# mravanelli/pytorch-kaldi

Hardware: AMD Instinct MI355X
Metric: train_frames_per_sec (higher is better)
Workload: dtype bf16

## Files before the change

include/pk_amd.h:

```cpp
#ifndef PK_AMD_H
#define PK_AMD_H

#include <stdint.h>

#ifdef __cplusplus
extern "C" {
#endif

#define PK_PREC_F32 0
#define PK_PREC_BF16 1

#define PK_ACT_LINEAR 0
#define PK_ACT_RELU 1
#define PK_ACT_TANH 2
#define PK_ACT_SIGMOID 3
#define PK_ACT_LEAKY_RELU 4
#define PK_ACT_ELU 5

#define PK_CELL_LIGRU 0
#define PK_CELL_RNN 1
#define PK_CELL_LSTM 2
#define PK_CELL_GRU 3
#define PK_CELL_MINGRU 4

#define PK_REC_STEPWISE 0
#define PK_REC_PERSISTENT 1

int pk_version(void);
const char* pk_last_error(void);
int pk_num_cu(void);

int pk_gemm(void* stream, int prec, int M, int N, int K, float alpha, const float* A, int64_t a_rs,
            int64_t a_cs, const float* B, int64_t b_rs, int64_t b_cs, float beta, float* C, int64_t ldc,
            const float* bias, int splitk, float* workspace);
void pk_gemm_f32_set_form(int form);

int pk_gemm_bf16_tile_m(int M);
int pk_gemm_bf16_auto_splitk(int M, int N, int K);
int pk_gemm_bf16_auto_splitk_cus(int M, int N, int K, int cus);
void pk_gemm_bf16_set_tile(int tile);
int pk_gemm_bf16(void* stream, int M, int N, int K, float alpha, const uint16_t* A, int64_t lda, int a_kc,
                 const uint16_t* B, int64_t ldb, int b_kc, float beta, float* C, int64_t ldc, const float* bias,
                 int splitk, float* workspace);
int64_t pk_gemm_bf16_stats_floats(int M, int N);
int pk_gemm_bf16_stats(void* stream, int M, int N, int K, float alpha, const uint16_t* A, int64_t lda, int a_kc,
                       const uint16_t* B, int64_t ldb, int b_kc, float* C, int64_t ldc, const float* bias, float* stats,
                       int* row_blocks);
int pk_cvt_bf16(void* stream, const float* src, int64_t ld_src, int64_t rows, int nseg, int seglen, int segpad,
                uint16_t* dst, int64_t ld_dst);

int64_t pk_bn_partial_floats(int64_t M, int64_t N);
int pk_bn_stats(void* stream, const float* x, int64_t ldx, int64_t M, int64_t N, float* partial, float* mean,
                float* var);
int pk_bn_stats_merge(void* stream, const float* partial, int rb, int64_t N, float* mean, float* var);
int pk_bn_finalize(void* stream, int64_t N, const float* mean, const float* var, const float* gamma,
                   const float* beta, float eps, float* scale, float* shift, float* running_mean,
                   float* running_var, float momentum, double count);
int pk_bn_finalize_gates(void* stream, int G, int H, const float* mean, const float* var, const float* gamma,
                         const float* beta, float eps, float* scale, float* shift, float* const* running_mean,
                         float* const* running_var, int64_t* const* num_batches, float momentum, double count);
int pk_bn_stats_merge_finalize_gates(void* stream, const float* partial, int rb, int G, int H, float* mean, float* var,
                                     const float* gamma, const float* beta, float eps, float* scale, float* shift,
                                     float* const* running_mean, float* const* running_var, int64_t* const* num_batches,
                                     float momentum, double count);
int pk_affine_act_fwd(void* stream, const float* x, int64_t ldx, int64_t M, int64_t N, const float* scale,
                      const float* shift, int act, const float* mask, float* y, int64_t ldy);
int pk_act_bwd(void* stream, const float* dy, const float* a, const float* mask, int act, int64_t n, float* g);
int pk_bn_bwd_reduce(void* stream, const float* g, const float* g2, int64_t ldg, const float* x, int64_t ldx,
                     int64_t M, int64_t N, const float* mean, const float* var, float eps, float* partial,
                     float* sum_g, float* sum_gx);
int pk_bn_bwd_apply(void* stream, const float* g, const float* g2, int64_t ldg, const float* x, int64_t ldx,
                    int64_t M, int64_t N, const float* mean, const float* var, float eps, const float* gamma,
                    const float* sum_g, const float* sum_gx, double count, float* dx, int64_t lddx);
int pk_bn_bwd_bf16(void* stream, const uint16_t* g0, const uint16_t* g1, int64_t g_pitch, int G, int H, const float* x,
                   int64_t ldx, int64_t M, const float* mean, const float* var, float eps, const float* gamma,
                   double count, float* partial, float* sum_g, float* sum_gx, uint16_t* out, int64_t out_pitch,
                   float* acc_beta, float* acc_gamma);
int pk_bn_act_bwd_small_covers(int64_t M, int64_t N);
int pk_bn_act_bwd_small(void* stream, const float* dy, const float* a, const float* mask, int act, const float* z,
                        const float* mean, const float* var, float eps, const float* gamma, int64_t M, int64_t N,
                        uint16_t* dzb, int64_t ldb, float* dz, float* sum_g, float* sum_gx, float* acc_beta,
                        float* acc_gamma, float* db, float* acc_bias);
int pk_colsum(void* stream, const float* g, const float* g2, int64_t ldg, int64_t M, int64_t N, float* partial,
              float* out);
int pk_add(void* stream, const float* a, const float* b, int64_t n, float* out);

int pk_mt19937_bernoulli(void* stream, uint32_t* state, int64_t n, float keep, float* out);

int pk_sinc_bank_fwd(void* stream, const float* low_hz, const float* band_hz, const float* n_, const float* window, int N, int K,
                     float sample_rate, float min_low, float min_band, float* filt, float* mx, int32_t* kstar);
int pk_sinc_bank_bwd(void* stream, const float* g, const float* low_hz, const float* band_hz, const float* n_, const float* window,
                     const float* mx, const int32_t* kstar, int N, int K, float sample_rate, float min_low, float min_band,
                     float* dlow, float* dband);

int pk_ln_last_act_drop_fwd(void* stream, const float* z, int64_t B, int C, int L, const float* gamma, const float* beta,
                            float eps, int act, const float* mask, float* a, float* y, float* mean, float* rinv);
int pk_ln_last_act_drop_bwd(void* stream, const float* dy, const float* z, const float* a, const float* mask, int64_t B, int C,
                            int L, const float* gamma, const float* mean, const float* rinv, float eps, int act, float* dz,
                            float* pg);

int pk_layernorm_fwd(void* stream, const float* x, int64_t rows, int64_t F, const float* gamma, const float* beta,
                     float eps, float* y, float* mean, float* rinv);
int pk_layernorm_bwd(void* stream, const float* dy, const float* x, int64_t rows, int64_t F, const float* gamma,
                     const float* mean, const float* rinv, float eps, float* dx, float* dgx);

int pk_logsoftmax_fwd(void* stream, const float* x, int64_t rows, int64_t N, float* y);
int pk_logsoftmax_bwd(void* stream, const float* dy, const float* y, int64_t rows, int64_t N, float* dx);
int pk_logsoftmax_bwd_ld(void* stream, const float* dy, const float* y, int64_t rows, int64_t N, float* dx, int64_t lddx);
int pk_logsoftmax_fwd_ld(void* stream, const float* x, int64_t ldx, int64_t rows, int64_t N, float* y);
int64_t pk_logsoftmax_bwd_bf16_partial_floats(int64_t rows, int64_t N);
int pk_logsoftmax_bwd_bf16(void* stream, const float* dy, const float* y, int64_t rows, int64_t N, uint16_t* dxb,
                           int64_t ldb, float* partial, float* colsum);
int64_t pk_nll_err_partial_floats(int64_t rows);
int pk_nll_err_fwd(void* stream, const float* y, const int64_t* lab, int64_t ignore_index, int64_t rows, int64_t N,
                   float* partial, float* out4, float* loss_out, float* bad_acc);
int pk_logsoftmax_fwd_ld_argmax(void* stream, const float* x, int64_t ldx, int64_t rows, int64_t N, float* y, int32_t* amax);
int pk_nll_err_fwd_argmax(void* stream, const float* y, const int64_t* lab, const int32_t* amax, int64_t ignore_index,
                          int64_t rows, int64_t N, float* partial, float* out4, float* loss_out, float* bad_acc);
int pk_nll_logsoftmax_bwd_bf16(void* stream, const float* y, const int64_t* lab, const float* dloss, const float* count,
                               int64_t ignore_index, int64_t rows, int64_t N, uint16_t* dxb, int64_t ldb, float* partial,
                               float* colsum);
int pk_logsoftmax_bwd_bf16_p(void* stream, const float* dy, const float* y, int64_t rows, int64_t N, uint16_t* dxb,
                             int64_t ldb, int64_t pitch, float* partial, float* colsum);
int pk_nll_logsoftmax_bwd_bf16_p(void* stream, const float* y, const int64_t* lab, const float* dloss, const float* count,
                                 int64_t ignore_index, int64_t rows, int64_t N, uint16_t* dxb, int64_t ldb, int64_t pitch,
                                 float* partial, float* colsum);

int pk_rec_num_saved(int cell);
int pk_rec_num_gates(int cell);
int64_t pk_rec_work_floats(int cell, int T, int B, int bidir, int H);
int64_t pk_rec_ln_saved_floats(int T, int B, int bidir, int H);
int64_t pk_rec_ln_work_floats(int T, int B, int bidir, int H);
int pk_rec_fwd(void* stream, int algo, int prec, int cell, int act, int T, int B, int bidir, int H,
               const float* P, const float* pscale, const float* pshift, const float* U, const float* mask,
               float mask_scalar, const float* ln_gamma, const float* ln_beta, float* Y, float* S, float* LNS,
               float* work);
int pk_rec_bwd(void* stream, int algo, int prec, int cell, int act, int T, int B, int bidir, int H,
               const float* U, const float* mask, float mask_scalar, const float* ln_gamma, const float* Y,
               const float* S, const float* LNS, const float* dY, float* dP2, float* dU, float* dln_gamma,
               float* dln_beta, float* work);

int pk_rec_plan_cus(int R, int H);
int pk_rec_self_fill(int cell);
int pk_rec_fwd_bf16(void* stream, int cell, int act, int T, int B, int bidir, int H, const float* P,
                    const float* pscale, const float* pshift, const float* U, const float* mask, float mask_scalar,
                    float* Y, float* S, uint16_t* Yb, int64_t y_pitch, int prefilled);
int pk_rec_bwd_bf16(void* stream, int cell, int act, int T, int B, int bidir, int H, const float* U, const float* mask,
                    float mask_scalar, const float* Y, const float* S, const float* dY, float* dP2, uint16_t* dGb,
                    int64_t g_pitch, int prefilled);
int pk_rec_fwd_bf16_ln(void* stream, int cell, int act, int T, int B, int bidir, int H, const float* P,
                       const float* pscale, const float* pshift, const float* U, const float* mask, float mask_scalar,
                       const float* ln_gamma, const float* ln_beta, float ln_eps, float* Y, float* S, float* LNS,
                       uint16_t* Yb, int64_t y_pitch, int prefilled, float* lnwork);
int pk_rec_bwd_bf16_ln(void* stream, int cell, int act, int T, int B, int bidir, int H, const float* U, const float* mask,
                       float mask_scalar, const float* ln_gamma, float ln_eps, const float* Y, const float* S,
                       const float* LNS, const float* dY, float* dP2, uint16_t* dGb, int64_t g_pitch, int prefilled,
                       float* lnwork, float* dln_gamma, float* dln_beta);
void pk_persist2_set_trace(void* dev_buf);
void pk_persist2_set_empty_step(int on);
void pk_persist2_set_mode(int force_safe);
void pk_persist2_set_poll_delay(int units);
void pk_persist2_set_lstm_waves(int waves);
int pk_persist2_get_lstm_waves(void);
void pk_rec_helper_set_mode(int mode);
int pk_rec_helper_get_mode(void);
int pk_rec2p_fwd_bf16(void* stream, int cell, int act, int T, int B, int bidir, int H, const float* P,
                      const float* pscale, const float* pshift, const float* U, const float* mask, float mask_scalar,
                      float* Y, float* S, uint16_t* Yb, uint16_t* Xb, int64_t y_pitch, int prefilled);
int pk_rec2p_bwd_bf16(void* stream, int cell, int act, int T, int B, int bidir, int H, const float* U, const float* mask,
                      float mask_scalar, const float* Y, const float* S, const float* dY, uint16_t* dGb, int64_t g_pitch,
                      int prefilled);
int pk_rec2p_fwd_bf16_ln(void* stream, int cell, int act, int T, int B, int bidir, int H, const float* P,
                         const float* pscale, const float* pshift, const float* U, const float* mask, float mask_scalar,
                         const float* ln_gamma, const float* ln_beta, float ln_eps, float* Y, float* S, float* LNS,
                         uint16_t* Yb, uint16_t* Xb, int64_t y_pitch, int prefilled, float* lnwork);
int pk_rec2p_bwd_bf16_ln(void* stream, int cell, int act, int T, int B, int bidir, int H, const float* U, const float* mask,
                         float mask_scalar, const float* ln_gamma, float ln_eps, const float* Y, const float* S,
                         const float* LNS, const float* dY, uint16_t* dGb, int64_t g_pitch, int prefilled, float* lnwork,
                         float* dln_gamma, float* dln_beta);
unsigned pk_persist2_error_count(void);
void pk_persist2_error_reset(void);

int pk_conv1d_pool_fwd(void* stream, const float* x, const float* w, const float* bias, int B, int Cin, int L,
                       int Cout, int K, int pool, float* y, int32_t* argmax, float* work);
int64_t pk_conv_fwd_work_floats(int Cin, int Cout, int K);
int64_t pk_conv_partial_floats(int B, int Cin, int L, int Cout, int K, int pool);
int pk_conv1d_pool_bwd(void* stream, const float* x, const float* w, const float* dy, const int32_t* argmax, int B,
                       int Cin, int L, int Cout, int K, int pool, float* dw, float* dbias, float* dx,
                       float* partial);

int pk_rmsprop_step(void* stream, float* p, const float* g, float* square_avg, int64_t n, float lr, float alpha,
                    float eps, float weight_decay);
int pk_sgd_step(void* stream, float* p, const float* g, float* momentum_buf, int64_t n, float lr, float momentum,
                float weight_decay, int first_step);
int pk_adam_step(void* stream, float* p, const float* g, float* exp_avg, float* exp_avg_sq, float* max_exp_avg_sq,
                 int64_t n, float lr, float beta1, float beta2, float eps, float weight_decay, int step);
int pk_fused_step(void* stream, int kind, float* p, float* g, float* s0, float* s1, float* s2, int64_t n, float lr, float h0,
                  float h1, float h2, float weight_decay, int step, int zero_grad, const int64_t* segs, int nseg,
                  uint16_t* shadow);

unsigned pk_persist_error_count(void);
void pk_persist_error_reset(void);

int pk_linear_bn_act_bf16_covers(int64_t M, int64_t N, int64_t K);
int pk_linear_bn_act_bf16(void* stream, int M, int N, int K, const uint16_t* xb, int64_t ldx, const uint16_t* wb, int64_t ldw,
                          const float* bias, const float* gamma, const float* beta, float eps, float momentum,
                          float* running_mean, float* running_var, int act, const float* mask, float* z, float* a,
                          float* y, uint16_t* yb, int64_t ldyb, float* mean, float* var);
int pk_gemm_bf16_small_splitk(int M, int N, int K);
int pk_linear_bn_act_bf16_sk(void* stream, int M, int N, int K, const uint16_t* xb, int64_t ldx, const uint16_t* wb,
                             int64_t ldw, const float* bias, const float* gamma, const float* beta, float eps,
                             float momentum, float* running_mean, float* running_var, int act, const float* mask,
                             float* z, float* a, float* y, uint16_t* yb, int64_t ldyb, float* mean, float* var,
                             int splitk, float* ws);
int pk_conv1d_pool_dgrad(void* stream, const float* w, const float* dy, const int32_t* argmax, int B, int Cin, int L, int Cout,
                         int K, int pool, float* dx, float* work);
int pk_conv_bf16_covers(int Cin, int Cout, int K, int pool);
int64_t pk_conv_bf16_work_floats(int B, int Cin, int L, int Cout, int K, int pool, int backward);
int pk_conv1d_pool_fwd_bf16(void* stream, const float* x, const float* w, const float* bias, int B, int Cin, int L, int Cout,
                            int K, int pool, float* y, int32_t* argmax, float* work);
int pk_conv1d_pool_bwd_bf16(void* stream, const float* x, const float* w, const float* dy, const int32_t* argmax, int B,
                            int Cin, int L, int Cout, int K, int pool, float* dw, float* dx, float* work);
int pk_selftest_mfma(void* stream, int* h_bad_count);
int pk_selftest_permlane(void* stream, int* h_bad_count);
int pk_selftest_dpp_row_sum(void* stream, int* h_bad_count);
int pk_selftest_cu_hog(void* stream, int blocks, int usec, float* buf);

typedef struct pk_ark pk_ark;
pk_ark* pk_ark_open(const char* path, int64_t offset);
void pk_ark_close(pk_ark* a);
int pk_ark_next(pk_ark* a, int key_expected, char* key, int keycap, int64_t* rows, int64_t* cols);
int pk_ark_read(pk_ark* a, float* dst);
int pk_ark_skip(pk_ark* a);
int pk_ivec_next(pk_ark* a, char* key, int keycap, int64_t* n);
int pk_ivec_read(pk_ark* a, int32_t* dst);
int pk_context_window(const float* x, int64_t rows, int64_t cols, int left, int right, float* out);
int pk_mean_var_norm(float* x, int64_t rows, int64_t cols);

#ifdef __cplusplus
}
#endif
#endif
```

pytorch-kaldi_amd/_lib.py:

```python
import ctypes
import os
import re
import threading

HERE = os.path.dirname(os.path.abspath(__file__))
LIB_PATH = os.path.join(HERE, "lib", "libpk_amd.so")
HEADER = os.path.join(HERE, "..", "include", "pk_amd.h")

_lock = threading.Lock()
_lib = None

c_void_p, c_int, c_float, c_double, c_int64 = ctypes.c_void_p, ctypes.c_int, ctypes.c_float, ctypes.c_double, ctypes.c_int64
P = c_void_p

SIGNATURES = {
    "pk_version": (c_int, []),
    "pk_last_error": (ctypes.c_char_p, []),
    "pk_num_cu": (c_int, []),
    "pk_gemm": (c_int, [P, c_int, c_int, c_int, c_int, c_float, P, c_int64, c_int64, P, c_int64, c_int64, c_float, P,
                        c_int64, P, c_int, P]),
    "pk_gemm_f32_set_form": (None, [c_int]),
    "pk_gemm_bf16_tile_m": (c_int, [c_int]),
    "pk_gemm_bf16_auto_splitk": (c_int, [c_int, c_int, c_int]),
    "pk_gemm_bf16_set_tile": (None, [c_int]),
    "pk_gemm_bf16": (c_int, [P, c_int, c_int, c_int, c_float, P, c_int64, c_int, P, c_int64, c_int, c_float, P, c_int64, P,
                             c_int, P]),
    "pk_gemm_bf16_stats_floats": (c_int64, [c_int, c_int]),
    "pk_gemm_bf16_stats": (c_int, [P, c_int, c_int, c_int, c_float, P, c_int64, c_int, P, c_int64, c_int, P, c_int64, P, P, P]),
    "pk_bn_stats_merge": (c_int, [P, P, c_int, c_int64, P, P]),
    "pk_cvt_bf16": (c_int, [P, P, c_int64, c_int64, c_int, c_int, c_int, P, c_int64]),
    "pk_bn_partial_floats": (c_int64, [c_int64, c_int64]),
    "pk_bn_stats": (c_int, [P, P, c_int64, c_int64, c_int64, P, P, P]),
    "pk_bn_finalize": (c_int, [P, c_int64, P, P, P, P, c_float, P, P, P, P, c_float, c_double]),
    "pk_bn_finalize_gates": (c_int, [P, c_int, c_int, P, P, P, P, c_float, P, P, P, P, P, c_float, c_double]),
    "pk_bn_stats_merge_finalize_gates": (c_int, [P, P, c_int, c_int, c_int, P, P, P, P, c_float, P, P, P, P, P, c_float,
                                                 c_double]),
    "pk_affine_act_fwd": (c_int, [P, P, c_int64, c_int64, c_int64, P, P, c_int, P, P, c_int64]),
    "pk_act_bwd": (c_int, [P, P, P, P, c_int, c_int64, P]),
    "pk_bn_bwd_reduce": (c_int, [P, P, P, c_int64, P, c_int64, c_int64, c_int64, P, P, c_float, P, P, P]),
    "pk_bn_bwd_apply": (c_int, [P, P, P, c_int64, P, c_int64, c_int64, c_int64, P, P, c_float, P, P, P, c_double, P,
                                c_int64]),
    "pk_bn_bwd_bf16": (c_int, [P, P, P, c_int64, c_int, c_int, P, c_int64, c_int64, P, P, c_float, P, c_double, P, P, P, P,
                               c_int64, P, P]),
    "pk_colsum": (c_int, [P, P, P, c_int64, c_int64, c_int64, P, P]),
    "pk_add": (c_int, [P, P, P, c_int64, P]),
    "pk_mt19937_bernoulli": (c_int, [P, P, c_int64, c_float, P]),
    "pk_sinc_bank_fwd": (c_int, [P, P, P, P, P, c_int, c_int, c_float, c_float, c_float, P, P, P]),
    "pk_sinc_bank_bwd": (c_int, [P, P, P, P, P, P, P, P, c_int, c_int, c_float, c_float, c_float, P, P]),
    "pk_ln_last_act_drop_fwd": (c_int, [P, P, c_int64, c_int, c_int, P, P, c_float, c_int, P, P, P, P, P]),
    "pk_ln_last_act_drop_bwd": (c_int, [P, P, P, P, P, c_int64, c_int, c_int, P, P, P, c_float, c_int, P, P]),
    "pk_layernorm_fwd": (c_int, [P, P, c_int64, c_int64, P, P, c_float, P, P, P]),
    "pk_layernorm_bwd": (c_int, [P, P, P, c_int64, c_int64, P, P, P, c_float, P, P]),
    "pk_logsoftmax_fwd": (c_int, [P, P, c_int64, c_int64, P]),
    "pk_logsoftmax_bwd": (c_int, [P, P, P, c_int64, c_int64, P]),
    "pk_logsoftmax_bwd_ld": (c_int, [P, P, P, c_int64, c_int64, P, c_int64]),
    "pk_logsoftmax_fwd_ld": (c_int, [P, P, c_int64, c_int64, c_int64, P]),
    "pk_logsoftmax_fwd_ld_argmax": (c_int, [P, P, c_int64, c_int64, c_int64, P, P]),
    "pk_logsoftmax_bwd_bf16_partial_floats": (c_int64, [c_int64, c_int64]),
    "pk_logsoftmax_bwd_bf16": (c_int, [P, P, P, c_int64, c_int64, P, c_int64, P, P]),
    "pk_nll_err_partial_floats": (c_int64, [c_int64]),
    "pk_nll_err_fwd": (c_int, [P, P, P, c_int64, c_int64, c_int64, P, P, P, P]),
    "pk_nll_err_fwd_argmax": (c_int, [P, P, P, P, c_int64, c_int64, c_int64, P, P, P, P]),
    "pk_nll_logsoftmax_bwd_bf16": (c_int, [P, P, P, P, P, c_int64, c_int64, c_int64, P, c_int64, P, P]),
    "pk_logsoftmax_bwd_bf16_p": (c_int, [P, P, P, c_int64, c_int64, P, c_int64, c_int64, P, P]),
    "pk_nll_logsoftmax_bwd_bf16_p": (c_int, [P, P, P, P, P, c_int64, c_int64, c_int64, P, c_int64, c_int64, P, P]),
    "pk_rec_num_saved": (c_int, [c_int]),
    "pk_rec_num_gates": (c_int, [c_int]),
    "pk_conv1d_pool_dgrad": (c_int, [P, P, P, P, c_int, c_int, c_int, c_int, c_int, c_int, P, P]),
    "pk_conv_bf16_covers": (c_int, [c_int, c_int, c_int, c_int]),
    "pk_conv_bf16_work_floats": (c_int64, [c_int, c_int, c_int, c_int, c_int, c_int, c_int]),
    "pk_conv1d_pool_fwd_bf16": (c_int, [P, P, P, P, c_int, c_int, c_int, c_int, c_int, c_int, P, P, P]),
    "pk_conv1d_pool_bwd_bf16": (c_int, [P, P, P, P, P, c_int, c_int, c_int, c_int, c_int, c_int, P, P, P]),
    "pk_bn_act_bwd_small_covers": (c_int, [c_int64, c_int64]),
    "pk_bn_act_bwd_small": (c_int, [P, P, P, P, c_int, P, P, P, c_float, P, c_int64, c_int64, P, c_int64, P, P, P, P, P, P, P]),
    "pk_rec_work_floats": (c_int64, [c_int, c_int, c_int, c_int, c_int]),
    "pk_rec_ln_saved_floats": (c_int64, [c_int, c_int, c_int, c_int]),
    "pk_rec_ln_work_floats": (c_int64, [c_int, c_int, c_int, c_int]),
    "pk_rec_fwd": (c_int, [P, c_int, c_int, c_int, c_int, c_int, c_int, c_int, c_int, P, P, P, P, P, c_float, P, P, P,
                           P, P, P]),
    "pk_rec_bwd": (c_int, [P, c_int, c_int, c_int, c_int, c_int, c_int, c_int, c_int, P, P, c_float, P, P, P, P, P, P,
                           P, P, P, P]),
    "pk_rec_self_fill": (c_int, [c_int]),
    "pk_rec_plan_cus": (c_int, [c_int, c_int]),
    "pk_gemm_bf16_auto_splitk_cus": (c_int, [c_int, c_int, c_int, c_int]),
    "pk_rec_fwd_bf16": (c_int, [P, c_int, c_int, c_int, c_int, c_int, c_int, P, P, P, P, P, c_float, P, P, P, c_int64, c_int]),
    "pk_rec_bwd_bf16": (c_int, [P, c_int, c_int, c_int, c_int, c_int, c_int, P, P, c_float, P, P, P, P, P, c_int64, c_int]),
    "pk_rec2p_fwd_bf16_ln": (c_int, [P, c_int, c_int, c_int, c_int, c_int, c_int, P, P, P, P, P, c_float, P, P, c_float, P, P, P,
                                     P, P, c_int64, c_int, P]),
    "pk_rec2p_bwd_bf16_ln": (c_int, [P, c_int, c_int, c_int, c_int, c_int, c_int, P, P, c_float, P, c_float, P, P, P, P, P,
                                     c_int64, c_int, P, P, P]),
    "pk_rec_fwd_bf16_ln": (c_int, [P, c_int, c_int, c_int, c_int, c_int, c_int, P, P, P, P, P, c_float, P, P, c_float, P, P, P,
                                   P, c_int64, c_int, P]),
    "pk_rec_bwd_bf16_ln": (c_int, [P, c_int, c_int, c_int, c_int, c_int, c_int, P, P, c_float, P, c_float, P, P, P, P, P, P,
                                   c_int64, c_int, P, P, P]),
    "pk_rec2p_fwd_bf16": (c_int, [P, c_int, c_int, c_int, c_int, c_int, c_int, P, P, P, P, P, c_float, P, P, P, P, c_int64, c_int]),
    "pk_rec2p_bwd_bf16": (c_int, [P, c_int, c_int, c_int, c_int, c_int, c_int, P, P, c_float, P, P, P, P, c_int64, c_int]),
    "pk_persist2_set_trace": (None, [P]),
    "pk_persist2_set_empty_step": (None, [c_int]),
    "pk_persist2_set_mode": (None, [c_int]),
    "pk_persist2_set_poll_delay": (None, [c_int]),
    "pk_persist2_set_lstm_waves": (None, [c_int]),
    "pk_rec_helper_set_mode": (None, [c_int]),
    "pk_rec_helper_get_mode": (c_int, []),
    "pk_persist2_get_lstm_waves": (c_int, []),
    "pk_persist2_error_count": (ctypes.c_uint, []),
    "pk_persist2_error_reset": (None, []),
    "pk_conv1d_pool_fwd": (c_int, [P, P, P, P, c_int, c_int, c_int, c_int, c_int, c_int, P, P, P]),
    "pk_conv_fwd_work_floats": (c_int64, [c_int, c_int, c_int]),
    "pk_conv_partial_floats": (c_int64, [c_int, c_int, c_int, c_int, c_int, c_int]),
    "pk_conv1d_pool_bwd": (c_int, [P, P, P, P, P, c_int, c_int, c_int, c_int, c_int, c_int, P, P, P, P]),
    "pk_ark_open": (P, [ctypes.c_char_p, c_int64]),
    "pk_ark_close": (None, [P]),
    "pk_ark_next": (c_int, [P, c_int, ctypes.c_char_p, c_int, ctypes.POINTER(c_int64), ctypes.POINTER(c_int64)]),
    "pk_ark_read": (c_int, [P, P]),
    "pk_ark_skip": (c_int, [P]),
    "pk_ivec_next": (c_int, [P, ctypes.c_char_p, c_int, ctypes.POINTER(c_int64)]),
    "pk_ivec_read": (c_int, [P, P]),
    "pk_context_window": (c_int, [P, c_int64, c_int64, c_int, c_int, P]),
    "pk_mean_var_norm": (c_int, [P, c_int64, c_int64]),
    "pk_rmsprop_step": (c_int, [P, P, P, P, c_int64, c_float, c_float, c_float, c_float]),
    "pk_sgd_step": (c_int, [P, P, P, P, c_int64, c_float, c_float, c_float, c_int]),
    "pk_adam_step": (c_int, [P, P, P, P, P, P, c_int64, c_float, c_float, c_float, c_float, c_float, c_int]),
    "pk_fused_step": (c_int, [P, c_int, P, P, P, P, P, c_int64, c_float, c_float, c_float, c_float, c_float, c_int, c_int, P, c_int, P]),
    "pk_persist_error_count": (ctypes.c_uint, []),
    "pk_persist_error_reset": (None, []),
    "pk_linear_bn_act_bf16_covers": (c_int, [c_int64, c_int64, c_int64]),
    "pk_linear_bn_act_bf16": (c_int, [P, c_int, c_int, c_int, P, c_int64, P, c_int64, P, P, P, c_float, c_float, P, P, c_int, P,
                                      P, P, P, P, c_int64, P, P]),
    "pk_gemm_bf16_small_splitk": (c_int, [c_int, c_int, c_int]),
    "pk_linear_bn_act_bf16_sk": (c_int, [P, c_int, c_int, c_int, P, c_int64, P, c_int64, P, P, P, c_float, c_float, P, P, c_int, P,
                                         P, P, P, P, c_int64, P, P, c_int, P]),
    "pk_selftest_mfma": (c_int, [P, ctypes.POINTER(c_int)]),
    "pk_selftest_permlane": (c_int, [P, ctypes.POINTER(c_int)]),
    "pk_selftest_dpp_row_sum": (c_int, [P, ctypes.POINTER(c_int)]),
    "pk_selftest_cu_hog": (c_int, [P, c_int, c_int, P]),
}


def declared_symbols():
    with open(HEADER) as f:
        text = re.sub(r"/\*.*?\*/", "", f.read(), flags=re.S)
    return sorted(set(re.findall(r"\b(pk_[a-z0-9_]+)\s*\(", text)))


class PkError(RuntimeError):
    pass


def _map_torch_hip_runtime():
    import torch

    hip = os.path.join(os.path.dirname(torch.__file__), "lib", "libamdhip64.so")
    if os.path.exists(hip):
        ctypes.CDLL(hip, mode=ctypes.RTLD_GLOBAL)
    return hip


def hip_runtimes_mapped():
    try:
        with open("/proc/self/maps") as f:
            return {line.split()[-1] for line in f if "libamdhip64" in line}
    except OSError:
        return set()


def load():
    global _lib
    if _lib is not None:
        return _lib
    with _lock:
        if _lib is not None:
            return _lib
        if not os.path.exists(LIB_PATH):
            raise PkError(
                "libpk_amd.so is not built (%s). Run `python -c 'import __graft_entry__ as g; g.build()'`; "
                "this engine has no CPU fallback." % LIB_PATH)
        warn_unknown_switches()
        _map_torch_hip_runtime()
        lib = ctypes.CDLL(LIB_PATH)
        runtimes = hip_runtimes_mapped()
        if len(runtimes) > 1:
            raise PkError("two HIP runtimes in one process (%s): libpk_amd.so must share the one torch uses - streams and "
                          "device pointers of one runtime mean nothing to the other" % ", ".join(sorted(runtimes)))
        for name, (res, args) in SIGNATURES.items():
            fn = getattr(lib, name)
            fn.restype = res
            fn.argtypes = args
        _lib = lib
    return _lib


def check(rc, what):
    if rc != 0:
        msg = load().pk_last_error()
        raise PkError("%s failed (rc=%d): %s" % (what, rc, msg.decode() if msg else "?"))


def raise_if_persist_failed():
    lib = load()
    n = lib.pk_persist_error_count() + lib.pk_persist2_error_count()
    if n:
        lib.pk_persist_error_reset()
        lib.pk_persist2_error_reset()
        raise PkError("persistent recurrent kernel: %d wave(s) timed out waiting for a peer workgroup "
                      "(results of that launch are invalid)" % n)


_profiler = None
_raw_load = load


class _TimedLib:

    def __init__(self, lib, prof):
        self._lib, self._prof = lib, prof

    def __getattr__(self, name):
        fn = getattr(self._lib, name)
        sig = SIGNATURES.get(name)
        if sig is None or not sig[1] or sig[1][0] is not P or name.startswith("pk_selftest_"):
            return fn
        prof = self._prof

        def timed(*a):
            import torch

            e0 = torch.cuda.Event(enable_timing=True)
            e1 = torch.cuda.Event(enable_timing=True)
            e0.record()
            rc = fn(*a)
            e1.record()
            prof.events.append((name, e0, e1))
            return rc

        return timed


_EXP_CACHE = (None, {})
# ... 107 lines not shown
```

pytorch-kaldi_amd/csrc/pk_gemm_bf16.hip:

```cpp
#include <stdlib.h>

#include "pk_common.h"

namespace {

constexpr int TM = 128, TN = 128, TK = 64;
typedef short s4v __attribute__((ext_vector_type(4)));

struct BArgs {
    int M, N, K;
    float alpha, beta;
    const unsigned short* A;
    long lda;
    const unsigned short* B;
    long ldb;
    float* C;
    long ldc;
    const float* bias;
    float* ws;
    int k_per_split;
    int tiles_m, tiles_n;
    int items, per_xcd;
    const unsigned short* zeros;
    float* stats;
// ... 993 lines not shown
                for (int ah = 0; ah < 2; ++ah)
#pragma unroll
                    for (int i = 0; i < 4; ++i) {
                        const int row = m0 + ah * 128 + wm * 64 + i * 16 + (lane & 15);
                        const f32x4 v = acc[ah][bh][i][j];
                        f32x4 o;
#pragma unroll
                        for (int r = 0; r < 4; ++r) o[r] = alpha * v[r] + bv[r];
                        *reinterpret_cast<f32x4*>(base + (long)row * ld + col) = o;
                    }
            }
        return;
    }
#pragma unroll
    for (int ah = 0; ah < 2; ++ah)
#pragma unroll
        for (int bh = 0; bh < 2; ++bh)
#pragma unroll
            for (int i = 0; i < 4; ++i)
#pragma unroll
                for (int j = 0; j < 2; ++j)
                    store_frag(p, acc[ah][bh][i][j], m0 + ah * 128 + wm * 64 + i * 16 + (lane & 15),
                               n0 + bh * 128 + wn * 32 + j * 16 + (lane >> 4) * 4, split, vec_ok);
}

__global__ void splitk_reduce_bf_kernel(const float* __restrict__ ws, int splitk, int M, int N, float alpha, float beta,
                                        const float* __restrict__ bias, float* __restrict__ C, long ldc) {
    const long total = (long)M * N;
    if ((N & 3) == 0 && (ldc & 3) == 0 && (((uintptr_t)C | (uintptr_t)ws) & 15) == 0) {
        const long quads = total >> 2;
        for (long qd = blockIdx.x * (long)blockDim.x + threadIdx.x; qd < quads; qd += (long)gridDim.x * blockDim.x) {
            const long i = qd << 2;
            const int row = (int)(i / N), col = (int)(i - (long)row * N);
            f32x4 s = f32x4{0.f, 0.f, 0.f, 0.f};
            for (int k0 = 0; k0 < splitk; k0 += 8) {
                f32x4 t[8];
#pragma unroll
                for (int j = 0; j < 8; ++j) t[j] = *reinterpret_cast<const f32x4*>(ws + (long)(k0 + j < splitk ? k0 + j : splitk - 1) * total + i);
#pragma unroll
                for (int j = 0; j < 8; ++j)
#pragma unroll
                    for (int e = 0; e < 4; ++e) s[e] += (k0 + j < splitk) ? t[j][e] : 0.f;
            }
            float* c = C + (long)row * ldc + col;
            f32x4 o;
#pragma unroll
            for (int e = 0; e < 4; ++e) o[e] = alpha * s[e] + (bias ? bias[col + e] : 0.f);
            if (beta != 0.f) {
                const f32x4 cv = *reinterpret_cast<const f32x4*>(c);
#pragma unroll
                for (int e = 0; e < 4; ++e) o[e] += beta * cv[e];
            }
            *reinterpret_cast<f32x4*>(c) = o;
        }
        return;
    }
    for (long i = blockIdx.x * (long)blockDim.x + threadIdx.x; i < total; i += (long)gridDim.x * blockDim.x) {
        const int row = (int)(i / N), col = (int)(i % N);
        float s = 0.f;
        for (int k = 0; k < splitk; ++k) s += ws[(long)k * total + i];
        float o = alpha * s + (bias ? bias[col] : 0.f);
        float* c = C + (long)row * ldc + col;
        if (beta != 0.f) o += beta * (*c);
        *c = o;
    }
}

__global__ void cvt_bf16_kernel(const float* __restrict__ src, long lds, long rows, int nseg, int seglen, int segpad,
                                unsigned short* __restrict__ dst, long ldd) {
    const long chunks_per_row = ldd >> 3;
    const long total = rows * chunks_per_row;
    for (long i = blockIdx.x * (long)blockDim.x + threadIdx.x; i < total; i += (long)gridDim.x * blockDim.x) {
        const long r = i / chunks_per_row;
        const int c0 = (int)(i - r * chunks_per_row) * 8;
        const float* s = src + r * lds;
        unsigned pk[4];
#pragma unroll
        for (int e = 0; e < 4; ++e) {
            float v[2];
#pragma unroll
            for (int h = 0; h < 2; ++h) {
                const int c = c0 + 2 * e + h;
                const int sg = c / segpad, off = c - sg * segpad;
                v[h] = (sg < nseg && off < seglen) ? s[sg * seglen + off] : 0.f;
            }
            pk[e] = pk_pack_bf2(v[0], v[1]);
        }
        *reinterpret_cast<uint4*>(dst + r * ldd + c0) = make_uint4(pk[0], pk[1], pk[2], pk[3]);
    }
}

}

extern "C" int pk_cvt_bf16(void* stream, const float* src, int64_t ld_src, int64_t rows, int nseg, int seglen, int segpad,
                           uint16_t* dst, int64_t ld_dst) {
    if (rows <= 0) return 0;
    PK_REQUIRE(nseg >= 1 && seglen >= 1 && segpad >= seglen, "pk_cvt_bf16: bad segments");
    PK_REQUIRE((ld_dst % 8) == 0 && ld_dst >= (int64_t)nseg * segpad - (segpad - seglen) && ((uintptr_t)dst & 15) == 0,
               "pk_cvt_bf16: destination pitch must be a multiple of 8 elements and hold every segment");
    const long total = rows * (ld_dst >> 3);
    long blocks = (total + 255) / 256;
    if (blocks > 8192) blocks = 8192;
    hipLaunchKernelGGL(cvt_bf16_kernel, dim3((unsigned)blocks), dim3(256), 0, pk_stream(stream), src, (long)ld_src,
                       (long)rows, nseg, seglen, segpad, (unsigned short*)dst, (long)ld_dst);
    PK_LAUNCH_CHECK();
    return 0;
}

static int g_gemm_tile_forced = -1;
extern "C" void pk_gemm_bf16_set_tile(int tile) { g_gemm_tile_forced = (tile == 128 || tile == 256) ? tile : 0; }
static int gemm_tile_for(int M, int N, int a_kc, int b_kc, int K = 1 << 30) {
    int& forced = g_gemm_tile_forced;
    if (forced < 0) {
        const char* e = pk_experiment("gemm_tile");
        forced = (e && atoi(e) == 128) ? 128 : (e && atoi(e) == 256) ? 256 : 0;
    }
    if (forced) return forced;
    static int rows256 = -1;
    if (rows256 < 0) {
        const char* e = pk_experiment("gemm_tile_rows");
        rows256 = (e && atoi(e) == 0) ? 0 : 1;
    }
    if (rows256 && a_kc && M >= 16384 && N >= 1024) return 256;
    if (!a_kc && !b_kc && M >= 1024 && N >= 1024) {
        const long tiles256 = (long)((M + 255) / 256) * ((N + 255) / 256);
        if (K < 2048 && tiles256 < 64) return 128;
        return 256;
    }
    return 128;
}

extern "C" int pk_gemm_bf16_tile_m(int M) {
    (void)M;
    return TM;
}

extern "C" int pk_gemm_bf16_auto_splitk_cus(int M, int N, int K, int cus) {
    if (K < 2048 || M <= 0 || N <= 0) return 1;
    const int t = gemm_tile_for(M, N, 0, 0);
    const long tiles = (long)((M + t - 1) / t) * ((N + t - 1) / t);
    long ncu = pk_num_cu();
    if (cus > 0 && cus < ncu) ncu = cus;
    long s = (t == 256 ? ncu : 2 * ncu) / (tiles > 0 ? tiles : 1);
    if (s < 1) s = 1;
    if (s > 32) s = 32;
    const long kmax = K / 512 > 0 ? K / 512 : 1;
    if (s > kmax) s = kmax;
    return (int)s;
}
extern "C" int pk_gemm_bf16_auto_splitk(int M, int N, int K) { return pk_gemm_bf16_auto_splitk_cus(M, N, K, 0); }

static int gemm_bf16_impl(void* stream, int M, int N, int K, float alpha, const uint16_t* A, int64_t lda, int a_kc,
                          const uint16_t* B, int64_t ldb, int b_kc, float beta, float* C, int64_t ldc, const float* bias,
                          int splitk, float* workspace, float* stats) {
    if (M <= 0 || N <= 0) return 0;
    PK_REQUIRE(K >= 0, "pk_gemm_bf16: negative K");
    PK_REQUIRE((lda % 8) == 0 && (ldb % 8) == 0 && ((uintptr_t)A & 15) == 0 && ((uintptr_t)B & 15) == 0,
               "pk_gemm_bf16: operands need 16-byte aligned bases and pitches that are multiples of 8 elements");
    PK_REQUIRE(!a_kc || (K % 8) == 0 || lda >= ((K + 7) & ~7), "pk_gemm_bf16: A pitch shorter than K rounded up to 8");
    PK_REQUIRE(!b_kc || (K % 8) == 0 || ldb >= ((K + 7) & ~7), "pk_gemm_bf16: B pitch shorter than K rounded up to 8");
    PK_REQUIRE(a_kc || lda >= ((M + 7) & ~7), "pk_gemm_bf16: k-major A needs a pitch of at least M rounded up to 8");
    PK_REQUIRE(b_kc || ldb >= ((N + 7) & ~7), "pk_gemm_bf16: k-major B needs a pitch of at least N rounded up to 8");
    hipStream_t st = pk_stream(stream);
    BArgs p;
    p.M = M; p.N = N; p.K = K;
    p.alpha = alpha; p.beta = beta;
    p.A = A; p.lda = lda; p.B = B; p.ldb = ldb;
    p.C = C; p.ldc = ldc; p.bias = bias;
    p.stats = stats;
    const int tile = gemm_tile_for(M, N, a_kc, b_kc, K);
    PK_REQUIRE(stats == nullptr || (tile == 256 && a_kc && b_kc && splitk <= 1 && beta == 0.f), "pk_gemm_bf16_stats: internal: shape not covered");
    p.tiles_m = (M + tile - 1) / tile;
    p.tiles_n = (N + tile - 1) / tile;
    static void* zp = nullptr;
    if (zp == nullptr) PK_CHECK_HIP(hipGetSymbolAddress(&zp, HIP_SYMBOL(g_zero_page)));
    p.zeros = (const unsigned short*)zp;
    if (splitk < 1) splitk = 1;
    if (splitk > 1) {
        PK_REQUIRE(workspace != nullptr, "pk_gemm_bf16: split-K needs a workspace");
        int kps = (K + splitk - 1) / splitk;
        kps = ((kps + TK - 1) / TK) * TK;
        splitk = kps > 0 ? (K + kps - 1) / kps : 1;
        p.k_per_split = kps;
    }
    if (splitk <= 1) {
        splitk = 1;
        p.k_per_split = ((K + TK - 1) / TK) * TK;
        if (p.k_per_split == 0) p.k_per_split = TK;
    }
    p.ws = splitk > 1 ? workspace : nullptr;
    p.items = splitk * p.tiles_m * p.tiles_n;
    p.per_xcd = (p.items + 7) / 8;
    {
        static int skinny_on = -1;
        if (skinny_on < 0) {
            const char* e = pk_experiment("gemm_skinny");
            skinny_on = (e && e[0] == '0') ? 0 : 1;
        }
        if (skinny_on && !g_gemm_tile_forced && a_kc && M <= TM && splitk > 1 && p.k_per_split <= SK_TILES * TK && stats == nullptr) {
            static bool attr_done = false;
            if (!attr_done) {
                PK_CHECK_HIP(hipFuncSetAttribute((const void*)gemm_bf16sk_kernel<true>, hipFuncAttributeMaxDynamicSharedMemorySize, SK_TILES * SSTAGE));
                PK_CHECK_HIP(hipFuncSetAttribute((const void*)gemm_bf16sk_kernel<false>, hipFuncAttributeMaxDynamicSharedMemorySize, SK_TILES * SSTAGE));
                attr_done = true;
            }
            const dim3 sgrid((unsigned)((N + SN - 1) / SN), (unsigned)splitk);
            if (b_kc) hipLaunchKernelGGL((gemm_bf16sk_kernel<true>), sgrid, dim3(256), SK_TILES * SSTAGE, st, p);
            else hipLaunchKernelGGL((gemm_bf16sk_kernel<false>), sgrid, dim3(256), SK_TILES * SSTAGE, st, p);
            PK_LAUNCH_CHECK();
            const long total = (long)M * N;
            int blocks = (int)((total + 255) / 256);
            if (blocks > 2048) blocks = 2048;
            hipLaunchKernelGGL(splitk_reduce_bf_kernel, dim3(blocks), dim3(256), 0, st, workspace, splitk, M, N, alpha, beta,
                               bias, C, (long)ldc);
            PK_LAUNCH_CHECK();
            return 0;
        }
        if (skinny_on && !g_gemm_tile_forced && !a_kc && !b_kc && splitk == 1 && K <= 512 && stats == nullptr &&
            (long)((M + TM - 1) / TM) * ((N + TN - 1) / TN) <= 192 && M >= 64 && N >= 64) {
            const dim3 tgrid((unsigned)((N + 63) / 64), (unsigned)((M + 63) / 64));
            hipLaunchKernelGGL(gemm_bf16_t64_kernel, tgrid, dim3(256), T64_TILES * T64_STAGE, st, p);
            PK_LAUNCH_CHECK();
            return 0;
        }
        if (skinny_on && !g_gemm_tile_forced && a_kc && M <= TM && N >= 4 * SN && splitk == 1 && stats == nullptr) {
            BnActArgs q = {};
            const dim3 sgrid((unsigned)((N + SN - 1) / SN));
            if (b_kc) hipLaunchKernelGGL((gemm_bf16s_kernel<false, true>), sgrid, dim3(256), 2 * SSTAGE, st, p, q);
            else hipLaunchKernelGGL((gemm_bf16s_kernel<false, false>), sgrid, dim3(256), 2 * SSTAGE, st, p, q);
            PK_LAUNCH_CHECK();
            return 0;
        }
    }
    if (tile == 256) {
        static bool attr_done = false;
        if (!attr_done) {
            PK_CHECK_HIP(hipFuncSetAttribute((const void*)gemm_bf16_256_kernel<true, true>, hipFuncAttributeMaxDynamicSharedMemorySize, 8 * PIECE));
            PK_CHECK_HIP(hipFuncSetAttribute((const void*)gemm_bf16_256_kernel<true, false>, hipFuncAttributeMaxDynamicSharedMemorySize, 8 * PIECE));
            PK_CHECK_HIP(hipFuncSetAttribute((const void*)gemm_bf16_256_kernel<false, true>, hipFuncAttributeMaxDynamicSharedMemorySize, 8 * PIECE));
            PK_CHECK_HIP(hipFuncSetAttribute((const void*)gemm_bf16_256_kernel<false, false>, hipFuncAttributeMaxDynamicSharedMemorySize, 8 * PIECE));
            attr_done = true;
        }
        dim3 grid256((unsigned)(p.per_xcd * 8)), block512(512);
        const size_t lds256 = 8 * PIECE;
        if (a_kc && b_kc) hipLaunchKernelGGL((gemm_bf16_256_kernel<true, true>), grid256, block512, lds256, st, p);
        else if (a_kc && !b_kc) hipLaunchKernelGGL((gemm_bf16_256_kernel<true, false>), grid256, block512, lds256, st, p);
        else if (!a_kc && b_kc) hipLaunchKernelGGL((gemm_bf16_256_kernel<false, true>), grid256, block512, lds256, st, p);
        else hipLaunchKernelGGL((gemm_bf16_256_kernel<false, false>), grid256, block512, lds256, st, p);
        PK_LAUNCH_CHECK();
        if (splitk > 1) {
            const long total = (long)M * N;
            int blocks = (int)((total + 255) / 256);
            if (blocks > 2048) blocks = 2048;
            hipLaunchKernelGGL(splitk_reduce_bf_kernel, dim3(blocks), dim3(256), 0, st, workspace, splitk, M, N, alpha, beta,
                               bias, C, (long)ldc);
            PK_LAUNCH_CHECK();
        }
        return 0;
    }
    dim3 grid((unsigned)(p.per_xcd * 8)), block(256);
    static int forced = -1;
    if (forced < 0) {
        const char* e = pk_experiment("gemm_stages");
        forced = (e && e[0] == '1') ? 1 : (e && e[0] == '2') ? 2 : 0;
        PK_CHECK_HIP(hipFuncSetAttribute((const void*)gemm_bf16x_kernel<true, true, 2>, hipFuncAttributeMaxDynamicSharedMemorySize, 65536));
        PK_CHECK_HIP(hipFuncSetAttribute((const void*)gemm_bf16x_kernel<true, false, 2>, hipFuncAttributeMaxDynamicSharedMemorySize, 65536));
        PK_CHECK_HIP(hipFuncSetAttribute((const void*)gemm_bf16x_kernel<false, true, 2>, hipFuncAttributeMaxDynamicSharedMemorySize, 65536));
        PK_CHECK_HIP(hipFuncSetAttribute((const void*)gemm_bf16x_kernel<false, false, 2>, hipFuncAttributeMaxDynamicSharedMemorySize, 65536));
    }
    const int stages = forced ? forced : (a_kc ? 1 : 2);
    const size_t lds = stages == 2 ? 65536 : 32768;
#define PK_LAUNCH_BF(ST)                                                                                     \
    do {                                                                                                     \
        if (a_kc && b_kc) hipLaunchKernelGGL((gemm_bf16x_kernel<true, true, ST>), grid, block, lds, st, p);    \
        else if (a_kc && !b_kc) hipLaunchKernelGGL((gemm_bf16x_kernel<true, false, ST>), grid, block, lds, st, p); \
        else if (!a_kc && b_kc) hipLaunchKernelGGL((gemm_bf16x_kernel<false, true, ST>), grid, block, lds, st, p); \
        else hipLaunchKernelGGL((gemm_bf16x_kernel<false, false, ST>), grid, block, lds, st, p);              \
    } while (0)
    if (stages == 2) PK_LAUNCH_BF(2);
    else PK_LAUNCH_BF(1);
#undef PK_LAUNCH_BF
    PK_LAUNCH_CHECK();
    if (splitk > 1) {
        const long total = (long)M * N;
        int blocks = (int)((total + 255) / 256);
        if (blocks > 2048) blocks = 2048;
        hipLaunchKernelGGL(splitk_reduce_bf_kernel, dim3(blocks), dim3(256), 0, st, workspace, splitk, M, N, alpha, beta,
                           bias, C, (long)ldc);
        PK_LAUNCH_CHECK();
    }
    return 0;
}

extern "C" int pk_gemm_bf16(void* stream, int M, int N, int K, float alpha, const uint16_t* A, int64_t lda, int a_kc,
                            const uint16_t* B, int64_t ldb, int b_kc, float beta, float* C, int64_t ldc,
                            const float* bias, int splitk, float* workspace) {
    return gemm_bf16_impl(stream, M, N, K, alpha, A, lda, a_kc, B, ldb, b_kc, beta, C, ldc, bias, splitk, workspace, nullptr);
}

extern "C" int64_t pk_gemm_bf16_stats_floats(int M, int N) { return (int64_t)((M + 255) / 256) * N * 3; }

extern "C" int pk_gemm_bf16_stats(void* stream, int M, int N, int K, float alpha, const uint16_t* A, int64_t lda, int a_kc,
                                  const uint16_t* B, int64_t ldb, int b_kc, float* C, int64_t ldc, const float* bias,
                                  float* stats, int* row_blocks) {
    PK_REQUIRE(row_blocks != nullptr, "pk_gemm_bf16_stats: null row_blocks");
    const bool fused = stats != nullptr && M > 0 && N > 0 && K > 0 && a_kc && b_kc && gemm_tile_for(M, N, a_kc, b_kc) == 256;
    *row_blocks = fused ? (M + 255) / 256 : 0;
    return gemm_bf16_impl(stream, M, N, K, alpha, A, lda, a_kc, B, ldb, b_kc, 0.f, C, ldc, bias, 1, nullptr,
                          fused ? stats : nullptr);
}

extern "C" int pk_gemm_bf16_small_splitk(int M, int N, int K) {
    if (M < 1 || M > TM || N < 1 || K < 2 * TK) return 1;
    const int col_tiles = (N + SN - 1) / SN;
    int s = 256 / col_tiles;
    const int need = (K + SK_TILES * TK - 1) / (SK_TILES * TK);
    if (s < need) s = need;
    if (s > 16) s = 16;
    const int tiles = (K + TK - 1) / TK;
    if (s > tiles) s = tiles;
    if (s < 2) return 1;
    int kps = ((K + s - 1) / s + TK - 1) / TK * TK;
    if (kps > SK_TILES * TK) return 1;
    return (K + kps - 1) / kps;
}

extern "C" int pk_linear_bn_act_bf16_sk(void* stream, int M, int N, int K, const uint16_t* xb, int64_t ldx, const uint16_t* wb,
                                        int64_t ldw, const float* bias, const float* gamma, const float* beta, float eps,
                                        float momentum, float* running_mean, float* running_var, int act, const float* mask,
                                        float* z, float* a, float* y, uint16_t* yb, int64_t ldyb, float* mean, float* var,
                                        int splitk, float* ws) {
    PK_REQUIRE(pk_linear_bn_act_bf16_covers(M, N, K), "pk_linear_bn_act_bf16_sk: needs 2 <= M <= 128 rows and N a multiple of 8 (got %d x %d)", M, N);
    PK_REQUIRE((ldx % 8) == 0 && (ldw % 8) == 0 && ((uintptr_t)xb & 15) == 0 && ((uintptr_t)wb & 15) == 0 && ldx >= ((K + 7) & ~7) &&
                   ldw >= ((K + 7) & ~7),
               "pk_linear_bn_act_bf16_sk: operands need 16-byte aligned bases and pitches that are multiples of 8 elements");
    PK_REQUIRE(z && a && yb && mean && var && (mask == nullptr || y != nullptr) && ldyb >= N && (ldyb % 4) == 0,
               "pk_linear_bn_act_bf16_sk: null output or bad pitch");
    PK_REQUIRE((((uintptr_t)z | (uintptr_t)a | (uintptr_t)y | (uintptr_t)mask | (uintptr_t)ws | (uintptr_t)bias) & 15) == 0 && ((uintptr_t)yb & 7) == 0,
               "pk_linear_bn_act_bf16_sk: fp32 matrices need 16-byte aligned bases");
    PK_REQUIRE(splitk >= 2 && ws != nullptr, "pk_linear_bn_act_bf16_sk: needs splitk >= 2 and a workspace of splitk x M x N floats");
    int kps = ((K + splitk - 1) / splitk + TK - 1) / TK * TK;
    PK_REQUIRE(kps <= SK_TILES * TK, "pk_linear_bn_act_bf16_sk: %d splits of K = %d exceed %d k-tiles per workgroup", splitk, K, SK_TILES);
    splitk = (K + kps - 1) / kps;
    hipStream_t st = pk_stream(stream);
    BArgs p;
    p.M = M; p.N = N; p.K = K;
    p.alpha = 1.f; p.beta = 0.f;
    p.A = xb; p.lda = ldx; p.B = wb; p.ldb = ldw;
    p.C = z; p.ldc = N; p.bias = nullptr;
    p.stats = nullptr; p.ws = ws;
    p.tiles_m = 1; p.tiles_n = (N + TN - 1) / TN;
    p.k_per_split = kps;
    p.items = p.tiles_n; p.per_xcd = (p.items + 7) / 8;
    static void* zp = nullptr;
    if (zp == nullptr) PK_CHECK_HIP(hipGetSymbolAddress(&zp, HIP_SYMBOL(g_zero_page)));
    p.zeros = (const unsigned short*)zp;
    static bool attr_done = false;
    if (!attr_done) {
        PK_CHECK_HIP(hipFuncSetAttribute((const void*)gemm_bf16sk_kernel<true>, hipFuncAttributeMaxDynamicSharedMemorySize, SK_TILES * SSTAGE));
        attr_done = true;
    }
    hipLaunchKernelGGL((gemm_bf16sk_kernel<true>), dim3((unsigned)((N + SN - 1) / SN), (unsigned)splitk), dim3(256), SK_TILES * SSTAGE, st, p);
    PK_LAUNCH_CHECK();
    BnActArgs q;
    q.gamma = gamma; q.beta = beta; q.mask = mask;
    q.eps = eps; q.momentum = momentum; q.unbias = M > 1 ? (float)M / (float)(M - 1) : 1.f;
    q.rmean = running_mean; q.rvar = running_var; q.mean = mean; q.var = var;
    q.zout = z; q.aout = a; q.yout = y; q.yb = (unsigned short*)yb; q.ldyb = ldyb; q.act = act;
    hipLaunchKernelGGL(linear_bn_act_epi_kernel, dim3((unsigned)((N + EP_COLS - 1) / EP_COLS)), dim3(256), 0, st, ws, splitk, M, N, bias, q);
    PK_LAUNCH_CHECK();
    return 0;
}

extern "C" int pk_linear_bn_act_bf16_covers(int64_t M, int64_t N, int64_t K) {
    return M >= 2 && M <= TM && N >= 8 && (N % 8) == 0 && K >= 1;
}
extern "C" int pk_linear_bn_act_bf16(void* stream, int M, int N, int K, const uint16_t* xb, int64_t ldx, const uint16_t* wb,
                                     int64_t ldw, const float* bias, const float* gamma, const float* beta, float eps,
                                     float momentum, float* running_mean, float* running_var, int act, const float* mask,
                                     float* z, float* a, float* y, uint16_t* yb, int64_t ldyb, float* mean, float* var) {
    PK_REQUIRE(pk_linear_bn_act_bf16_covers(M, N, K), "pk_linear_bn_act_bf16: needs 2 <= M <= 128 rows and N a multiple of 8 (got %d x %d)", M, N);
    PK_REQUIRE((ldx % 8) == 0 && (ldw % 8) == 0 && ((uintptr_t)xb & 15) == 0 && ((uintptr_t)wb & 15) == 0 && ldx >= ((K + 7) & ~7) &&
                   ldw >= ((K + 7) & ~7),
               "pk_linear_bn_act_bf16: operands need 16-byte aligned bases and pitches that are multiples of 8 elements");
    PK_REQUIRE(z && a && yb && mean && var && (mask == nullptr || y != nullptr) && ldyb >= N && (ldyb % 4) == 0,
               "pk_linear_bn_act_bf16: null output or bad pitch");
    PK_REQUIRE((((uintptr_t)z | (uintptr_t)a | (uintptr_t)y | (uintptr_t)mask) & 15) == 0 && ((uintptr_t)yb & 7) == 0,
               "pk_linear_bn_act_bf16: fp32 matrices need 16-byte aligned bases");
    hipStream_t st = pk_stream(stream);
    BArgs p;
    p.M = M; p.N = N; p.K = K;
    p.alpha = 1.f; p.beta = 0.f;
    p.A = xb; p.lda = ldx; p.B = wb; p.ldb = ldw;
    p.C = z; p.ldc = N; p.bias = bias;
    p.stats = nullptr; p.ws = nullptr;
    p.tiles_m = 1; p.tiles_n = (N + TN - 1) / TN;
    p.k_per_split = ((K + TK - 1) / TK) * TK;
    p.items = p.tiles_n; p.per_xcd = (p.items + 7) / 8;
    static void* zp = nullptr;
    if (zp == nullptr) PK_CHECK_HIP(hipGetSymbolAddress(&zp, HIP_SYMBOL(g_zero_page)));
    p.zeros = (const unsigned short*)zp;
    BnActArgs q;
    q.gamma = gamma; q.beta = beta; q.mask = mask;
    q.eps = eps; q.momentum = momentum; q.unbias = M > 1 ? (float)M / (float)(M - 1) : 1.f;
    q.rmean = running_mean; q.rvar = running_var; q.mean = mean; q.var = var;
    q.zout = z; q.aout = a; q.yout = y; q.yb = (unsigned short*)yb; q.ldyb = ldyb; q.act = act;
    hipLaunchKernelGGL((gemm_bf16s_kernel<true>), dim3((unsigned)((N + SN - 1) / SN)), dim3(256), 2 * SSTAGE, st, p, q);
    PK_LAUNCH_CHECK();
    return 0;
}
```

pytorch-kaldi_amd/csrc/pk_rec2_common.h:

```cpp
#pragma once
#ifndef PK_REC2_PRECISE
#define PK_CELL_FAST_MATH 1
#endif
#include "pk_cell.h"

#define PK_R2_FILL_AHEAD 4
struct R2Args {
    int T, B, R, H, Hp, YH, act;
    int C, Pn, rpc, row0;
    const float *P, *pscale, *pshift, *U, *mask;
    float mask_scalar;
    float* Y;
    float* S;
    unsigned short* Yb;
    unsigned short* Xb;
    int Ypitch;
    const float* dY;
    float* dP2;
    unsigned short* dGb;
    int Gpitch;
    float* Yx;
    float* dGx;
    float* Xx;
    unsigned* err;
    int spin_limit;
    float* trash;
    int poll_delay;
    int force_safe;
    unsigned* xcd_tab;
    unsigned hs_gen;
    unsigned long long* trace;
    int helper_delay;
    int self_fill;
    int flush_late;
    int empty_step;
    const float *ln_gamma, *ln_beta;
    float ln_eps;
    float* lnh;
    float* lnstat;
    float* lnx;
    float* lnpart;
    int ln_cg0;
    int ln_ncg;
};

struct Plan2 {
    int Pn, C, rpc, launches;
};

namespace {

typedef unsigned int u32x4 __attribute__((ext_vector_type(4)));

constexpr int KPAD = 576;
constexpr int KSTEPS = 18;
constexpr int RMAX = 16;

__host__ __device__ constexpr int pk_r2_lda_bf16(int k_elems) { return k_elems + 8 * ((((2 - k_elems / 8) % 16) + 16) % 16); }
__host__ __device__ constexpr int pk_r2_lda_f32(int k_elems) { return k_elems + 4 * ((((2 - k_elems / 4) % 16) + 16) % 16); }


#define PK_TRACE(slot)                                                                      \
    do {                                                                                    \
        if (TR && a.trace != nullptr && blockIdx.x == 0 && tid == 0) a.trace[(long)step_idx * 8 + (slot)] = __builtin_amdgcn_s_memtime(); \
    } while (0)

__device__ __forceinline__ bool has_sent16(const u32x4 v) {
    const unsigned m01 = v[0] > v[1] ? v[0] : v[1], m23 = v[2] > v[3] ? v[2] : v[3];
    return (m01 > m23 ? m01 : m23) == 0xFFFFFFFFu;
}
__device__ __forceinline__ unsigned short to_bf_pub(float f) {
    const unsigned short u = __builtin_bit_cast(unsigned short, (__bf16)f);
    return u == (unsigned short)0xFFFF ? (unsigned short)0x7FC0 : u;
}
__device__ __forceinline__ bool spin_check2(int& spins, int spin_limit, unsigned* err, int lane) {
    if (++spins > spin_limit) {
        if (lane == 0) atomicAdd_system(err, 1u);
        return true;
    }
    if ((spins & 63) == 0 && __hip_atomic_load(err, __ATOMIC_RELAXED, __HIP_MEMORY_SCOPE_SYSTEM) != 0u) return true;
    __builtin_amdgcn_s_sleep(1);
    return false;
}
__device__ __forceinline__ __amdgpu_buffer_rsrc_t make_rsrc(const void* p, unsigned bytes) {
    return __builtin_amdgcn_make_buffer_rsrc(const_cast<void*>(p), 0, (int)bytes, 0x00020000);
}

template <bool FAST>
__device__ __forceinline__ u32x4 poll_load(__amdgpu_buffer_rsrc_t rs, unsigned off) {
    return FAST ? __builtin_amdgcn_raw_buffer_load_b128(rs, off, 0, 2) : __builtin_amdgcn_raw_buffer_load_b128(rs, off, 0, 16);
}
template <bool FAST>
__device__ __forceinline__ void pub_store(__amdgpu_buffer_rsrc_t rs, unsigned off, u32x4 v) {
    if (FAST) __builtin_amdgcn_raw_buffer_store_b128(v, rs, off, 0, 0);
    else __builtin_amdgcn_raw_buffer_store_b128(v, rs, off, 0, 16);
}

template <int NCH, bool FAST>
__device__ __forceinline__ bool poll_to_lds(__amdgpu_buffer_rsrc_t rs, const unsigned (&goff)[NCH], const int (&loff)[NCH],
                                            unsigned char* tile, unsigned* err, int spin_limit, int lane, bool dead,
                                            int& retries) {
    u32x4 v[NCH];
#pragma unroll
    for (int i = 0; i < NCH; ++i) v[i] = poll_load<FAST>(rs, goff[i]);
    bool bad = false;
#pragma unroll
    for (int i = 0; i < NCH; ++i) bad = bad | has_sent16(v[i]);
    if (__any(bad) && !dead) {
        int spins = 0;
        while (true) {
#pragma unroll
            for (int i = 0; i < NCH; ++i)
                if (has_sent16(v[i])) v[i] = poll_load<FAST>(rs, goff[i]);
            bad = false;
#pragma unroll
            for (int i = 0; i < NCH; ++i) bad = bad | has_sent16(v[i]);
            ++retries;
            if (!__any(bad)) break;
            if (spin_check2(spins, spin_limit, err, lane)) {
                dead = true;
                break;
            }
        }
    }
#pragma unroll
    for (int i = 0; i < NCH; ++i) *reinterpret_cast<u32x4*>(tile + loff[i]) = v[i];
    return dead;
}

__device__ __forceinline__ float dpp_row_sum(float v) {
    v += __int_as_float(__builtin_amdgcn_update_dpp(0, __float_as_int(v), 0xB1, 0xF, 0xF, true));
    v += __int_as_float(__builtin_amdgcn_update_dpp(0, __float_as_int(v), 0x4E, 0xF, 0xF, true));
    v += __int_as_float(__builtin_amdgcn_update_dpp(0, __float_as_int(v), 0x141, 0xF, 0xF, true));
    v += __int_as_float(__builtin_amdgcn_update_dpp(0, __float_as_int(v), 0x140, 0xF, 0xF, true));
    return v;
}
__device__ __forceinline__ unsigned ln_bits(float f) {
    const unsigned u = __float_as_uint(f);
    return u == 0xFFFFFFFFu ? 0x7FC00000u : u;
}
template <bool FAST, int NP = 3>
__device__ __forceinline__ bool ln_row_allreduce(__amdgpu_buffer_rsrc_t rsx, unsigned pub_off, const unsigned (&poll_off)[NP],
                                                 float (&a)[4], float (&b)[4], unsigned* err, int spin_limit, int lane, bool dead) {
#pragma unroll
    for (int r = 0; r < 4; ++r) {
        a[r] = dpp_row_sum(a[r]);
        b[r] = dpp_row_sum(b[r]);
    }
    pub_store<FAST>(rsx, pub_off, u32x4{ln_bits(a[0]), ln_bits(b[0]), ln_bits(a[1]), ln_bits(b[1])});
    pub_store<FAST>(rsx, pub_off + 16u, u32x4{ln_bits(a[2]), ln_bits(b[2]), ln_bits(a[3]), ln_bits(b[3])});
    u32x4 v[2 * NP];
#pragma unroll
    for (int i = 0; i < 2 * NP; ++i) v[i] = poll_load<FAST>(rsx, poll_off[i >> 1] + (unsigned)(i & 1) * 16u);
    bool bad = false;
#pragma unroll
    for (int i = 0; i < 2 * NP; ++i) bad = bad | has_sent16(v[i]);
    if (__any(bad) && !dead) {
        int spins = 0;
        while (true) {
#pragma unroll
            for (int i = 0; i < 2 * NP; ++i)
                if (has_sent16(v[i])) v[i] = poll_load<FAST>(rsx, poll_off[i >> 1] + (unsigned)(i & 1) * 16u);
            bad = false;
#pragma unroll
            for (int i = 0; i < 2 * NP; ++i) bad = bad | has_sent16(v[i]);
            if (!__any(bad)) break;
            if (spin_check2(spins, spin_limit, err, lane)) {
                dead = true;
                break;
            }
        }
    }
#pragma unroll
    for (int r = 0; r < 4; ++r) {
        const int ch = r >> 1, e = (r & 1) * 2;
        float sa = __uint_as_float(v[ch][e]), sb = __uint_as_float(v[ch][e + 1]);
#pragma unroll
        for (int g = 1; g < NP; ++g) {
            sa += __uint_as_float(v[2 * g + ch][e]);
            sb += __uint_as_float(v[2 * g + ch][e + 1]);
        }
        a[r] = dpp_row_sum(sa);
        b[r] = dpp_row_sum(sb);
    }
    return dead;
}
template <int NP>
struct LnSlotsN {
    unsigned pub, poll[NP], slab, size;
    bool pub_ok, poll_ok[NP];
    __device__ __forceinline__ unsigned pub_at(int step) const { return pub_ok ? pub + (unsigned)step * slab : size; }
    __device__ __forceinline__ void poll_at(int step, unsigned (&o)[NP]) const {
#pragma unroll
        for (int i = 0; i < NP; ++i) o[i] = poll_ok[i] ? poll[i] + (unsigned)step * slab : size;
    }
};
// ... 187 lines not shown
```

pytorch-kaldi_amd/csrc/pk_rec_persist2.hip:

```cpp
#include <atomic>
#include <stdlib.h>

#include "pk_rec2_common.h"

namespace {

template <int CELL, int ACT, bool TR, bool LN = false, bool NOSAVE = false>
__global__ __launch_bounds__(256, 1) void rec2_fwd_kernel(R2Args a) {
    const int act = ACT >= 0 ? ACT : a.act;
    constexpr int G = pk_cell_gates(CELL), NS = pk_cell_saved(CELL);
    constexpr int LDA = pk_r2_lda_bf16(KPAD);
    constexpr int ATILE = RMAX * LDA * 2;
    constexpr int NCH = (RMAX * (KPAD / 8) + 255) / 256;
    constexpr int NF = G + 1 + NS + (LN ? 1 : 0);
    constexpr int WAVE_LDS = NF * 1024 + 512;
    constexpr int LDS_TRASH = 2 * ATILE + 4 * WAVE_LDS;
    extern __shared__ __attribute__((aligned(16))) unsigned char smem[];

    const int tid = threadIdx.x, lane = tid & 63, wave = tid >> 6;
    const int c = blockIdx.x % a.C, p = blockIdx.x / a.C;
    const int H = a.H, Hp = a.Hp, B = a.B, T = a.T, GH = G * H;
    const int n_base = a.row0 + c * a.rpc;
    int nrows = a.R - n_base;
    nrows = nrows < a.rpc ? nrows : a.rpc;
    if (nrows <= 0) return;
    const int ubase = p * 64 + wave * 16;
    const int unit = ubase + (lane & 15);
    const bool unit_ok = unit < H;
    const int kq = lane >> 4;

    bf16x8 Bf[G][KSTEPS];
    {
        const unsigned szU = (unsigned)((size_t)G * H * H * 4);
        const __amdgpu_buffer_rsrc_t rsU = make_rsrc(a.U, szU);
#pragma unroll
        for (int g = 0; g < G; ++g) {
            u32x4 raw[KSTEPS][2];
#pragma unroll
            for (int kk = 0; kk < KSTEPS; ++kk) {
                const int k0 = kk * 32 + kq * 8;
                const unsigned off = (unsigned)(((g * H + unit) * H + k0) * 4);
                raw[kk][0] = __builtin_amdgcn_raw_buffer_load_b128(rsU, (unit_ok && k0 < H) ? off : szU, 0, 0);
                raw[kk][1] = __builtin_amdgcn_raw_buffer_load_b128(rsU, (unit_ok && k0 + 4 < H) ? off + 16 : szU, 0, 0);
            }
#pragma unroll
            for (int kk = 0; kk < KSTEPS; ++kk) {
                bf16x8 f;
#pragma unroll
                for (int e = 0; e < 8; ++e) {
                    const int k = kk * 32 + kq * 8 + e;
                    const float w = (k < H) ? __uint_as_float(raw[kk][e >> 2][e & 3]) : 0.f;
                    f[e] = (short)pk_f2bf(w);
                }
                Bf[g][kk] = f;
            }
        }
    }
    float psc[G], psh[G];
#pragma unroll
    for (int g = 0; g < G; ++g) {
        psc[g] = unit_ok ? a.pscale[g * H + unit] : 0.f;
        psh[g] = unit_ok ? a.pshift[g * H + unit] : 0.f;
    }
    for (int i = tid; i < (LDS_TRASH + 16) / 4; i += 256) reinterpret_cast<unsigned*>(smem)[i] = 0u;

    const int CPR = Hp >> 3;
    const unsigned TS = (unsigned)B * a.Ypitch * 2u;
    const unsigned szYb = (unsigned)T * TS;
    unsigned cbase[NCH], cstep[NCH];
    int clds[NCH];
#pragma unroll
    for (int i = 0; i < NCH; ++i) {
        const int ci = tid + 256 * i;
        const bool ok = ci < nrows * CPR;
        const int row = ok ? ci / CPR : 0, col = ok ? ci - row * CPR : 0;
        const int n = n_base + row;
        const int dir = n >= B ? 1 : 0, b = n - dir * B;
        cbase[i] = ok ? ((unsigned)b * a.Ypitch + dir * Hp + col * 8) * 2u + (unsigned)(dir ? (T - 1) : 0) * TS : szYb;
        cstep[i] = ok ? (dir ? 0u - TS : TS) : 0u;
        clds[i] = ok ? row * (LDA * 2) + col * 16 : LDS_TRASH;
    }
    float rvf[4], msk[4], hprev[4], cprev[4];
#pragma unroll
    for (int r = 0; r < 4; ++r) {
        const int row = kq * 4 + r, n = n_base + row;
        const bool ok = row < nrows && unit_ok;
        rvf[r] = ok ? 1.f : 0.f;
        msk[r] = (a.mask != nullptr && ok) ? a.mask[(long)n * H + unit] : a.mask_scalar;
        hprev[r] = 0.f;
        cprev[r] = 0.f;
    }
    const int vrow = lane >> 2, vu0 = ubase + (lane & 3) * 4;
    const int vn = n_base + (vrow < nrows ? vrow : 0);
    const int vdir = vn >= B ? 1 : 0, vb = vn - vdir * B;
    int vnv = H - vu0;
    vnv = vnv > 4 ? 4 : (vnv < 0 ? 0 : vnv);
    const int edge = __any(vnv > 0 && vnv < 4) != 0 ? ((H & 1) ? 2 : 1) : 0;
    vnv = vrow < nrows ? vnv : 0;
    const unsigned vP0 = ((unsigned)vb * GH + vu0), vPs = (unsigned)B * GH;
    const unsigned vY0 = ((unsigned)vb * a.YH + vdir * H + vu0), vYs = (unsigned)B * a.YH;
    const unsigned vS0 = (((unsigned)vdir * T * B + vb) * (NS * H) + vu0), vSs = (unsigned)B * NS * H;
    const int prow = lane >> 1, phalf = lane & 1;
    const int pu0 = ubase + phalf * 8;
    const bool pk_ok = lane < 32 && prow < nrows && pu0 < Hp;
    const int pn = n_base + (prow < nrows ? prow : 0);
    const int pdir = pn >= B ? 1 : 0, pb = pn - pdir * B;
    const unsigned pbase = pk_ok ? ((unsigned)pb * a.Ypitch + pdir * Hp + pu0) * 2u : szYb;

    unsigned char* wl = smem + 2 * ATILE + wave * WAVE_LDS;
    float* patchP = reinterpret_cast<float*>(wl);
    float* patchY = reinterpret_cast<float*>(wl + G * 1024);
    float* patchS = reinterpret_cast<float*>(wl + (G + 1) * 1024);
    float* patchL = reinterpret_cast<float*>(wl + (G + 1 + NS) * 1024);
    unsigned short* patchB = reinterpret_cast<unsigned short*>(wl + NF * 1024);
    const __amdgpu_buffer_rsrc_t rs = make_rsrc(a.Yb, szYb);
    float* trash = a.trash + (tid & 63) * 4;
    const LnSlots ls = LN ? ln_slots(a, c, p, wave, lane, T) : LnSlots();
    const __amdgpu_buffer_rsrc_t rsx = make_rsrc(LN ? (const void*)a.lnx : (const void*)a.Yb, LN ? ls.size : 0u);
    const float gam = (LN && unit_ok) ? a.ln_gamma[unit] : 0.f, bet = (LN && unit_ok) ? a.ln_beta[unit] : 0.f;
    const float invH = 1.0f / (float)H, inv_nm1 = 1.0f / (float)(H - 1);
    float piv[4] = {0.f, 0.f, 0.f, 0.f};
    pk_f32x2 st_val = {0.f, 0.f};
    const int st_row = kq * 4 + (lane & 3);
    const bool st_ok = LN && p == 0 && wave == 0 && (lane & 15) < 4 && st_row < nrows;
    float* const st_base = st_ok ? a.lnstat + (long)(n_base + st_row) * 2 : trash;
    const long st_step = st_ok ? (long)a.R * 2 : 0;

    f32x4 pv[G];
    auto load_proj = [&](int tt, auto E) {
        const unsigned ts = (unsigned)(vdir ? (T - 1 - tt) : tt);
#pragma unroll
        for (int g = 0; g < G; ++g) pv[g] = ld4<decltype(E)::value>(a.P, vP0 + ts * vPs + g * H, vnv);
    };
    const bool want_y = a.Y != nullptr;
    auto flush_outputs = [&](int tt, auto E) {
        constexpr int EE = decltype(E)::value;
        const unsigned ts = (unsigned)(vdir ? (T - 1 - tt) : tt);
        if (!NOSAVE || want_y) st4<EE>(a.Y, vY0 + ts * vYs, vnv, trash, patch_get_vec(patchY, lane));
        if constexpr (!NOSAVE) {
#pragma unroll
            for (int k = 0; k < NS; ++k) st4<EE>(a.S, vS0 + ts * vSs + k * H, vnv, trash, patch_get_vec(patchS + k * 256, lane));
        }
        if (LN) {
            st4<EE>(a.lnh, vY0 + ts * vYs, vnv, trash, patch_get_vec(patchL, lane));
            *reinterpret_cast<pk_f32x2*>(st_base + (long)tt * st_step) = st_val;
        }
    };
#define PK_LP0(E) load_proj(0, E)
    PK_EDGE_DISPATCH(PK_LP0);
    const u32x4 sentinel = u32x4{0xFFFFFFFFu, 0xFFFFFFFFu, 0xFFFFFFFFu, 0xFFFFFFFFu};
    if (a.self_fill) {
        for (int tt = 0; tt < PK_R2_FILL_AHEAD && tt < T; ++tt)
            pub_store<false>(rs, pbase + (pk_ok ? (unsigned)(pdir ? (T - 1 - tt) : tt) * TS : 0u), sentinel);
        asm volatile("s_waitcnt vmcnt(0)" ::: "memory");
    }
    __syncthreads();

    bool dead = false;
    const bool fast_rt = __builtin_amdgcn_readfirstlane((int)(cluster_on_one_xcd(a, c, p, tid, dead) && a.force_safe == 0)) != 0;
    auto run = [&](auto FASTC, auto SEC) {
    const bool fast = decltype(FASTC)::value < 0 ? fast_rt : decltype(FASTC)::value != 0;
    constexpr int SE = decltype(SEC)::value;
    for (int t = 0; t < T; ++t) {
        const int step_idx = t;
        PK_TRACE(0);
        f32x4 acc[G];
#pragma unroll
        for (int g = 0; g < G; ++g) acc[g] = f32x4{0.f, 0.f, 0.f, 0.f};
        unsigned char* At = smem + (t & 1) * ATILE;
        if (t > 0) {
            unsigned goff[NCH];
#pragma unroll
            for (int i = 0; i < NCH; ++i) goff[i] = cbase[i] + (unsigned)(t - 1) * cstep[i];
            for (int d = 0; d < a.poll_delay; ++d) __builtin_amdgcn_s_sleep(1);
            int retries = 0;
            dead = fast ? poll_to_lds<NCH, true>(rs, goff, clds, At, a.err, a.spin_limit, lane, dead, retries)
                        : poll_to_lds<NCH, false>(rs, goff, clds, At, a.err, a.spin_limit, lane, dead, retries);
            if (a.trace != nullptr && blockIdx.x == 0 && tid == 0) a.trace[(long)step_idx * 8 + 6] = (unsigned long long)retries;
        }
        PK_TRACE(1);
#pragma unroll
        for (int g = 0; g < G; ++g) patch_put_vec(patchP + g * 256, lane, pv[g]);
        if (t > 0) PK_BARRIER_LDS();
        else PK_LDS_ORDER();
        PK_TRACE(2);
        if (t > 0) {
#define PK_FO(E) flush_outputs(t - 1, E)
            PK_EDGE_DISPATCH_S(PK_FO);
        }
        if (t + 1 < T) {
#define PK_LP1(E) load_proj(t + 1, E)
            PK_EDGE_DISPATCH_S(PK_LP1);
        }
        if (a.self_fill && t + PK_R2_FILL_AHEAD < T) {
            const unsigned off = pbase + (pk_ok ? (unsigned)(pdir ? (T - 1 - (t + PK_R2_FILL_AHEAD)) : (t + PK_R2_FILL_AHEAD)) * TS : 0u);
            if (fast) pub_store<true>(rs, off, sentinel);
            else pub_store<false>(rs, off, sentinel);
        }
        const bool empty = TR && a.empty_step != 0;
        if (t > 0 && !empty) {
            const unsigned char* Ar = At + (lane & 15) * (LDA * 2) + kq * 16;
#pragma unroll
            for (int kk = 0; kk < KSTEPS; ++kk) {
                const bf16x8 af = *reinterpret_cast<const bf16x8*>(Ar + kk * 64);
#pragma unroll
                for (int g = 0; g < G; ++g) acc[g] = __builtin_amdgcn_mfma_f32_16x16x32_bf16(af, Bf[g][kk], acc[g], 0, 0, 0);
            }
        }
        PK_TRACE(3);
        float pre[G][4];
#pragma unroll
        for (int g = 0; g < G; ++g) patch_get_cd(patchP + g * 256, kq, lane, pre[g]);
        float hv[4], sv[NS][4];
#pragma unroll
        for (int r = 0; r < 4; ++r) {
            float pr[G];
#pragma unroll
            for (int g = 0; g < G; ++g) pr[g] = pre[g][r] * psc[g] + psh[g] + acc[g][r];
            float h, cc, s[NS];
            if (empty) {
                h = 0.25f;
                cc = 0.f;
#pragma unroll
                for (int k = 0; k < NS; ++k) s[k] = pr[0];
            } else {
                pk_cell_fwd<CELL>(act, pr, hprev[r], cprev[r], msk[r], h, cc, s);
            }
            h = rvf[r] != 0.f ? h : 0.f;
            cc = rvf[r] != 0.f ? cc : 0.f;
            hprev[r] = h;
            cprev[r] = cc;
            hv[r] = h;
#pragma unroll
            for (int k = 0; k < NS; ++k) sv[k][r] = s[k];
            if (!LN) patchB[(kq * 4 + r) * 16 + (lane & 15)] = to_bf_pub(h);
        }
        if (LN) {
            if (t == 0) {
                float ma[4], mb[4];
#pragma unroll
                for (int r = 0; r < 4; ++r) {
                    ma[r] = rvf[r] != 0.f ? hv[r] : 0.f;
                    mb[r] = 0.f;
                }
                unsigned po0[3];
                ls.poll_at(T, po0);
                dead = fast ? ln_row_allreduce<true>(rsx, ls.pub_at(T), po0, ma, mb, a.err, a.spin_limit, lane, dead)
                            : ln_row_allreduce<false>(rsx, ls.pub_at(T), po0, ma, mb, a.err, a.spin_limit, lane, dead);
#pragma unroll
                for (int r = 0; r < 4; ++r) piv[r] = ma[r] * invH;
            }
            float la[4], lb[4];
#pragma unroll
            for (int r = 0; r < 4; ++r) {
                const float d = hv[r] - piv[r];
                la[r] = rvf[r] != 0.f ? d : 0.f;
                lb[r] = rvf[r] != 0.f ? d * d : 0.f;
            }
            unsigned po[3];
            ls.poll_at(t, po);
            dead = fast ? ln_row_allreduce<true>(rsx, ls.pub_at(t), po, la, lb, a.err, a.spin_limit, lane, dead)
                        : ln_row_allreduce<false>(rsx, ls.pub_at(t), po, la, lb, a.err, a.spin_limit, lane, dead);
            patch_put_cd(patchL, kq, lane, hv);
            float mu4[4], ri4[4];
#pragma unroll
            for (int r = 0; r < 4; ++r) {
                const float md = la[r] * invH;
                const float mu = piv[r] + md;
                const float var = fmaxf((lb[r] - la[r] * md) * inv_nm1, 0.f);
                const float ri = 1.0f / (sqrtf(var) + a.ln_eps);
                const float hn = rvf[r] != 0.f ? gam * ((hv[r] - mu) * ri) + bet : 0.f;
                hv[r] = hn;
                hprev[r] = hn;
                piv[r] = mu;
                mu4[r] = mu;
                ri4[r] = ri;
                patchB[(kq * 4 + r) * 16 + (lane & 15)] = to_bf_pub(hn);
            }
            const int u3 = lane & 3;
            st_val[0] = u3 == 0 ? mu4[0] : u3 == 1 ? mu4[1] : u3 == 2 ? mu4[2] : mu4[3];
            st_val[1] = u3 == 0 ? ri4[0] : u3 == 1 ? ri4[1] : u3 == 2 ? ri4[2] : ri4[3];
        }
        PK_TRACE(4);
        PK_LDS_ORDER();
        {
            const u32x4 o = *reinterpret_cast<const u32x4*>(reinterpret_cast<const unsigned char*>(patchB) + (prow & 15) * 32 + phalf * 16);
            const unsigned off = pbase + (pk_ok ? (unsigned)(pdir ? (T - 1 - t) : t) * TS : 0u);
            if (fast) pub_store<true>(rs, off, o);
            else pub_store<false>(rs, off, o);
        }
        if (!NOSAVE || want_y) patch_put_cd(patchY, kq, lane, hv);
        if constexpr (!NOSAVE) {
#pragma unroll
            for (int k = 0; k < NS; ++k) patch_put_cd(patchS + k * 256, kq, lane, sv[k]);
        }
        PK_LDS_ORDER();
        PK_TRACE(5);
    }
    };
    if constexpr (LN) {
        run(BoolC<-1>(), BoolC<-1>());
    } else {
        PK_RUN_SPECIALISED(run, fast_rt);
    }
#define PK_FOL(E) flush_outputs(T - 1, E)
    PK_EDGE_DISPATCH(PK_FOL);
}

template <int CELL, int ACT, bool TR, bool LN = false>
__global__ __launch_bounds__(256, 1) void rec2_bwd_kernel(R2Args a) {
    const int act = ACT >= 0 ? ACT : a.act;
    constexpr int G = pk_cell_gates(CELL), NS = pk_cell_saved(CELL);
    constexpr bool LSTM = (CELL == PK_CELL_LSTM);
    constexpr int LDA = pk_r2_lda_bf16(G * KPAD);
    constexpr int ATILE = RMAX * LDA * 2;
    constexpr int NBUF = (2 * ATILE > 96 * 1024) ? 1 : 2;
    constexpr int NCH = (RMAX * G * (KPAD / 8) + 255) / 256;
    constexpr int NIN = NS + 2 + (LSTM ? 1 : 0) + (LN ? 1 : 0);
    constexpr int ILN = NS + 2 + (LSTM ? 1 : 0);
    constexpr int WAVE_LDS = (NIN + G) * 1024 + G * 512;
    constexpr int LDS_TRASH = NBUF * ATILE + 4 * WAVE_LDS;
    extern __shared__ __attribute__((aligned(16))) unsigned char smem[];

    const int tid = threadIdx.x, lane = tid & 63, wave = tid >> 6;
    const int c = blockIdx.x % a.C, p = blockIdx.x / a.C;
    const int H = a.H, Hp = a.Hp, B = a.B, T = a.T, GH = G * H;
    const unsigned TB = (unsigned)T * B;
    const int n_base = a.row0 + c * a.rpc;
    int nrows = a.R - n_base;
    nrows = nrows < a.rpc ? nrows : a.rpc;
    if (nrows <= 0) return;
    const int ubase = p * 64 + wave * 16;
    const int unit = ubase + (lane & 15);
    const bool unit_ok = unit < H;
    const int kq = lane >> 4;

    bf16x8 Bf[G][KSTEPS];
    {
        const unsigned szU = (unsigned)((size_t)G * H * H * 4);
        const __amdgpu_buffer_rsrc_t rsU = make_rsrc(a.U, szU);
#pragma unroll
        for (int g = 0; g < G; ++g)
#pragma unroll
            for (int kk = 0; kk < KSTEPS; ++kk) {
                unsigned raw[8];
#pragma unroll
                for (int e = 0; e < 8; ++e) {
                    const int j = kk * 32 + kq * 8 + e;
                    raw[e] = __builtin_amdgcn_raw_buffer_load_b32(rsU, (unit_ok && j < H) ? (unsigned)(((g * H + j) * H + unit) * 4) : szU, 0, 0);
                }
                bf16x8 f;
#pragma unroll
                for (int e = 0; e < 8; ++e) f[e] = (short)pk_f2bf(__uint_as_float(raw[e]));
                Bf[g][kk] = f;
            }
    }
    for (int i = tid; i < (LDS_TRASH + 16) / 4; i += 256) reinterpret_cast<unsigned*>(smem)[i] = 0u;

    const int CPR = Hp >> 3;
    const unsigned TS = (unsigned)B * a.Gpitch * 2u;
    const unsigned ndir = (unsigned)(a.R / B);
    const unsigned szGb = ndir * (unsigned)T * TS;
    unsigned cbase[NCH], cstep[NCH];
    int clds[NCH];
#pragma unroll
    for (int i = 0; i < NCH; ++i) {
        const int ci = tid + 256 * i;
        const bool ok = ci < nrows * G * CPR;
        const int row = ok ? ci / (G * CPR) : 0;
        const int rem = ok ? ci - row * (G * CPR) : 0;
        const int g = rem / CPR, col = rem - g * CPR;
        const int n = n_base + row;
        const int dir = n >= B ? 1 : 0, b = n - dir * B;
        cbase[i] = ok ? (unsigned)dir * (unsigned)T * TS + ((unsigned)b * a.Gpitch + g * Hp + col * 8) * 2u +
                            (unsigned)(dir ? 0 : (T - 1)) * TS
                      : szGb;
        cstep[i] = ok ? (dir ? TS : 0u - TS) : 0u;
        clds[i] = ok ? row * (LDA * 2) + (g * KPAD + col * 8) * 2 : LDS_TRASH;
    }
    float rvf[4], msk[4], dh_dir[4], dc_car[4];
#pragma unroll
    for (int r = 0; r < 4; ++r) {
        const int row = kq * 4 + r, n = n_base + row;
        const bool ok = row < nrows && unit_ok;
        rvf[r] = ok ? 1.f : 0.f;
        msk[r] = (a.mask != nullptr && ok) ? a.mask[(long)n * H + unit] : a.mask_scalar;
        dh_dir[r] = 0.f;
        dc_car[r] = 0.f;
    }
    const int vrow = lane >> 2, vu0 = ubase + (lane & 3) * 4;
    const int vn = n_base + (vrow < nrows ? vrow : 0);
    const int vdir = vn >= B ? 1 : 0, vb = vn - vdir * B;
    int vnv = H - vu0;
    vnv = vnv > 4 ? 4 : (vnv < 0 ? 0 : vnv);
    const int edge = __any(vnv > 0 && vnv < 4) != 0 ? ((H & 1) ? 2 : 1) : 0;
    vnv = vrow < nrows ? vnv : 0;
    const unsigned vY0 = ((unsigned)vb * a.YH + vdir * H + vu0), vYs = (unsigned)B * a.YH;
    const unsigned vS0 = (((unsigned)vdir * TB + vb) * (NS * H) + vu0), vSs = (unsigned)B * NS * H;
    const unsigned vG0 = (((unsigned)vdir * TB + vb) * GH + vu0), vGs = (unsigned)B * GH;
    const int prow = lane >> 1, phalf = lane & 1;
    const int pu0 = ubase + phalf * 8;
    const bool pk_ok = lane < 32 && prow < nrows && pu0 < Hp;
    const int pn = n_base + (prow < nrows ? prow : 0);
    const int pdir = pn >= B ? 1 : 0, pb = pn - pdir * B;
    const unsigned pbase = pk_ok ? (unsigned)pdir * (unsigned)T * TS + ((unsigned)pb * a.Gpitch + pu0) * 2u : szGb;

    unsigned char* wl = smem + NBUF * ATILE + wave * WAVE_LDS;
    float* patchI = reinterpret_cast<float*>(wl);
    float* patchG = reinterpret_cast<float*>(wl + NIN * 1024);
    unsigned short* patchB = reinterpret_cast<unsigned short*>(wl + (NIN + G) * 1024);
    const __amdgpu_buffer_rsrc_t rs = make_rsrc(a.dGb, szGb);
    float* trash = a.trash + (tid & 63) * 4;
    const __amdgpu_buffer_rsrc_t rsx = make_rsrc(LN ? (const void*)a.lnx : (const void*)a.dGb,
                                                 LN ? (unsigned)T * ((unsigned)a.ln_ncg * 4u * 4u * (unsigned)a.Pn * 32u) : 0u);

    f32x4 iv[NIN];
    auto load_step_e = [&](int t, auto E) {
        constexpr int EE = decltype(E)::value;
        const unsigned ts = (unsigned)(vdir ? (T - 1 - t) : t);
        const unsigned tp = t > 0 ? (vdir ? ts + 1 : ts - 1) : ts;
        const int nvp = t > 0 ? vnv : 0;
#pragma unroll
        for (int k = 0; k < NS; ++k) iv[k] = ld4<EE>(a.S, vS0 + ts * vSs + k * H, vnv);
        iv[NS] = ld4<EE>(a.Y, vY0 + tp * vYs, nvp);
        iv[NS + 1] = ld4<EE>(a.dY, vY0 + ts * vYs, vnv);
        if (LSTM) iv[NS + 2] = ld4<EE>(a.S, vS0 + tp * vSs + 4 * H, nvp);
        if (LN) iv[ILN] = ld4<EE>(a.lnh, vY0 + ts * vYs, vnv);
        if (t == 0) {
            iv[NS] = f32x4{0.f, 0.f, 0.f, 0.f};
            if (LSTM) iv[NS + 2] = f32x4{0.f, 0.f, 0.f, 0.f};
        }
    };
    const LnSlots ls = LN ? ln_slots(a, c, p, wave, lane, T) : LnSlots();
    const float gam = (LN && unit_ok) ? a.ln_gamma[unit] : 0.f;
    const float invH = 1.0f / (float)H, inv_nm1 = 1.0f / (float)(H - 1);
    float accg = 0.f, accb = 0.f;
    pk_f32x2 stn[4];
    long st_off[4];
#pragma unroll
    for (int r = 0; r < 4; ++r) {
        const int row = kq * 4 + r;
        st_off[r] = (LN && row < nrows) ? (long)(n_base + row) * 2 : 0;
        stn[r] = pk_f32x2{0.f, 1.f};
    }
    auto load_stats = [&](int t) {
#pragma unroll
        for (int r = 0; r < 4; ++r) stn[r] = *reinterpret_cast<const pk_f32x2*>(a.lnstat + (long)t * a.R * 2 + st_off[r]);
    };
    if (LN) load_stats(T - 1);
    auto load_step = [&](int t, auto SEC) {
        constexpr int SE = decltype(SEC)::value;
#define PK_LS(E) load_step_e(t, E)
        PK_EDGE_DISPATCH_S(PK_LS);
    };
    auto flush_outputs_e = [&](int tt, auto E) {
        const unsigned ts = (unsigned)(vdir ? (T - 1 - tt) : tt);
#pragma unroll
        for (int g = 0; g < G; ++g)
// ... 194 lines not shown
    if (C >= 8) C -= C % 8;
    {
        static int cap = -1;
        if (cap < 0) {
            const char* e = pk_experiment("rec_clusters");
            cap = e ? atoi(e) : 0;
        }
        const int full = (((R + RMAX - 1) / RMAX) + 7) & ~7;
        const int want = cap > 0 ? cap : full;
        if (want < C) C = want;
    }
    int rpc = (R + C - 1) / C;
    if (rpc > RMAX) rpc = RMAX;
    if (rpc < 1) rpc = 1;
    int need = (R + rpc - 1) / rpc;
    pl.launches = (need + C - 1) / C;
    if (pl.launches == 1) C = need;
    pl.C = C;
    pl.rpc = rpc;
    return 0;
}

static inline int64_t ln_stat_offset(int64_t T, int64_t R, int64_t H) { return (T * R * H + 3) / 4 * 4; }
extern "C" int64_t pk_rec_ln_saved_floats(int T, int B, int bidir, int H) {
    const int64_t R = (int64_t)B * (1 + bidir);
    const int64_t pers = ln_stat_offset(T, R, H) + (int64_t)T * R * 2 + 64;
    const int64_t step = (int64_t)T * R * (H + 2);
    return pers > step ? pers : step;
}
static int64_t ln_exchange_floats(int T, const Plan2& pl) { return (int64_t)(T + 1) * pl.launches * pl.C * 4 * (4 * pl.Pn) * 8; }
int64_t pk_rec4f_ln_work_floats(int T, int B, int bidir, int H);
extern "C" int64_t pk_rec_ln_work_floats(int T, int B, int bidir, int H) {
    Plan2 pl;
    if (T <= 0 || B <= 0 || H <= 0 || H > KPAD || pk_rec2_make_plan(B * (1 + bidir), H, pl) != 0) return 0;
    const int64_t ncg = (int64_t)pl.launches * pl.C;
    const int64_t gen2 = ln_exchange_floats(T, pl) + 2 * ncg * KPAD + pk_bn_partial_floats(ncg, KPAD) + 256;
    const int64_t gen4 = pk_rec4f_ln_work_floats(T, B, bidir, H);
    return gen2 > gen4 ? gen2 : gen4;
}
int pk_rec2_ln_setup(hipStream_t st, R2Args& a, const Plan2& pl, const PkLnHost* ln, bool backward) {
    a.ln_gamma = a.ln_beta = nullptr;
    a.lnh = a.lnstat = a.lnx = a.lnpart = nullptr;
    a.ln_eps = 0.f; a.ln_cg0 = 0; a.ln_ncg = 0;
    if (ln == nullptr) return 0;
    PK_REQUIRE(ln->gamma && ln->LNS && ln->lnwork && (backward ? (ln->dgamma && ln->dbeta) : ln->beta != nullptr),
               "persistent recurrence with per-step LayerNorm: gamma / beta / LNS / scratch pointers missing");
    PK_REQUIRE(a.H > 1, "per-step LayerNorm needs H > 1");
    const int64_t xf = ln_exchange_floats(a.T, pl);
    PK_REQUIRE((double)xf * 4.0 < 4.0e9, "per-step LayerNorm: the row-statistics exchange exceeds the 4 GB buffer-descriptor range");
    PK_REQUIRE((((uintptr_t)ln->LNS | (uintptr_t)ln->lnwork) & 15) == 0, "per-step LayerNorm: LNS / scratch must be 16-byte aligned");
    a.ln_gamma = ln->gamma; a.ln_beta = ln->beta; a.ln_eps = ln->eps;
    a.lnh = ln->LNS;
    a.lnstat = ln->LNS + ln_stat_offset(a.T, a.R, a.H);
    a.lnx = ln->lnwork;
    a.lnpart = ln->lnwork + xf;
    a.ln_ncg = pl.launches * pl.C;
    PK_CHECK_HIP(hipMemsetAsync(a.lnx, 0xFF, (size_t)xf * 4, st));
    if (backward) PK_CHECK_HIP(hipMemsetAsync(a.lnpart, 0, (size_t)2 * a.ln_ncg * KPAD * 4, st));
    return 0;
}
int pk_rec2_ln_finish(hipStream_t st, const R2Args& a, const PkLnHost* ln) {
    if (ln == nullptr) return 0;
    float* part = a.lnpart + (size_t)2 * a.ln_ncg * KPAD;
    int rc = pk_colsum((void*)st, a.lnpart, nullptr, KPAD, a.ln_ncg, a.H, part, ln->dgamma);
    if (rc) return rc;
    return pk_colsum((void*)st, a.lnpart + (size_t)a.ln_ncg * KPAD, nullptr, KPAD, a.ln_ncg, a.H, part, ln->dbeta);
}

int pk_rec2_check(const char* who, int cell_ok, int cell, int T, int B, int bidir, int H) {
    PK_REQUIRE(cell_ok, "%s: cell %d is not covered by this entry point", who, cell);
    PK_REQUIRE(T > 0 && B > 0 && H > 0 && H <= KPAD && (bidir == 0 || bidir == 1), "%s: bad geometry T=%d B=%d H=%d (H <= %d)",
               who, T, B, H, KPAD);
    return 0;
}

static int default_poll_delay(bool backward, int cell) {
    static int env[2] = {-2, -2};
    int& e = env[backward ? 1 : 0];
    if (e == -2) {
        const char* v = pk_experiment(backward ? "poll_delay_bwd" : "poll_delay_fwd");
        e = v ? atoi(v) : -1;
    }
    if (e >= 0) return e;
    if (backward && cell == PK_CELL_LSTM) return 0;
    return 2;
}

int pk_rec2_host_setup(R2Args& a, bool backward, int cell) {
    int rc = ensure_err2();
    if (rc) return rc;
    a.err = g2_err_dev; a.spin_limit = 400000; a.trace = g2_trace; a.xcd_tab = g2_xcd_tab; a.force_safe = g2_force_safe;
    a.trash = g2_trash; a.poll_delay = g2_poll_delay >= 0 ? g2_poll_delay : default_poll_delay(backward, cell);
    a.helper_delay = 0;
    a.empty_step = g2_empty_step;
    a.self_fill = 0;
    {
        static int fl = -1;
        if (fl < 0) {
            const char* e = pk_experiment("rec_flush_late");
            fl = e ? atoi(e) : 0;
        }
        a.flush_late = fl;
    }
    return 0;
}
int pk_rec2_check_residency(const void* kernel, int threads, size_t lds, int grid, const char* who) {
    struct Entry { const void* k; size_t lds; int threads; int cap; };
    static Entry cache[64];
    static int n_cache = 0;
    int cap = -1;
    for (int i = 0; i < n_cache; ++i)
        if (cache[i].k == kernel && cache[i].lds == lds && cache[i].threads == threads) cap = cache[i].cap;
    if (cap < 0) {
        int per_cu = 0;
        PK_CHECK_HIP(hipOccupancyMaxActiveBlocksPerMultiprocessor(&per_cu, kernel, threads, lds));
        cap = per_cu * pk_num_cu();
        if (n_cache < 64) cache[n_cache++] = Entry{kernel, lds, threads, cap};
    }
    PK_REQUIRE(grid <= cap, "%s: a grid of %d workgroups cannot be co-resident on this device (%d fit): the persistent "
               "recurrence would dead-lock into spin time-outs", who, grid, cap);
    return 0;
}

int pk_rec2_reset_handshake(hipStream_t st, R2Args& a) {
    static std::atomic<unsigned> gen{0};
    hipStreamCaptureStatus cs = hipStreamCaptureStatusNone;
    if (hipStreamIsCapturing(st, &cs) != hipSuccess) cs = hipStreamCaptureStatusNone;
    unsigned g = gen.fetch_add(1u) + 1u;
    if (g >= 0x0FFFFFEFu) {
        PK_REQUIRE(cs == hipStreamCaptureStatusNone, "persistent recurrence: the handshake generation wrapped inside a stream "
                   "capture (2^28 launches): end the capture, launch once eagerly, capture again");
        PK_CHECK_HIP(hipDeviceSynchronize());
        PK_CHECK_HIP(hipMemset(g2_xcd_tab, 0xFF, XCD_TAB_BYTES));
        PK_CHECK_HIP(hipDeviceSynchronize());
        gen.store(1u);
        g = 1u;
    }
    if (cs != hipStreamCaptureStatusNone) PK_CHECK_HIP(hipMemsetAsync(g2_xcd_tab, 0xFF, XCD_TAB_BYTES, st));
    a.hs_gen = g;
    return 0;
}

extern "C" int pk_rec_self_fill(int cell) {
    (void)cell;
    return 1;
}

extern "C" int pk_rec_plan_cus(int R, int H) {
    Plan2 pl;
    if (R <= 0 || H <= 0 || H > KPAD || pk_rec2_make_plan(R, H, pl) != 0) return 0;
    return pl.C * pl.Pn;
}

extern "C" void pk_persist2_set_mode(int force_safe) { g2_force_safe = force_safe ? 1 : 0; }
extern "C" void pk_persist2_set_poll_delay(int units) { g2_poll_delay = units; }
extern "C" void pk_persist2_set_trace(void* dev_buf) { g2_trace = (unsigned long long*)dev_buf; }
extern "C" void pk_persist2_set_empty_step(int on) { g2_empty_step = on; }
extern "C" unsigned pk_persist2_error_count(void) { return g2_err_host ? *g2_err_host : 0u; }
extern "C" void pk_persist2_error_reset(void) {
    if (g2_err_host) *g2_err_host = 0u;
}

typedef void (*Rec2Kernel)(R2Args);
inline int act_slot(int act) { return act == PK_ACT_RELU ? 0 : act == PK_ACT_TANH ? 1 : 2; }
template <int CELL>
Rec2Kernel pick_fwd(int act) {
    return act == PK_ACT_RELU ? rec2_fwd_kernel<CELL, PK_ACT_RELU, false>
         : act == PK_ACT_TANH ? rec2_fwd_kernel<CELL, PK_ACT_TANH, false> : rec2_fwd_kernel<CELL, -1, false>;
}
template <int CELL>
Rec2Kernel pick_fwd_nosave(int act) {
    return act == PK_ACT_RELU ? rec2_fwd_kernel<CELL, PK_ACT_RELU, false, false, true>
         : act == PK_ACT_TANH ? rec2_fwd_kernel<CELL, PK_ACT_TANH, false, false, true> : rec2_fwd_kernel<CELL, -1, false, false, true>;
}
template <int CELL>
Rec2Kernel pick_bwd(int act) {
    return act == PK_ACT_RELU ? rec2_bwd_kernel<CELL, PK_ACT_RELU, false>
         : act == PK_ACT_TANH ? rec2_bwd_kernel<CELL, PK_ACT_TANH, false> : rec2_bwd_kernel<CELL, -1, false>;
}
inline bool traced(int cell, int act) { return g2_trace != nullptr && cell == PK_CELL_LIGRU && act == PK_ACT_RELU; }
inline Rec2Kernel pick_fwd_ln(int cell) {
    return cell == PK_CELL_LIGRU ? rec2_fwd_kernel<PK_CELL_LIGRU, -1, false, true>
         : cell == PK_CELL_RNN ? rec2_fwd_kernel<PK_CELL_RNN, -1, false, true> : rec2_fwd_kernel<PK_CELL_LSTM, -1, false, true>;
}
inline Rec2Kernel pick_bwd_ln(int cell) {
    return cell == PK_CELL_LIGRU ? rec2_bwd_kernel<PK_CELL_LIGRU, -1, false, true>
         : cell == PK_CELL_RNN ? rec2_bwd_kernel<PK_CELL_RNN, -1, false, true> : rec2_bwd_kernel<PK_CELL_LSTM, -1, false, true>;
}
inline Rec2Kernel pick_fwd(int cell, int act) {
    if (traced(cell, act)) return rec2_fwd_kernel<PK_CELL_LIGRU, PK_ACT_RELU, true>;
    return cell == PK_CELL_LIGRU ? pick_fwd<PK_CELL_LIGRU>(act) : cell == PK_CELL_RNN ? pick_fwd<PK_CELL_RNN>(act) : pick_fwd<PK_CELL_LSTM>(act);
}
inline Rec2Kernel pick_bwd(int cell, int act) {
    if (traced(cell, act)) return rec2_bwd_kernel<PK_CELL_LIGRU, PK_ACT_RELU, true>;
    return cell == PK_CELL_LIGRU ? pick_bwd<PK_CELL_LIGRU>(act) : cell == PK_CELL_RNN ? pick_bwd<PK_CELL_RNN>(act) : pick_bwd<PK_CELL_LSTM>(act);
}

static int rec_fwd_bf16_impl(void* stream, int cell, int act, int T, int B, int bidir, int H, const float* P,
                             const float* pscale, const float* pshift, const float* U, const float* mask,
                             float mask_scalar, float* Y, float* S, uint16_t* Yb, int64_t y_pitch, int prefilled,
                             const PkLnHost* ln) {
    int rc = pk_rec2_check("pk_rec_fwd_bf16", 1, cell, T, B, bidir, H);
    if (rc) return rc;
    PK_REQUIRE(S != nullptr || (ln == nullptr && !traced(cell, act)), "pk_rec_fwd_bf16: S may be null only without per-step LayerNorm");
    PK_REQUIRE(Y != nullptr || S == nullptr, "pk_rec_fwd_bf16: Y may be null only together with S");
    hipStream_t st = pk_stream(stream);
    const int ndir = 1 + bidir, R = B * ndir, Hp = (H + 7) & ~7;
    PK_REQUIRE(y_pitch >= (int64_t)ndir * Hp && (y_pitch % 8) == 0 && ((uintptr_t)Yb & 15) == 0,
               "pk_rec_fwd_bf16: Yb pitch must be a multiple of 8 and hold %d x %d elements", ndir, Hp);
    PK_REQUIRE((double)T * B * y_pitch * 2.0 < 4.0e9, "pk_rec_fwd_bf16: exchange buffer exceeds the 4 GB buffer-descriptor range");
    Plan2 pl;
    rc = pk_rec2_make_plan(R, H, pl);
    if (rc) return rc;
    R2Args a;
    a.T = T; a.B = B; a.R = R; a.H = H; a.Hp = Hp; a.YH = ndir * H; a.act = act;
    a.C = pl.C; a.Pn = pl.Pn; a.rpc = pl.rpc; a.row0 = 0;
    a.P = P; a.pscale = pscale; a.pshift = pshift; a.U = U; a.mask = mask; a.mask_scalar = mask_scalar;
    a.Y = Y; a.S = S; a.Yb = (unsigned short*)Yb; a.Xb = nullptr; a.Ypitch = (int)y_pitch;
    a.dY = nullptr; a.dP2 = nullptr; a.dGb = nullptr; a.Gpitch = 0;
    rc = pk_rec2_host_setup(a, false, cell);
    if (rc) return rc;
    const bool lstm8 = cell == PK_CELL_LSTM && pk_rec2l_enabled();
    a.self_fill = prefilled == 2 ? 1 : 0;
    if (prefilled != 1 && !a.self_fill) PK_CHECK_HIP(hipMemsetAsync(Yb, 0xFF, (size_t)T * B * y_pitch * 2, st));
    rc = pk_rec2_ln_setup(st, a, pl, ln, false);
    if (rc) return rc;
    if (lstm8 && !ln) return pk_rec2l_launch(st, a, pl, act, false);
    if (!ln && pk_rec3_covers(cell, 0)) return pk_rec3_launch(st, a, pl, cell, act, false, traced(cell, act));
    const int G = pk_cell_gates(cell);
    const size_t lds = 2 * (size_t)RMAX * pk_r2_lda_bf16(KPAD) * 2 + 4 * ((size_t)(G + 1 + pk_cell_saved(cell) + (ln ? 1 : 0)) * 1024 + 512) + 16;
    const bool nosave = S == nullptr;
    const Rec2Kernel k = ln ? pick_fwd_ln(cell)
                       : nosave ? (cell == PK_CELL_LIGRU ? pick_fwd_nosave<PK_CELL_LIGRU>(act) : cell == PK_CELL_RNN ? pick_fwd_nosave<PK_CELL_RNN>(act)
                                                                                                                      : pick_fwd_nosave<PK_CELL_LSTM>(act))
                                : pick_fwd(cell, act);
    {
        static size_t granted[3][8] = {{0}, {0}, {0}};
        const int slot = cell == PK_CELL_LIGRU ? 0 : cell == PK_CELL_RNN ? 1 : 2;
        const int as = ln ? 4 : nosave ? 5 + act_slot(act) : traced(cell, act) ? 3 : act_slot(act);
        if (granted[slot][as] < lds) {
            PK_CHECK_HIP(hipFuncSetAttribute((const void*)k, hipFuncAttributeMaxDynamicSharedMemorySize, (int)lds));
            granted[slot][as] = lds;
        }
    }
    for (int l = 0; l < pl.launches; ++l) {
        a.row0 = l * pl.C * pl.rpc;
        a.ln_cg0 = l * pl.C;
        rc = pk_rec2_reset_handshake(st, a);
        if (rc) return rc;
        dim3 grid(pl.C * pl.Pn), block(256);
        rc = pk_rec2_check_residency((const void*)k, 256, lds, pl.C * pl.Pn, "pk_rec_fwd_bf16");
        if (rc) return rc;
        const int help = ln ? 0 : pk_rec_helper_wanted(false, pl.launches, cell);
        if (help && (rc = pk_rec_helper_fork(st)) != 0) return rc;
        hipLaunchKernelGGL(k, grid, block, lds, st, a);
        PK_LAUNCH_CHECK();
        if (help && (rc = pk_rec_helper_launch(st, a, pl, G, pk_cell_saved(cell), false, true, help)) != 0) return rc;
    }
    return 0;
}
extern "C" int pk_rec_fwd_bf16(void* stream, int cell, int act, int T, int B, int bidir, int H, const float* P,
                               const float* pscale, const float* pshift, const float* U, const float* mask,
                               float mask_scalar, float* Y, float* S, uint16_t* Yb, int64_t y_pitch, int prefilled) {
    return rec_fwd_bf16_impl(stream, cell, act, T, B, bidir, H, P, pscale, pshift, U, mask, mask_scalar, Y, S, Yb, y_pitch,
                             prefilled, nullptr);
}
extern "C" int pk_rec_fwd_bf16_ln(void* stream, int cell, int act, int T, int B, int bidir, int H, const float* P,
                                  const float* pscale, const float* pshift, const float* U, const float* mask,
                                  float mask_scalar, const float* ln_gamma, const float* ln_beta, float ln_eps, float* Y,
                                  float* S, float* LNS, uint16_t* Yb, int64_t y_pitch, int prefilled, float* lnwork) {
    PK_REQUIRE(ln_gamma && ln_beta && LNS && lnwork, "pk_rec_fwd_bf16_ln: null LayerNorm argument");
    const PkLnHost ln = {ln_gamma, ln_beta, ln_eps, LNS, lnwork, nullptr, nullptr};
    return rec_fwd_bf16_impl(stream, cell, act, T, B, bidir, H, P, pscale, pshift, U, mask, mask_scalar, Y, S, Yb, y_pitch,
                             prefilled, &ln);
}

static int rec_bwd_bf16_impl(void* stream, int cell, int act, int T, int B, int bidir, int H, const float* U,
                             const float* mask, float mask_scalar, const float* Y, const float* S, const float* dY,
                             float* dP2, uint16_t* dGb, int64_t g_pitch, int prefilled, const PkLnHost* ln) {
    int rc = pk_rec2_check("pk_rec_bwd_bf16", 1, cell, T, B, bidir, H);
    if (rc) return rc;
    hipStream_t st = pk_stream(stream);
    const int ndir = 1 + bidir, R = B * ndir, Hp = (H + 7) & ~7, G = pk_cell_gates(cell);
    PK_REQUIRE(g_pitch >= (int64_t)G * Hp && (g_pitch % 8) == 0 && ((uintptr_t)dGb & 15) == 0,
               "pk_rec_bwd_bf16: dGb pitch must be a multiple of 8 and hold %d x %d elements", G, Hp);
    PK_REQUIRE((double)ndir * T * B * g_pitch * 2.0 < 4.0e9, "pk_rec_bwd_bf16: exchange buffer exceeds the 4 GB buffer-descriptor range");
    Plan2 pl;
    rc = pk_rec2_make_plan(R, H, pl);
    if (rc) return rc;
    R2Args a;
    a.T = T; a.B = B; a.R = R; a.H = H; a.Hp = Hp; a.YH = ndir * H; a.act = act;
    a.C = pl.C; a.Pn = pl.Pn; a.rpc = pl.rpc; a.row0 = 0;
    a.P = nullptr; a.pscale = nullptr; a.pshift = nullptr; a.U = U; a.mask = mask; a.mask_scalar = mask_scalar;
    a.Y = const_cast<float*>(Y); a.S = const_cast<float*>(S); a.Yb = nullptr; a.Xb = nullptr; a.Ypitch = 0;
    a.dY = dY; a.dP2 = dP2; a.dGb = (unsigned short*)dGb; a.Gpitch = (int)g_pitch;
    rc = pk_rec2_host_setup(a, true, cell);
    if (rc) return rc;
    const bool lstm8 = cell == PK_CELL_LSTM && pk_rec2l_enabled();
    a.self_fill = prefilled == 2 ? 1 : 0;
    if (prefilled != 1 && !a.self_fill) PK_CHECK_HIP(hipMemsetAsync(dGb, 0xFF, (size_t)ndir * T * B * g_pitch * 2, st));
    rc = pk_rec2_ln_setup(st, a, pl, ln, true);
    if (rc) return rc;
    if (lstm8 && !ln) return pk_rec2l_launch(st, a, pl, act, true);
    if (!ln && pk_rec3_covers(cell, 1)) return pk_rec3_launch(st, a, pl, cell, act, true, traced(cell, act));
    const size_t atile = (size_t)RMAX * pk_r2_lda_bf16(G * KPAD) * 2;
    const int nin = pk_cell_saved(cell) + 2 + (cell == PK_CELL_LSTM ? 1 : 0) + (ln ? 1 : 0);
    const size_t lds = (2 * atile > 96 * 1024 ? 1 : 2) * atile + 4 * ((size_t)(nin + G) * 1024 + (size_t)G * 512) + 16;
    const Rec2Kernel k = ln ? pick_bwd_ln(cell) : pick_bwd(cell, act);
    {
        static size_t granted[3][5] = {{0, 0, 0, 0, 0}, {0, 0, 0, 0, 0}, {0, 0, 0, 0, 0}};
        const int slot = cell == PK_CELL_LIGRU ? 0 : cell == PK_CELL_RNN ? 1 : 2;
        const int as = ln ? 4 : traced(cell, act) ? 3 : act_slot(act);
        if (granted[slot][as] < lds) {
            PK_CHECK_HIP(hipFuncSetAttribute((const void*)k, hipFuncAttributeMaxDynamicSharedMemorySize, (int)lds));
            granted[slot][as] = lds;
        }
    }
    for (int l = 0; l < pl.launches; ++l) {
        a.row0 = l * pl.C * pl.rpc;
        a.ln_cg0 = l * pl.C;
        rc = pk_rec2_reset_handshake(st, a);
        if (rc) return rc;
        dim3 grid(pl.C * pl.Pn), block(256);
        rc = pk_rec2_check_residency((const void*)k, 256, lds, pl.C * pl.Pn, "pk_rec_bwd_bf16");
        if (rc) return rc;
        const int help = ln ? 0 : pk_rec_helper_wanted(true, pl.launches, cell);
        if (help && (rc = pk_rec_helper_fork(st)) != 0) return rc;
        hipLaunchKernelGGL(k, grid, block, lds, st, a);
        PK_LAUNCH_CHECK();
        if (help && (rc = pk_rec_helper_launch(st, a, pl, G, pk_cell_saved(cell), true, true, help)) != 0) return rc;
    }
    return pk_rec2_ln_finish(st, a, ln);
}
extern "C" int pk_rec_bwd_bf16(void* stream, int cell, int act, int T, int B, int bidir, int H, const float* U,
                               const float* mask, float mask_scalar, const float* Y, const float* S, const float* dY,
                               float* dP2, uint16_t* dGb, int64_t g_pitch, int prefilled) {
    return rec_bwd_bf16_impl(stream, cell, act, T, B, bidir, H, U, mask, mask_scalar, Y, S, dY, dP2, dGb, g_pitch, prefilled,
                             nullptr);
}
extern "C" int pk_rec_bwd_bf16_ln(void* stream, int cell, int act, int T, int B, int bidir, int H, const float* U,
                                  const float* mask, float mask_scalar, const float* ln_gamma, float ln_eps, const float* Y,
                                  const float* S, const float* LNS, const float* dY, float* dP2, uint16_t* dGb,
                                  int64_t g_pitch, int prefilled, float* lnwork, float* dln_gamma, float* dln_beta) {
    PK_REQUIRE(ln_gamma && LNS && lnwork && dln_gamma && dln_beta, "pk_rec_bwd_bf16_ln: null LayerNorm argument");
    const PkLnHost ln = {ln_gamma, nullptr, ln_eps, const_cast<float*>(LNS), lnwork, dln_gamma, dln_beta};
    return rec_bwd_bf16_impl(stream, cell, act, T, B, bidir, H, U, mask, mask_scalar, Y, S, dY, dP2, dGb, g_pitch, prefilled,
                             &ln);
}
```

pytorch-kaldi_amd/functional.py:

```python
import ctypes
import os
import weakref

import torch

from . import _lib

PREC = {"fp32": 0, "bf16": 1}
ACT = {"linear": 0, "relu": 1, "tanh": 2, "sigmoid": 3, "leaky_relu": 4, "elu": 5}
CELL = {"liGRU": 0, "RNN": 1, "LSTM": 2, "GRU": 3, "minimalGRU": 4}
REC_STEPWISE, REC_PERSISTENT = 0, 1


class _Settings:

    def __init__(self):
        self.precision = os.environ.get("PK_PRECISION", "fp32")
        self.rec_algo = os.environ.get("PK_REC_ALGO", "auto")
        self.mask_rng = os.environ.get("PK_MASK_RNG", "device")
        assert self.mask_rng in ("reference", "reference_host", "device"), self.mask_rng
        self.wgrad_side = _lib.experiment("wgrad_side", "1") != "0"
        self.self_fill = _lib.experiment("rec_self_fill", "1") != "0"
        self.side_late = _lib.experiment("side_late", "1") != "0"
        self.side_cus = _lib.experiment("side_cus", "0") != "0"
# ... 208 lines not shown
            raise _lib.PkError("forced dropout mask %s for a %s tensor" % (tuple(m.shape), tuple(like.shape)))
        return m.to(device=like.device, dtype=torch.float32) / (1.0 - p)
    if _Ahead.queue:
        shape, q, m = _Ahead.queue.pop(0)
        if shape == tuple(like.shape) and q == p and m.device == like.device:
            return m
        _Ahead.queue = []
    return torch.empty_like(like).bernoulli_(1.0 - p).div_(1.0 - p)


def _p(t):
    return None if t is None else ctypes.c_void_p(t.data_ptr())


def _stream():
    return ctypes.c_void_p(torch.cuda.current_stream().cuda_stream)


def _need_gpu(*ts):
    for t in ts:
        if t is not None and not t.is_cuda:
            raise _lib.PkError("pytorch-kaldi_amd runs on the GPU only (got a %s tensor); there is no CPU fallback. "
                               "Set use_cuda=True in the cfg." % t.device)
        if t is not None and t.dtype != torch.float32:
            raise _lib.PkError("pytorch-kaldi_amd kernels take fp32 tensors (got %s)" % t.dtype)


def _rows2d(x):
    if x.dim() != 2:
        x = x.reshape(-1, x.shape[-1])
    if x.stride(1) != 1 or (x.shape[0] > 1 and x.stride(0) < x.shape[1]):
        x = x.contiguous()
    return x


def _new(*shape, like):
    return torch.empty(*shape, device=like.device, dtype=torch.float32)


def _splitk(out_tiles, K):
    if K < 4096:
        return 1
    slots = int(_lib.experiment("f32_splitk_slots", "1024"))
    s = max(1, slots // max(1, out_tiles))
    return int(min(16, s, max(1, K // 1024)))


def _small_m_splitk(M, N, K):
    if M > 256 or K < 512 or _lib.experiment("f32_small_splitk", "1") == "0":
        return 1
    return int(max(1, min(16, 512 // max(1, _tiles(M, N)), K // 64)))


def gemm(M, N, K, A, a_rs, a_cs, B, b_rs, b_cs, C, ldc, alpha=1.0, beta=0.0, bias=None, splitk=1, prec=None):
    lib = _lib.load()
    ws = None
    if splitk == 1 and a_cs == 1 and (prec or settings.precision) == "fp32":
        splitk = _small_m_splitk(M, N, K)
    if splitk > 1:
        ws = torch.empty(splitk * M * N, device=C.device, dtype=torch.float32)
    rc = lib.pk_gemm(_stream(), PREC[prec or settings.precision], M, N, K, alpha, _p(A), a_rs, a_cs, _p(B), b_rs, b_cs,
                     beta, _p(C), ldc, _p(bias), splitk, _p(ws))
    _lib.check(rc, "pk_gemm")
    return C


def _tiles(M, N):
    return ((M + 127) // 128) * ((N + 127) // 128)


def _tiles_bf(M, N):
    return (M, N)


def _up(n, m):
    return (n + m - 1) // m * m


def weight_bf16(w):
    sh = getattr(w, "_pk_shadow", None)
    if sh is not None:
        view, version, alive, flat_version = sh
        if alive() is not None:
            owner = getattr(w, "_pk_owner", None)
            owner = owner() if owner is not None else None
            fv = owner.flat._version if owner is not None else flat_version
            if w._version == version and fv == flat_version:
                return view
            cvt_bf16(w.detach(), out=view)
            w._pk_shadow = (view, w._version, alive, fv)
            return view
    owner = getattr(w, "_pk_owner", None)
    owner = owner() if owner is not None else None
    if owner is not None and w.is_contiguous():
        owner.want_shadow(w)
    return cvt_bf16(w.contiguous())


def cvt_bf16(x2, nseg=1, seglen=None, segpad=None, out=None):
    lib = _lib.load()
    rows, cols = x2.shape
    if seglen is None:
        nseg, seglen = 1, cols
    if segpad is None:
        segpad = _up(seglen, 8)
    assert nseg * seglen == cols and x2.stride(1) == 1
    pitch = _up(nseg * segpad, 64)
    if out is None:
        out = torch.empty(rows, pitch, device=x2.device, dtype=torch.bfloat16)
    assert tuple(out.shape) == (rows, pitch) and out.dtype == torch.bfloat16 and out.is_contiguous()
    _lib.check(lib.pk_cvt_bf16(_stream(), _p(x2), x2.stride(0), rows, nseg, seglen, segpad, _p(out), pitch),
               "pk_cvt_bf16")
    return out


_SMALL_SPLITK = _lib.experiment("small_splitk", "1") != "0"


def gemm_bf16(M, N, K, A, lda, a_kc, B, ldb, b_kc, C, ldc, alpha=1.0, beta=0.0, bias=None, splitk=1):
    lib = _lib.load()
    ws = None
    if splitk == 1 and a_kc and M <= 128 and _SMALL_SPLITK:
        splitk = int(lib.pk_gemm_bf16_small_splitk(M, N, K))
    if splitk > 1:
        ws = torch.empty(splitk * M * N, device=C.device, dtype=torch.float32)

    def ptr(t):
        if isinstance(t, tuple):
            return ctypes.c_void_p(t[0].data_ptr() + 2 * t[1])
        return ctypes.c_void_p(t.data_ptr())

    rc = lib.pk_gemm_bf16(_stream(), M, N, K, alpha, ptr(A), lda, int(a_kc), ptr(B), ldb, int(b_kc), beta, _p(C), ldc,
                          _p(bias), splitk, _p(ws))
    _lib.check(rc, "pk_gemm_bf16")
    return C


def gemm_bf16_bn_stats(M, N, K, A, lda, a_kc, B, ldb, b_kc, C, ldc, bias=None, gates=None):
    lib = _lib.load()

    def done(mean, var):
        return (mean, var) if gates is None else (mean, var) + tuple(bn_finalize_gates(mean, var, *gates))

    if _lib.experiment("gemm_stats", "1") == "0":
        gemm_bf16(M, N, K, A, lda, a_kc, B, ldb, b_kc, C, ldc, bias=bias)
        return done(*bn_stats(C if ldc == N else C.as_strided((M, N), (ldc, 1))))
    stats = torch.empty(int(lib.pk_gemm_bf16_stats_floats(M, N)), device=C.device, dtype=torch.float32)
    rb = ctypes.c_int(0)
    rc = lib.pk_gemm_bf16_stats(_stream(), M, N, K, 1.0, _p(A), lda, int(a_kc), _p(B), ldb, int(b_kc), _p(C), ldc, _p(bias),
                                _p(stats), ctypes.byref(rb))
    _lib.check(rc, "pk_gemm_bf16_stats")
    if rb.value == 0:
        return done(*bn_stats(C if ldc == N else C.as_strided((M, N), (ldc, 1))))
    mean, var = torch.empty(N, device=C.device), torch.empty(N, device=C.device)
    if gates is not None:
        gamma, beta, eps, H, rms, rvs, nbs, momentum, count = gates
        G = len(rms)
        scale, shift = torch.empty_like(mean), torch.empty_like(mean)
        arr = lambda ts: (ctypes.c_void_p * G)(*[t.data_ptr() for t in ts])
        _lib.check(lib.pk_bn_stats_merge_finalize_gates(_stream(), _p(stats), rb.value, G, H, _p(mean), _p(var), _p(gamma),
                                                        _p(beta), eps, _p(scale), _p(shift), arr(rms), arr(rvs), arr(nbs),
                                                        momentum, float(count)), "pk_bn_stats_merge_finalize_gates")
        return mean, var, scale, shift
    _lib.check(lib.pk_bn_stats_merge(_stream(), _p(stats), rb.value, N, _p(mean), _p(var)), "pk_bn_stats_merge")
    return mean, var


def _splitk_bf(out_tiles, K):
    M, N = out_tiles
    return int(_lib.load().pk_gemm_bf16_auto_splitk_cus(int(M), int(N), int(K), int(_SideCus.cus)))


class _SideCus:
    cus = 0


def _sized_for(cus, fn):
    def run():
        old, _SideCus.cus = _SideCus.cus, cus
        try:
            fn()
        finally:
            _SideCus.cus = old
    return run


def bf16_mode():
    return settings.precision == "bf16"



class _Side:
    stream = None
    pending = False
    listener = None
    deferred = []


def set_side_listener(fn):
    _Side.listener = fn


def side_targets_ok(params):
    return bf16_mode() and side_targets_any_ok(params)


def side_targets_any_ok(params):
    if not bf16_mode() and _lib.experiment("f32_wgrad_side", "1") == "0":
        return False
    return (settings.wgrad_side and params is not None and len(params) > 0
            and all(getattr(q, "_pk_flat", False) and q.grad is not None and q.requires_grad for q in params))


class accumulating_backward:
    depth = 0

    def __enter__(self):
        accumulating_backward.depth += 1
        return self

    def __exit__(self, *exc):
        accumulating_backward.depth -= 1
        return False


def direct_grads_ok(params):
    return (accumulating_backward.depth > 0 and _Side.listener is None and _lib.experiment("direct_grads", "1") != "0"
            and torch.is_grad_enabled() is False and side_targets_ok(params))


def direct_affine_ok(params):
    return (accumulating_backward.depth > 0 and _Side.listener is None and _lib.experiment("direct_grads", "1") != "0"
            and torch.is_grad_enabled() and side_targets_ok(params))


_DEBUG_SKIP_SIDE = _lib.experiment("debug_skip_side", "0") == "1"


def _make_side_stream():
    return torch.cuda.Stream()


def side_launch(fn, keep, params=None, defer=False):
    if defer and settings.side_late and _lib.experiment("side_defer_heads", "1") != "0":
        _Side.deferred.append((fn, keep, params))
        _Side.pending = True
        return
    flush_deferred_side()
    main = torch.cuda.current_stream()
    if _Side.stream is None:
        _Side.stream = _make_side_stream()
    side = _Side.stream
    side.wait_stream(main)
    with torch.cuda.stream(side):
        if not _DEBUG_SKIP_SIDE:
            fn()
    for t in keep:
        if t is not None:
            t.record_stream(side)
    _Side.pending = True
    if _Side.listener is not None and params:
        _Side.listener(params)


def flush_deferred_side():
    if _Side.deferred:
        items, _Side.deferred = _Side.deferred, []
        for fn, keep, params in items:
            side_launch(fn, keep, params)


def join_side():
    flush_deferred_side()
    if _Side.pending:
        if _Side.stream is not None:
            torch.cuda.current_stream().wait_stream(_Side.stream)
        _Side.pending = False


def adjacent_view(ts):
    if not ts:
        return None
    base = ts[0]
    if len(ts) == 1:
        return base.detach() if base.is_contiguous() else None
    ptr, rows = base.data_ptr(), 0
    for t in ts:
        if (not t.is_contiguous() or t.dtype != base.dtype or t.shape[1:] != base.shape[1:] or t.data_ptr() != ptr
                or t.untyped_storage().data_ptr() != base.untyped_storage().data_ptr()):
            return None
        ptr += t.numel() * t.element_size()
        rows += t.shape[0]
    if base.data_ptr() % 16 != 0:
        return None
    return base.detach().as_strided((rows,) + tuple(base.shape[1:]), base.stride())


def _accumulate_rows(params, rows):
    with torch.no_grad():
        gview = adjacent_view([q.grad for q in params])
        whole = adjacent_view(list(rows)) if gview is not None else None
        if whole is not None and whole.shape == gview.shape:
            gview.add_(whole)
            return
        for q, r in zip(params, rows):
            q.grad.add_(r)

_XB_LAST = None


def _cvt_bf16_shared(x2):
    global _XB_LAST
    key = (x2.data_ptr(), tuple(x2.shape), tuple(x2.stride()), x2._version)
    if _XB_LAST is not None and _XB_LAST[1] == key and x2.numel() >= (1 << 20):
        return _XB_LAST[2]
    xb = cvt_bf16(x2)
    _XB_LAST = (x2, key, xb) if x2.numel() >= (1 << 20) else None
    return xb
# ... 976 lines not shown
            dlg, dlb = _new(H, like=dY), _new(H, like=dY)
        dGb = None
        if ctx.Yb is not None:
            Hp = _up(H, 8)
            dGb = torch.empty(ndir * TB, _up(G * Hp, 64), device=dY.device, dtype=torch.bfloat16)
            if ctx.Xb is not None:
                lnwork = _new(n_lnwork, like=dY)
                rc = lib.pk_rec2p_bwd_bf16_ln(_stream(), CELL[cell], ACT[act], T, B, int(bidir), H, _p(Ucat), _p(mask),
                                              float(mask_scalar), _p(ln_gamma), LN_EPS, _p(Y), _p(S), _p(LNS), _p(dY),
                                              _p(dGb), dGb.shape[1], 2 if settings.self_fill else 0, _p(lnwork),
                                              _p(dlg), _p(dlb))
                flat = dP2.view(ndir * TB, GH)
                for g_ in range(G):
                    flat[:, g_ * H:(g_ + 1) * H].copy_(dGb[:, g_ * Hp:g_ * Hp + H])
            elif ln_gamma is not None:
                lnwork = _new(n_lnwork, like=dY)
                rc = lib.pk_rec_bwd_bf16_ln(_stream(), CELL[cell], ACT[act], T, B, int(bidir), H, _p(Ucat), _p(mask),
                                            float(mask_scalar), _p(ln_gamma), LN_EPS, _p(Y), _p(S), _p(LNS), _p(dY),
                                            _p(dP2), _p(dGb), dGb.shape[1], 2 if settings.self_fill else 0, _p(lnwork),
                                            _p(dlg), _p(dlb))
            else:
                rc = lib.pk_rec_bwd_bf16(_stream(), CELL[cell], ACT[act], T, B, int(bidir), H, _p(Ucat), _p(mask),
                                         float(mask_scalar), _p(Y), _p(S), _p(dY), _p(dP2), _p(dGb), dGb.shape[1],
                                         2 if settings.self_fill else 0)
            _lib.check(rc, "pk_rec_bwd_bf16")
        else:
            side_u = (not bf) and ctx.side_u and side_targets_any_ok(ctx.uparams)
            flush_deferred_side()
            rc = lib.pk_rec_bwd(_stream(), ctx.algo, ctx.prec, CELL[cell], ACT[act], T, B, int(bidir), H, _p(Ucat),
                                _p(mask), float(mask_scalar), _p(ln_gamma), _p(Y), _p(S), _p(LNS), _p(dY), _p(dP2),
                                None if (bf or ctx.side_u) else _p(dU), _p(dlg), _p(dlb), _p(work))
            _lib.check(rc, "pk_rec_bwd")
            if ctx.side_u and not side_u:
                raise _lib.PkError("recurrent layer: the flat gradient buffer the weights' gradients were to be added to is gone "
                                   "between forward and backward (optim.FlatParams.zero_grad() re-aliases it)")
        NS_ = lib.pk_rec_num_saved(CELL[cell])

        def do_dU_f32():
            gview = adjacent_view([q.grad for q in ctx.uparams])
            if gview is not None:
                _deferred_dU_f32(cell, T, B, ndir, H, G, NS_, Y, S, dP2, gview, True)
            else:
                _deferred_dU_f32(cell, T, B, ndir, H, G, NS_, Y, S, dP2, dU, False)
                _accumulate_rows(ctx.uparams, [dU[g * H:(g + 1) * H] for g in range(G)])

        if bf:
            _deferred_dU_bf16(lib, cell, T, B, ndir, H, G, Y, S, dP2, dU, ctx.Yb, dGb, ctx.Xb)
            ctx.Yb = ctx.Xb = None
        g1 = dP2[0]
        g2 = dP2[1] if bidir else None
        dgamma = dbeta = dbias = None
        ldp = GH
        if use_bn and not bf and GH % 4 != 0:
            ldp = _up(GH, 4)
        dPraw = _new(TB, ldp, like=dY)
        if use_bn:
            part = _new(int(lib.pk_bn_partial_floats(TB, GH)), like=dY)
            sum_g, sum_gx = _new(GH, like=dY), _new(GH, like=dY)
            _lib.check(lib.pk_bn_bwd_reduce(_stream(), _p(g1), _p(g2), GH, _p(P), GH, TB, GH, _p(mean), _p(var), eps,
                                            _p(part), _p(sum_g), _p(sum_gx)), "pk_bn_bwd_reduce")
            dgamma, dbeta = sum_gx, sum_g
            if training:
                _lib.check(lib.pk_bn_bwd_apply(_stream(), _p(g1), _p(g2), GH, _p(P), GH, TB, GH, _p(mean), _p(var), eps,
                                               _p(gamma), _p(sum_g), _p(sum_gx), float(TB), _p(dPraw), ldp),
                           "pk_bn_bwd_apply")
            else:
                gs = g1
                if g2 is not None:
                    gs = _new(TB, GH, like=dY)
                    _lib.check(lib.pk_add(_stream(), _p(g1), _p(g2), TB * GH, _p(gs)), "pk_add")
                zero = torch.zeros_like(pscale)
                _lib.check(lib.pk_affine_act_fwd(_stream(), _p(gs), GH, TB, GH, _p(pscale), _p(zero), 0, None,
                                                 _p(dPraw), ldp), "pk_affine_act_fwd")
        else:
            if g2 is not None:
                _lib.check(lib.pk_add(_stream(), _p(g1), _p(g2), TB * GH, _p(dPraw)), "pk_add")
            else:
                dPraw = g1
            if ctx.has_bias:
                dbias = colsum(dPraw)
        dx = dW = None
        dW = _new(GH, D, like=dY)
        if bf:
            xb, Wb = x2, Wcat
            dPb = cvt_bf16(dPraw)
            if ctx.needs_input_grad[0]:
                dx = _new(TB, D, like=dY)
                gemm_bf16(TB, D, GH, dPb, dPb.shape[1], 1, Wb, Wb.shape[1], 0, dx, D)
                dx = dx.view(T, B, D)
            gemm_bf16(GH, D, TB, dPb, dPb.shape[1], 0, xb, xb.shape[1], 0, dW, D, splitk=_splitk_bf(_tiles_bf(GH, D), TB))
            return dx, dW, dbias, dU, dgamma, dbeta, None, None, None, dlg, dlb, None
        if ctx.needs_input_grad[0]:
            dx = _new(TB, D, like=dY)
            gemm(TB, D, GH, dPraw, ldp, 1, Wcat, D, 1, dx, D)
            dx = dx.view(T, B, D)
        side_w = ctx.side_w and side_targets_any_ok(ctx.wparams)
        if ctx.side_w and not side_w:
            raise _lib.PkError("recurrent layer: the flat gradient buffer of the input weights is gone between forward and backward")
        if ctx.side_u:
            side_launch(do_dU_f32, (Y, S, dP2, dU), ctx.uparams)

        def do_dW_f32():
            gview = adjacent_view([q.grad for q in ctx.wparams])
            sk = _splitk(_tiles(GH, D), TB)
            if gview is not None:
                gemm(GH, D, TB, dPraw, 1, ldp, x2, x2.stride(0), 1, gview, D, beta=1.0, splitk=sk)
            else:
                gemm(GH, D, TB, dPraw, 1, ldp, x2, x2.stride(0), 1, dW, D, splitk=sk)
                _accumulate_rows(ctx.wparams, [dW[g * H:(g + 1) * H] for g in range(G)])

        if side_w:
            side_launch(do_dW_f32, (dPraw, x2, dW), ctx.wparams)
        else:
            gemm(GH, D, TB, dPraw, 1, ldp, x2, x2.stride(0), 1, dW, D, splitk=_splitk(_tiles(GH, D), TB))
        return (dx, None if side_w else dW, dbias, None if ctx.side_u else dU, dgamma, dbeta, None, None, None, dlg, dlb, None)


def perf_path_ok(cell, H, use_ln, use_bn, training):
    if not bf16_mode() or settings.rec_algo == "stepwise":
        return False
    if cell not in ("liGRU", "RNN", "LSTM", "GRU", "minimalGRU") or H > 576 or use_ln:
        return False
    return training or not use_bn or not torch.is_grad_enabled()


class _Prefill:
    stream = None

    def __init__(self):
        self.done = 0

    def start(self, *bufs):
        if not settings.wgrad_side:
            return
        main = torch.cuda.current_stream()
        if _Prefill.stream is None:
            _Prefill.stream = torch.cuda.Stream()
        st = _Prefill.stream
        st.wait_stream(main)
        with torch.cuda.stream(st):
            for b in bufs:
                if b is not None:
                    b.view(torch.int16).fill_(-1)
        for b in bufs:
            if b is not None:
                b.record_stream(st)
        self.done = 1

    def wait(self):
        if self.done:
            torch.cuda.current_stream().wait_stream(_Prefill.stream)


class RecLayerPerfFn(torch.autograd.Function):

    @staticmethod
    def forward(ctx, x, xb_in, Wcat, bcat, Ucat, gamma, beta, running_mean, running_var, mask, cfg, edge=None):
        ctx.set_materialize_grads(False)
        _need_gpu(x, Wcat, bcat, Ucat, gamma, beta, mask)
        lib = _lib.load()
        cell, act, H, bidir, use_bn, training, eps, momentum, mask_scalar, xseg = cfg[:10]
        ctx.wparams, ctx.uparams = (cfg[10], cfg[11]) if len(cfg) > 10 else (None, None)
        ctx.side_w, ctx.side_u = (bool(cfg[12]), bool(cfg[13])) if len(cfg) > 13 else (False, False)
        ctx.affine = cfg[15] if len(cfg) > 15 else None
        T, B, D = x.shape
        G = lib.pk_rec_num_gates(CELL[cell])
        NS = lib.pk_rec_num_saved(CELL[cell])
        ndir = 2 if bidir else 1
        TB, GH = T * B, G * H
        Wcat = Wcat.contiguous()
        Ucat = Ucat.contiguous()
        if xb_in is None:
            xseg = None
            xb, Wb, K = cvt_bf16(_rows2d(x)), cvt_bf16(Wcat), D
        else:
            nseg, seglen, segpad = xseg
            assert nseg * seglen == D and xb_in.shape[0] == TB
            xb, Wb, K = xb_in, cvt_bf16(Wcat, nseg, seglen, segpad), nseg * segpad
            assert Wb.shape[1] == xb.shape[1]
        Hp = _up(H, 8)
        Yb = torch.empty(TB, _up(ndir * Hp, 64), device=x.device, dtype=torch.bfloat16)
        two_phase = cell in ("GRU", "minimalGRU")
        self_fill = settings.self_fill and lib.pk_rec_self_fill(CELL[cell]) == 1
        dGb = None
        if any(ctx.needs_input_grad) and not self_fill:
            dGb = torch.empty(ndir * TB, _up(G * Hp, 64), device=x.device, dtype=torch.bfloat16)
        Xb = torch.empty_like(Yb) if two_phase else None
        fill = _Prefill()
        if not self_fill:
            fill.start(Yb, Xb, dGb)
        P = _new(TB, GH, like=Wcat)
        mean = var = None
        bn_bufs = cfg[14] if len(cfg) > 14 else None
        pscale = pshift = None
        if use_bn and training and bn_bufs is not None:
            mean, var, pscale, pshift = gemm_bf16_bn_stats(TB, GH, K, xb, xb.shape[1], 1, Wb, Wb.shape[1], 1, P, GH, gates=(
                gamma, beta, eps, H, bn_bufs[0], bn_bufs[1], bn_bufs[2], momentum, ndir * TB))
        elif use_bn and training:
            mean, var = gemm_bf16_bn_stats(TB, GH, K, xb, xb.shape[1], 1, Wb, Wb.shape[1], 1, P, GH)
        else:
            gemm_bf16(TB, GH, K, xb, xb.shape[1], 1, Wb, Wb.shape[1], 1, P, GH)
        if use_bn:
            if pscale is not None:
                pass
            elif training:
                pscale, pshift = bn_finalize(mean, var, gamma, beta, eps, running_mean, running_var, momentum, ndir * TB)
            else:
                mean, var = running_mean, running_var
                pscale, pshift = bn_finalize(mean, var, gamma, beta, eps)
        else:
            pscale = torch.ones(GH, device=x.device)
            pshift = bcat.contiguous() if bcat is not None else torch.zeros(GH, device=x.device)
        infer = not any(ctx.needs_input_grad) and _Kinks.queue is None and _lib.experiment("fwd_nosave", "1") != "0"
        keep_y = bool(cfg[16]) if len(cfg) > 16 else True
        Y = _new(T, B, ndir * H, like=Wcat)
        S = None if infer else _new(ndir, TB, NS * H, like=Wcat)
        Yarg = Y if (keep_y or not infer) else None
        _lib.raise_if_persist_failed()
        fill.wait()
        if two_phase:
            rc = lib.pk_rec2p_fwd_bf16(_stream(), CELL[cell], ACT[act], T, B, int(bidir), H, _p(P), _p(pscale),
                                       _p(pshift), _p(Ucat), _p(mask), float(mask_scalar), _p(Yarg), _p(S), _p(Yb), _p(Xb),
                                       Yb.shape[1], 2 if self_fill else fill.done)
            _lib.check(rc, "pk_rec2p_fwd_bf16")
        else:
            rc = lib.pk_rec_fwd_bf16(_stream(), CELL[cell], ACT[act], T, B, int(bidir), H, _p(P), _p(pscale), _p(pshift),
                                     _p(Ucat), _p(mask), float(mask_scalar), _p(Yarg), _p(S), _p(Yb), Yb.shape[1],
                                     2 if self_fill else fill.done)
            _lib.check(rc, "pk_rec_fwd_bf16")
        if S is not None:
            _force_kinks(S, cell, T, B, ndir, H)
        ctx.self_fill = self_fill
        ctx.dGb = dGb if fill.done else None
        ctx.Xb = Xb
        ctx.save_for_backward(xb, Wb, Wcat, Ucat, P, mean, var, gamma, mask, Y, S, Yb)
        ctx.cfg = cfg[:9] + (xseg,)
        ctx.in_shape = x.shape
        ctx.has_bias = bcat is not None
        if use_bn and training:
            ctx.mark_non_differentiable(mean, var, Yb)
            return Y, mean, var, Yb
        ctx.mark_non_differentiable(Yb)
        return Y, None, None, Yb

    @staticmethod
    def backward(ctx, dY, _dm, _dv, _dyb):
        if dY is None:
            return (None,) * 12
        lib = _lib.load()
        xb, Wb, Wcat, Ucat, P, mean, var, gamma, mask, Y, S, Yb = ctx.saved_tensors
        cell, act, H, bidir, use_bn, training, eps, momentum, mask_scalar, xseg = ctx.cfg
        if use_bn and not training:
            raise _lib.PkError("perf-mode recurrent layer: backward through frozen BatchNorm statistics is not covered")
        T, B, D = ctx.in_shape
        G = lib.pk_rec_num_gates(CELL[cell])
        ndir = 2 if bidir else 1
        TB, GH = T * B, G * H
        Hp = _up(H, 8)
        dY = dY.contiguous()
        dGb, prefilled = ctx.dGb, 1
        ctx.dGb = None
        if dGb is None:
            dGb = torch.empty(ndir * TB, _up(G * Hp, 64), device=dY.device, dtype=torch.bfloat16)
            prefilled = 2 if ctx.self_fill else 0
        Gp = dGb.shape[1]
        flush_deferred_side()
        if ctx.Xb is not None:
            rc = lib.pk_rec2p_bwd_bf16(_stream(), CELL[cell], ACT[act], T, B, int(bidir), H, _p(Ucat), _p(mask),
                                       float(mask_scalar), _p(Y), _p(S), _p(dY), _p(dGb), Gp, prefilled)
            _lib.check(rc, "pk_rec2p_bwd_bf16")
        else:
            rc = lib.pk_rec_bwd_bf16(_stream(), CELL[cell], ACT[act], T, B, int(bidir), H, _p(Ucat), _p(mask),
                                     float(mask_scalar), _p(Y), _p(S), _p(dY), None, _p(dGb), Gp, prefilled)
            _lib.check(rc, "pk_rec_bwd_bf16")
        side_u, side_w = ctx.side_u, ctx.side_w
        Xb = ctx.Xb
        ctx.Xb = None
        dU = _new(GH, H, like=dY)

        def do_dU():
            _deferred_dU_bf16(lib, cell, T, B, ndir, H, G, Y, S, None, dU, Yb, dGb, Xb)
            if side_u:
                _accumulate_rows(ctx.uparams, [dU[g * H:(g + 1) * H] for g in range(G)])

        late = settings.side_late and bool(ctx.needs_input_grad[0])
        if side_u and not late:
            side_launch(do_dU, (Y, S, Yb, dGb, Xb, dU), ctx.uparams)
        elif not side_u:
            do_dU()
        dPb = torch.empty(TB, _up(GH, 64), device=dY.device, dtype=torch.bfloat16)
        part = _new(int(lib.pk_bn_partial_floats(TB, GH)), like=dY)
        sum_g = _new(GH, like=dY)
        sum_gx = _new(GH, like=dY) if use_bn else None
        g1 = ctypes.c_void_p(dGb.data_ptr() + 2 * TB * Gp) if bidir else None
        acc_g = acc_b = None
        if use_bn and ctx.affine is not None:
            acc_g = adjacent_view([q.grad for q in ctx.affine[0]])
            acc_b = adjacent_view([q.grad for q in ctx.affine[1]])
            if acc_g is None or acc_b is None:
                raise _lib.PkError("perf-mode recurrent layer: the BatchNorm gradients left the flat buffer between forward "
                                   "and backward (optim.FlatParams.zero_grad() re-aliases them)")
        rc = lib.pk_bn_bwd_bf16(_stream(), _p(dGb), g1, Gp, G, H, _p(P), GH, TB, _p(mean) if use_bn else None,
                                _p(var) if use_bn else None, eps, _p(gamma) if use_bn else None, float(TB), _p(part),
                                _p(sum_g), _p(sum_gx), _p(dPb), dPb.shape[1], _p(acc_b), _p(acc_g))
        _lib.check(rc, "pk_bn_bwd_bf16")
        dgamma = dbeta = dbias = None
        if use_bn and acc_g is None:
            dgamma, dbeta = sum_gx, sum_g
        elif not use_bn and ctx.has_bias:
            dbias = sum_g
        Kx = D if xseg is None else xseg[0] * xseg[2]
        dWp = _new(GH, Kx, like=dY)
        dW = None

        def do_dW():
            nonlocal dW
            gview = adjacent_view([q.grad for q in ctx.wparams]) if side_w else None
            sk = _splitk_bf(_tiles_bf(GH, Kx), TB)
            if gview is not None and xseg is None:
                gemm_bf16(GH, Kx, TB, dPb, dPb.shape[1], 0, xb, xb.shape[1], 0, gview, Kx, beta=1.0, splitk=sk)
                return
            gemm_bf16(GH, Kx, TB, dPb, dPb.shape[1], 0, xb, xb.shape[1], 0, dWp, Kx, splitk=sk)
            if gview is not None:
                nseg, seglen, segpad = xseg
                with torch.no_grad():
                    for s_ in range(nseg):
                        gview[:, s_ * seglen:(s_ + 1) * seglen].add_(dWp[:, s_ * segpad:s_ * segpad + seglen])
                return
            if xseg is None:
                dW = dWp
            else:
                nseg, seglen, segpad = xseg
                dW = torch.cat([dWp[:, s_ * segpad:s_ * segpad + seglen] for s_ in range(nseg)], 1)
            if side_w:
                _accumulate_rows(ctx.wparams, [dW[g * H:(g + 1) * H] for g in range(G)])

        if side_w and not late:
            side_launch(do_dW, (dPb, xb, dWp), ctx.wparams)
        dx = None
        if ctx.needs_input_grad[0]:
            Wb2 = Wb if xseg is None else cvt_bf16(Wcat)
            dx = _new(TB, D, like=dY)
            gemm_bf16(TB, D, GH, dPb, dPb.shape[1], 1, Wb2, Wb2.shape[1], 0, dx, D)
            dx = dx.view(T, B, D)
        if late:
            free = 0
            if settings.side_cus:
                held = int(lib.pk_rec_plan_cus(ndir * B, H))
                free = max(int(lib.pk_num_cu()) - held, 0) if held > 0 else 0
            if side_u:
                side_launch(_sized_for(free, do_dU), (Y, S, Yb, dGb, Xb, dU), ctx.uparams)
            if side_w:
                side_launch(_sized_for(free, do_dW), (dPb, xb, dWp), ctx.wparams)
        if not side_w:
            do_dW()
        return dx, None, (None if side_w else dW), dbias, (None if side_u else dU), dgamma, dbeta, None, None, None, None, None


CONV_BF16_DEFAULT = "1"


def conv_bf16_mode():
    return os.environ.get("PK_CONV_BF16", CONV_BF16_DEFAULT)


class ConvPoolFn(torch.autograd.Function):
    @staticmethod
    def forward(ctx, x, w, bias, pool):
        _need_gpu(x, w, bias)
        lib = _lib.load()
        x = x.contiguous()
        w = w.contiguous()
        B, Cin, L = x.shape
        Cout, _, K = w.shape
        Lp = (L - K + 1) // pool
        y = _new(B, Cout, Lp, like=x)
        arg = torch.empty(B, Cout, Lp, device=x.device, dtype=torch.int32)
        mode = conv_bf16_mode()
        ctx.conv_bf = (bf16_mode() and mode in ("1", "2") and (Cin >= 8 or mode == "2")
                       and lib.pk_conv_bf16_covers(Cin, Cout, K, pool) == 1)
        if ctx.conv_bf:
            work = _new(int(lib.pk_conv_bf16_work_floats(B, Cin, L, Cout, K, pool, 0)), like=x)
# ... 50 lines not shown
```

pytorch-kaldi_amd/nn.py:

```python
import math
import os
import weakref

import numpy as np
import torch
import torch.nn as nn

from . import functional as F_
from ._lib import PkError


def strtobool(s):
    s = str(s).strip().lower()
    if s in ("y", "yes", "t", "true", "on", "1"):
        return 1
    if s in ("n", "no", "f", "false", "off", "0"):
        return 0
    raise ValueError("invalid truth value %r" % (s,))


def _opt(options, key):
    try:
        return options[key]
    except KeyError:
# ... 250 lines not shown
            return rd["masks"][i]
        if rd is not None:
            self._rewind(rd["state0"], self._cur[:-1])
        m = self._draw(*want)
        if i == n_lay - 1 and self._done is None and self._ahead is None and self._alone(self):
            self._start(self._cur)
        return m

    def drain(self):
        self._join()
        if self._ahead is not None and torch.equal(torch.get_rng_state(), self._ahead["state1"]):
            torch.set_rng_state(self._ahead["state0"])
        self._ahead = self._ready = None


def drain_mask_prefetch():
    for pf in list(_MaskPrefetcher.live):
        pf.drain()
    _MaskPrefetcher.live = weakref.WeakSet()
    F_._RefRng.sync_back()


class _Recurrent(nn.Module):

    KIND = None

    def __init__(self, options, inp_dim):
        super().__init__()
        pre, gates, w_order, u_order, bn_order = _REC_SPEC[self.KIND]
        self._pre, self._gates = pre, gates
        self.input_dim = inp_dim
        lay = _ints(_opt(options, pre + "_lay"))
        setattr(self, pre + "_lay", lay)
        self._lay = lay
        self._drop = _floats(_opt(options, pre + "_drop"))
        self._use_bn = _bools(_opt(options, pre + "_use_batchnorm"))
        self._use_ln = _bools(_opt(options, pre + "_use_laynorm"))
        self._use_ln_inp = strtobool(_opt(options, pre + "_use_laynorm_inp"))
        self._use_bn_inp = strtobool(_opt(options, pre + "_use_batchnorm_inp"))
        self._orthinit = strtobool(_opt(options, pre + "_orthinit"))
        self._act = str(_opt(options, pre + "_act")).split(",")
        self.bidir = strtobool(_opt(options, pre + "_bidir"))
        self.use_cuda = strtobool(_opt(options, "use_cuda"))
        self.to_do = _opt(options, "to_do")
        self.test_flag = self.to_do != "train"
        for a in self._act:
            if a not in F_.ACT:
                raise PkError("%s: activation %r is not supported inside the recurrence" % (self.KIND, a))
        for name in [n for pair in zip(w_order, u_order) for n in pair] + ["ln"] + bn_order + ["act"]:
            setattr(self, name, nn.ModuleList([]))
        if self._use_ln_inp:
            self.ln0 = LayerNorm(self.input_dim)
        if self._use_bn_inp:
            self.bn0 = nn.BatchNorm1d(self.input_dim, momentum=0.05)
        self._n_lay = len(lay)
        cur = self.input_dim
        for i in range(self._n_lay):
            self.act.append(act_fun(self._act[i]))
            add_bias = not (self._use_ln[i] or self._use_bn[i])
            for name in w_order:
                getattr(self, name).append(nn.Linear(cur, lay[i], bias=add_bias))
            for name in u_order:
                getattr(self, name).append(nn.Linear(lay[i], lay[i], bias=False))
            if self._orthinit:
                for name in u_order:
                    nn.init.orthogonal_(getattr(self, name)[i].weight)
            for name in bn_order:
                getattr(self, name).append(nn.BatchNorm1d(lay[i], momentum=0.05))
            self.ln.append(LayerNorm(lay[i]))
            cur = 2 * lay[i] if self.bidir else lay[i]
        self.out_dim = lay[-1] + self.bidir * lay[-1]

    def pk_unused_parameters(self):
        out = []
        for i in range(self._n_lay):
            if not self._use_ln[i]:
                out += list(self.ln[i].parameters())
            if not self._use_bn[i]:
                for (_, _, b) in self._gates:
                    out += list(getattr(self, b)[i].parameters())
        return out

    def _drop_mask(self, i, batch, device):
        p = self._drop[i]
        if self.test_flag:
            return None, 1.0 - p
        rows = 2 * batch if self.bidir else batch
        if F_.settings.mask_rng == "device":
            H = self._lay[i]
            if (self._n_lay > 1 and len(set(self._lay)) == 1 and len(set(self._drop)) == 1 and (rows * H) % 4 == 0
                    and F_._lib.experiment("mask_one_draw", "1") != "0"):
                if i == 0:
                    self._mask_all = torch.empty(self._n_lay, rows, H, device=device).bernoulli_(1 - p)
                m_all = getattr(self, "_mask_all", None)
                if m_all is not None and m_all.shape[1] == rows and m_all.device == device:
                    if i == self._n_lay - 1:
                        self._mask_all = None
                    return m_all[i], 1.0
            return torch.empty(rows, H, device=device).bernoulli_(1 - p), 1.0
        if F_.settings.mask_rng == "reference":
            if i == 0:
                self._ref_masks = [(rows, device)] + F_._RefRng.masks(
                    [(rows, self._lay[j], self._drop[j]) for j in range(self._n_lay)], device)
            pend = getattr(self, "_ref_masks", None)
            if pend is None or pend[0] != (rows, device) or pend[1 + i] is None:
                return F_.ref_rng_mask(rows, self._lay[i], p, device), 1.0
            entry, pend[1 + i] = pend[1 + i], None
            if i == self._n_lay - 1:
                self._ref_masks = None
            return entry, 1.0
        if getattr(self, "_prefetch", None) is None or self._prefetch not in _MaskPrefetcher.live:
            self._prefetch = _MaskPrefetcher()
        m = self._prefetch.get(i, self._n_lay, rows, self._lay[i], p)
        return self._to_device_async(i, m, device), 1.0

    def _to_device_async(self, i, m, device):
        if device.type != "cuda":
            return m.to(device)
        if not hasattr(self, "_pin"):
            self._pin, self._pin_ev, self._pin_k = {}, {}, {}
        k = self._pin_k.get(i, 0)
        key = (i, k, tuple(m.shape))
        if key not in self._pin:
            self._pin[key] = torch.empty(m.shape, dtype=m.dtype).pin_memory()
            self._pin_ev[key] = None
        if self._pin_ev[key] is not None:
            self._pin_ev[key].synchronize()
        self._pin[key].copy_(m)
        d = self._pin[key].to(device, non_blocking=True)
        ev = torch.cuda.Event()
        ev.record()
        self._pin_ev[key] = ev
        self._pin_k[i] = 1 - k
        return d

    def pk_flat_groups(self):
        out = []
        if self._use_ln_inp:
            out.append(list(self.ln0.parameters()))
        if self._use_bn_inp:
            out.append(list(self.bn0.parameters()))
        for i in range(self._n_lay):
            Ws = [getattr(self, w)[i] for (w, _, _) in self._gates]
            Us = [getattr(self, u)[i] for (_, u, _) in self._gates]
            bns = [getattr(self, b)[i] for (_, _, b) in self._gates]
            out.append([m.weight for m in Ws])
            out.append([m.weight for m in Us])
            out.append([m.bias for m in Ws if m.bias is not None])
            out.append([b.weight for b in bns])
            out.append([b.bias for b in bns])
            out.append(list(self.ln[i].parameters()))
        return out

    def forward(self, x, drop_masks=None):
        if not x.is_cuda:
            raise PkError("pytorch-kaldi_amd.nn.%s runs on the GPU only: set use_cuda=True" % self.KIND)
        if self._use_ln_inp:
            x = self.ln0(x)
        if self._use_bn_inp:
            T, B, D = x.shape
            x = F_.norm_act_drop(x.reshape(T * B, D), self.bn0, True, self.training, "linear").view(T, B, D)
        masks = scalars = None
        if drop_masks is not None:
            masks = [m if m.numel() > 1 else None for m in drop_masks]
            scalars = [1.0 if m.numel() > 1 else float(m) for m in drop_masks]
            masks = [m.to(x.device).float().contiguous() if m is not None else None for m in masks]
        batch = x.shape[1]
        xb = xseg = None
        for i in range(self._n_lay):
            mask_i, scalar_i = (masks[i], scalars[i]) if masks is not None else self._drop_mask(i, batch, x.device)
            H = self._lay[i]
            Ws = [getattr(self, w)[i] for (w, _, _) in self._gates]
            Us = [getattr(self, u)[i] for (_, u, _) in self._gates]
            Wcat = Ucat = None
            bcat = None
            if Ws[0].bias is not None:
                bcat = torch.cat([m.bias for m in Ws], 0) if len(Ws) > 1 else Ws[0].bias
            gamma = beta = rmean = rvar = None
            use_bn = bool(self._use_bn[i])
            bns = [getattr(self, b)[i] for (_, _, b) in self._gates]
            affine = edge_t = None
            if use_bn:
                gps, bps = [b.weight for b in bns], [b.bias for b in bns]
                if (self.training and F_.direct_affine_ok(gps + bps)
                        and F_.perf_path_ok(self.KIND, H, bool(self._use_ln[i]), use_bn, self.training)):
                    gamma, beta = F_.adjacent_view([q.detach() for q in gps]), F_.adjacent_view([q.detach() for q in bps])
                    if (gamma is not None and beta is not None and F_.adjacent_view([q.grad for q in gps]) is not None
                            and F_.adjacent_view([q.grad for q in bps]) is not None):
                        affine, edge_t = (gps, bps), gps[0]
                if affine is None:
                    gamma = torch.cat(gps, 0)
                    beta = torch.cat(bps, 0)
                if not self.training:
                    rmean = torch.cat([b.running_mean for b in bns], 0)
                    rvar = torch.cat([b.running_var for b in bns], 0)
            if use_bn and self.training and x.shape[0] * x.shape[1] * (2 if self.bidir else 1) <= 1:
                raise ValueError("Expected more than 1 value per channel when training, got input size %s"
                                 % (tuple(x.shape),))
            cfg = (self.KIND, self._act[i], H, bool(self.bidir), use_bn, self.training, 1e-5, 0.05, scalar_i)
            if F_.perf_path_ok(self.KIND, H, bool(self._use_ln[i]), use_bn, self.training):
                wps, ups = [m.weight for m in Ws], [m.weight for m in Us]
                edge = torch.is_grad_enabled() and (use_bn or bcat is not None or x.requires_grad)
                side_w = edge and F_.side_targets_ok(wps)
                side_u = edge and F_.side_targets_ok(ups)
                if side_w or not torch.is_grad_enabled():
                    Wcat = F_.adjacent_view([w.detach() for w in wps])
                if side_u or not torch.is_grad_enabled():
                    Ucat = F_.adjacent_view([u.detach() for u in ups])
                if Wcat is None:
                    Wcat = torch.cat(wps, 0) if len(wps) > 1 else wps[0]
                if Ucat is None:
                    Ucat = torch.cat(ups, 0) if len(ups) > 1 else ups[0]
                keep_y = torch.is_grad_enabled() or i == self._n_lay - 1
                stats_in_kernel = use_bn and self.training
                bn_bufs = ([b.running_mean for b in bns], [b.running_var for b in bns],
                           [b.num_batches_tracked for b in bns]) if stats_in_kernel else None
                y, bmean, bvar, xb = F_.RecLayerPerfFn.apply(x, xb, Wcat.detach() if side_w else Wcat, bcat,
                                                           Ucat.detach() if side_u else Ucat, gamma, beta, rmean, rvar,
                                                           mask_i, cfg + (xseg, wps, ups, side_w, side_u, bn_bufs, affine,
                                                                          keep_y), edge_t)
                xseg = (2 if self.bidir else 1, H, (H + 7) // 8 * 8)
                if stats_in_kernel:
                    x = y
                    continue
            else:
                wps, ups = [m.weight for m in Ws], [m.weight for m in Us]
                edge = (not F_.bf16_mode()) and torch.is_grad_enabled() and (use_bn or bcat is not None or x.requires_grad)
                side_w = edge and F_.side_targets_any_ok(wps)
                side_u = edge and F_.side_targets_any_ok(ups)
                if side_w:
                    Wcat = F_.adjacent_view([w.detach() for w in wps])
                    if Wcat is None:
                        Wcat = torch.cat([w.detach() for w in wps], 0)
                else:
                    Wcat = torch.cat(wps, 0) if len(wps) > 1 else wps[0]
                if side_u:
                    Ucat = F_.adjacent_view([u.detach() for u in ups])
                    if Ucat is None:
                        Ucat = torch.cat([u.detach() for u in ups], 0)
                else:
                    Ucat = torch.cat(ups, 0) if len(ups) > 1 else ups[0]
                lng = self.ln[i].gamma if self._use_ln[i] else None
                lnb = self.ln[i].beta if self._use_ln[i] else None
                y, bmean, bvar = F_.RecLayerFn.apply(x, Wcat, bcat, Ucat, gamma, beta, rmean, rvar, mask_i, lng, lnb,
                                                     cfg + (wps, ups, side_w, side_u))
                xb = xseg = None
            if use_bn and self.training:
                n = x.shape[0] * x.shape[1] * (2 if self.bidir else 1)
                with torch.no_grad():
                    means, vars_ = [b.running_mean for b in bns], [b.running_var for b in bns]
                    torch._foreach_mul_(means + vars_, 0.95)
                    torch._foreach_add_(means, [bmean[k * H:(k + 1) * H] for k in range(len(bns))], alpha=0.05)
                    torch._foreach_add_(vars_, [bvar[k * H:(k + 1) * H] for k in range(len(bns))], alpha=0.05 * n / (n - 1))
                    torch._foreach_add_([b.num_batches_tracked for b in bns], 1)
            x = y
        if xb is not None:
            x._pk_twin = (xb, xseg, x._version)
        return x


class liGRU(_Recurrent):
    KIND = "liGRU"


class minimalGRU(_Recurrent):
    KIND = "minimalGRU"


class GRU(_Recurrent):
    KIND = "GRU"


class LSTM(_Recurrent):
    KIND = "LSTM"


class RNN(_Recurrent):
    KIND = "RNN"


class SincConv(nn.Module):

    @staticmethod
    def to_mel(hz):
        return 2595 * np.log10(1 + hz / 700)

    @staticmethod
    def to_hz(mel):
        return 700 * (10 ** (mel / 2595) - 1)

    def __init__(self, in_channels, out_channels, kernel_size, sample_rate=16000, min_low_hz=50, min_band_hz=50):
        super().__init__()
        if in_channels != 1:
            raise ValueError("SincConv only support one input channel (here, in_channels = {%i})" % (in_channels))
        self.out_channels = out_channels
        self.kernel_size = kernel_size + 1 if kernel_size % 2 == 0 else kernel_size
        self.sample_rate, self.min_low_hz, self.min_band_hz = sample_rate, min_low_hz, min_band_hz
        low_hz = 30
        high_hz = self.sample_rate / 2 - (self.min_low_hz + self.min_band_hz)
        mel = np.linspace(self.to_mel(low_hz), self.to_mel(high_hz), self.out_channels + 1)
        hz = self.to_hz(mel) / self.sample_rate
        self.low_hz_ = nn.Parameter(torch.Tensor(hz[:-1]).view(-1, 1))
        self.band_hz_ = nn.Parameter(torch.Tensor(np.diff(hz)).view(-1, 1))
        n_lin = torch.linspace(0, self.kernel_size, steps=self.kernel_size)
        self.window_ = 0.54 - 0.46 * torch.cos(2 * math.pi * n_lin / self.kernel_size)
        n = (self.kernel_size - 1) / 2
        self.n_ = torch.arange(-n, n + 1).view(1, -1) / self.sample_rate

    def _sinc(self, v):
        left = v[:, 0:int((v.shape[1] - 1) / 2)]
        yl = torch.sin(left) / left
        return torch.cat([yl, torch.ones([v.shape[0], 1], device=v.device), torch.flip(yl, dims=[1])], dim=1)

    def filters(self):
        dev = self.low_hz_.device
        self.n_ = self.n_.to(dev)
        self.window_ = self.window_.to(dev)
        if self.low_hz_.is_cuda:
            return F_.sinc_bank(self.low_hz_, self.band_hz_, self.n_, self.window_, self.sample_rate,
                                self.min_low_hz / self.sample_rate, self.min_band_hz / self.sample_rate)
        low = self.min_low_hz / self.sample_rate + torch.abs(self.low_hz_)
        high = low + self.min_band_hz / self.sample_rate + torch.abs(self.band_hz_)
        lp1 = 2 * low * self._sinc(2 * math.pi * (low * self.n_) * self.sample_rate)
        lp2 = 2 * high * self._sinc(2 * math.pi * (high * self.n_) * self.sample_rate)
        bp = lp2 - lp1
        mx, _ = torch.max(bp, dim=1, keepdim=True)
        bp = bp / mx
        return (bp * self.window_).view(self.out_channels, 1, self.kernel_size)


class _ConvStack(nn.Module):

    PRE = None

    def __init__(self, options, inp_dim):
        super().__init__()
        p = self.PRE
        self.input_dim = inp_dim
        self._n_filt = _ints(_opt(options, p + "_N_filt"))
        self._len_filt = _ints(_opt(options, p + "_len_filt"))
        self._pool = _ints(_opt(options, p + "_max_pool_len"))
        self._act = str(_opt(options, p + "_act")).split(",")
        self._drop = _floats(_opt(options, p + "_drop"))
        self._use_ln = _bools(_opt(options, p + "_use_laynorm"))
        self._use_bn = _bools(_opt(options, p + "_use_batchnorm"))
        self._use_ln_inp = strtobool(_opt(options, p + "_use_laynorm_inp"))
        self._use_bn_inp = strtobool(_opt(options, p + "_use_batchnorm_inp"))
        self._n_lay = len(self._n_filt)
        if p == "sinc":
            self.sinc_sample_rate = int(_opt(options, "sinc_sample_rate"))
            self.sinc_min_low_hz = int(_opt(options, "sinc_min_low_hz"))
            self.sinc_min_band_hz = int(_opt(options, "sinc_min_band_hz"))
        self.conv = nn.ModuleList([])
        self.bn = nn.ModuleList([])
        self.ln = nn.ModuleList([])
        self.act = nn.ModuleList([])
        self.drop = nn.ModuleList([])
        if self._use_ln_inp:
            self.ln0 = LayerNorm(self.input_dim)
        if self._use_bn_inp:
            self.bn0 = nn.BatchNorm1d([self.input_dim], momentum=0.05)
        cur = self.input_dim
        for i in range(self._n_lay):
            n_filt, len_filt = self._n_filt[i], self._len_filt[i]
            self.drop.append(nn.Dropout(p=self._drop[i]))
            self.act.append(act_fun(self._act[i]))
            pooled = int((cur - len_filt + 1) / self._pool[i])
            self.ln.append(LayerNorm([n_filt, pooled]))
            self.bn.append(nn.BatchNorm1d(n_filt, pooled, momentum=0.05))
            if i == 0:
                if p == "sinc":
                    self.conv.append(SincConv(1, n_filt, len_filt, sample_rate=self.sinc_sample_rate,
                                              min_low_hz=self.sinc_min_low_hz, min_band_hz=self.sinc_min_band_hz))
                else:
                    self.conv.append(nn.Conv1d(1, n_filt, len_filt))
            else:
                self.conv.append(nn.Conv1d(self._n_filt[i - 1], n_filt, len_filt))
            cur = pooled
        self.out_dim = cur * self._n_filt[-1]

    def pk_unused_parameters(self):
        out = []
        for i in range(self._n_lay):
            if not self._use_ln[i]:
                out += list(self.ln[i].parameters())
            if not self._use_bn[i]:
                out += list(self.bn[i].parameters())
        return out

    def _conv_pool(self, i, x):
        c = self.conv[i]
        if isinstance(c, SincConv):
            return F_.conv1d_pool(x, c.filters(), None, self._pool[i])
        return F_.conv1d_pool(x, c.weight, c.bias, self._pool[i])

    def _post(self, i, z, use_bn):
        B, C, L = z.shape
        mask = None
        if self.training and self._drop[i] > 0.0:
# ... 45 lines not shown
```

Before: 3.801 million.

## Stream next layer's input projection GEMM alongside segmented recurrent forward

Splits the liGRU/RNN recurrent forward into time segments and, on a side stream, runs the next layer's bf16 input-projection GEMM with fused BN statistics on row bands of the output as soon as those rows are final. The next layer then reuses the precomputed projection, stats and scale/shift instead of launching its own GEMM. The goal is to overlap the latency-bound recurrence, which leaves compute idle, with the following layer's projection. In exchange it adds extra kernel launches, segment restarts that reload the hidden state from Y, event and stream synchronisation, and contention between the persistent recurrent kernel and the GEMM for CUs.

```diff
diff --git a/include/pk_amd.h b/include/pk_amd.h
--- a/include/pk_amd.h
+++ b/include/pk_amd.h
@@ -46,6 +46,10 @@
 int pk_gemm_bf16_stats(void* stream, int M, int N, int K, float alpha, const uint16_t* A, int64_t lda, int a_kc,
                        const uint16_t* B, int64_t ldb, int b_kc, float* C, int64_t ldc, const float* bias, float* stats,
                        int* row_blocks);
+int pk_gemm_bf16_stats_rows(void* stream, int row0, int rows, int M_total, int N, int K, float alpha, const uint16_t* A,
+                            int64_t lda, int a_kc, const uint16_t* B, int64_t ldb, int b_kc, float* C, int64_t ldc,
+                            const float* bias, float* stats);
+int pk_gemm_bf16_stats_fused(int M, int N);
 int pk_cvt_bf16(void* stream, const float* src, int64_t ld_src, int64_t rows, int nseg, int seglen, int segpad,
                 uint16_t* dst, int64_t ld_dst);
 
@@ -148,6 +152,10 @@
 int pk_rec_bwd_bf16(void* stream, int cell, int act, int T, int B, int bidir, int H, const float* U, const float* mask,
                     float mask_scalar, const float* Y, const float* S, const float* dY, float* dP2, uint16_t* dGb,
                     int64_t g_pitch, int prefilled);
+int pk_rec_fwd_bf16_seg(void* stream, int cell, int act, int T, int B, int bidir, int H, const float* P,
+                        const float* pscale, const float* pshift, const float* U, const float* mask, float mask_scalar,
+                        float* Y, float* S, uint16_t* Yb, int64_t y_pitch, int prefilled, int t_begin, int t_end);
+int pk_proj_stream_plan(int T, int B, int bidir, int ncuts, const int* cuts, int* out_bands);
 int pk_rec_fwd_bf16_ln(void* stream, int cell, int act, int T, int B, int bidir, int H, const float* P,
                        const float* pscale, const float* pshift, const float* U, const float* mask, float mask_scalar,
                        const float* ln_gamma, const float* ln_beta, float ln_eps, float* Y, float* S, float* LNS,
diff --git a/pytorch-kaldi_amd/_lib.py b/pytorch-kaldi_amd/_lib.py
--- a/pytorch-kaldi_amd/_lib.py
+++ b/pytorch-kaldi_amd/_lib.py
@@ -27,6 +27,9 @@
                              c_int, P]),
     "pk_gemm_bf16_stats_floats": (c_int64, [c_int, c_int]),
     "pk_gemm_bf16_stats": (c_int, [P, c_int, c_int, c_int, c_float, P, c_int64, c_int, P, c_int64, c_int, P, c_int64, P, P, P]),
+    "pk_gemm_bf16_stats_fused": (c_int, [c_int, c_int]),
+    "pk_gemm_bf16_stats_rows": (c_int, [P, c_int, c_int, c_int, c_int, c_int, c_float, P, c_int64, c_int, P, c_int64, c_int, P,
+                                        c_int64, P, P]),
     "pk_bn_stats_merge": (c_int, [P, P, c_int, c_int64, P, P]),
     "pk_cvt_bf16": (c_int, [P, P, c_int64, c_int64, c_int, c_int, c_int, P, c_int64]),
     "pk_bn_partial_floats": (c_int64, [c_int64, c_int64]),
@@ -84,6 +87,9 @@
     "pk_rec_plan_cus": (c_int, [c_int, c_int]),
     "pk_gemm_bf16_auto_splitk_cus": (c_int, [c_int, c_int, c_int, c_int]),
     "pk_rec_fwd_bf16": (c_int, [P, c_int, c_int, c_int, c_int, c_int, c_int, P, P, P, P, P, c_float, P, P, P, c_int64, c_int]),
+    "pk_rec_fwd_bf16_seg": (c_int, [P, c_int, c_int, c_int, c_int, c_int, c_int, P, P, P, P, P, c_float, P, P, P, c_int64, c_int,
+                                    c_int, c_int]),
+    "pk_proj_stream_plan": (c_int, [c_int, c_int, c_int, c_int, P, P]),
     "pk_rec_bwd_bf16": (c_int, [P, c_int, c_int, c_int, c_int, c_int, c_int, P, P, c_float, P, P, P, P, P, c_int64, c_int]),
     "pk_rec2p_fwd_bf16_ln": (c_int, [P, c_int, c_int, c_int, c_int, c_int, c_int, P, P, P, P, P, c_float, P, P, c_float, P, P, P,
                                      P, P, c_int64, c_int, P]),
diff --git a/pytorch-kaldi_amd/csrc/pk_gemm_bf16.hip b/pytorch-kaldi_amd/csrc/pk_gemm_bf16.hip
--- a/pytorch-kaldi_amd/csrc/pk_gemm_bf16.hip
+++ b/pytorch-kaldi_amd/csrc/pk_gemm_bf16.hip
@@ -1169,7 +1169,7 @@
 
 static int gemm_bf16_impl(void* stream, int M, int N, int K, float alpha, const uint16_t* A, int64_t lda, int a_kc,
                           const uint16_t* B, int64_t ldb, int b_kc, float beta, float* C, int64_t ldc, const float* bias,
-                          int splitk, float* workspace, float* stats) {
+                          int splitk, float* workspace, float* stats, int tile_as = 0) {
     if (M <= 0 || N <= 0) return 0;
     PK_REQUIRE(K >= 0, "pk_gemm_bf16: negative K");
     PK_REQUIRE((lda % 8) == 0 && (ldb % 8) == 0 && ((uintptr_t)A & 15) == 0 && ((uintptr_t)B & 15) == 0,
@@ -1185,7 +1185,7 @@
     p.A = A; p.lda = lda; p.B = B; p.ldb = ldb;
     p.C = C; p.ldc = ldc; p.bias = bias;
     p.stats = stats;
-    const int tile = gemm_tile_for(M, N, a_kc, b_kc, K);
+    const int tile = tile_as ? tile_as : gemm_tile_for(M, N, a_kc, b_kc, K);
     PK_REQUIRE(stats == nullptr || (tile == 256 && a_kc && b_kc && splitk <= 1 && beta == 0.f), "pk_gemm_bf16_stats: internal: shape not covered");
     p.tiles_m = (M + tile - 1) / tile;
     p.tiles_n = (N + tile - 1) / tile;
@@ -1325,6 +1325,23 @@
     *row_blocks = fused ? (M + 255) / 256 : 0;
     return gemm_bf16_impl(stream, M, N, K, alpha, A, lda, a_kc, B, ldb, b_kc, 0.f, C, ldc, bias, 1, nullptr,
                           fused ? stats : nullptr);
+}
+
+extern "C" int pk_gemm_bf16_stats_fused(int M, int N) { return (M > 0 && N > 0 && gemm_tile_for(M, N, 1, 1) == 256) ? 1 : 0; }
+
+extern "C" int pk_gemm_bf16_stats_rows(void* stream, int row0, int rows, int M_total, int N, int K, float alpha,
+                                       const uint16_t* A, int64_t lda, int a_kc, const uint16_t* B, int64_t ldb, int b_kc,
+                                       float* C, int64_t ldc, const float* bias, float* stats) {
+    PK_REQUIRE(stats != nullptr && A != nullptr && C != nullptr, "pk_gemm_bf16_stats_rows: null argument");
+    PK_REQUIRE(M_total > 0 && N > 0 && K > 0 && row0 >= 0 && rows > 0 && (int64_t)row0 + rows <= M_total,
+               "pk_gemm_bf16_stats_rows: band [%d, %d + %d) outside the %d rows", row0, row0, rows, M_total);
+    PK_REQUIRE((row0 % 256) == 0, "pk_gemm_bf16_stats_rows: the band must start on a 256-row tile (row0 = %d)", row0);
+    PK_REQUIRE((rows % 256) == 0 || row0 + rows == M_total,
+               "pk_gemm_bf16_stats_rows: a band that does not end the matrix must be whole tiles (rows = %d)", rows);
+    PK_REQUIRE(a_kc && b_kc && gemm_tile_for(M_total, N, a_kc, b_kc) == 256,
+               "pk_gemm_bf16_stats_rows: the whole product does not run on the 256-tile");
+    return gemm_bf16_impl(stream, rows, N, K, alpha, A + (int64_t)row0 * lda, lda, a_kc, B, ldb, b_kc, 0.f,
+                          C + (int64_t)row0 * ldc, ldc, bias, 1, nullptr, stats + (int64_t)(row0 / 256) * N * 3, 256);
 }
 
 extern "C" int pk_gemm_bf16_small_splitk(int M, int N, int K) {
diff --git a/pytorch-kaldi_amd/csrc/pk_rec2_common.h b/pytorch-kaldi_amd/csrc/pk_rec2_common.h
--- a/pytorch-kaldi_amd/csrc/pk_rec2_common.h
+++ b/pytorch-kaldi_amd/csrc/pk_rec2_common.h
@@ -42,6 +42,7 @@
     float* lnpart;
     int ln_cg0;
     int ln_ncg;
+    int t_begin, t_end;
 };
 
 struct Plan2 {
diff --git a/pytorch-kaldi_amd/csrc/pk_rec_persist2.hip b/pytorch-kaldi_amd/csrc/pk_rec_persist2.hip
--- a/pytorch-kaldi_amd/csrc/pk_rec_persist2.hip
+++ b/pytorch-kaldi_amd/csrc/pk_rec_persist2.hip
@@ -5,8 +5,9 @@
 
 namespace {
 
-template <int CELL, int ACT, bool TR, bool LN = false, bool NOSAVE = false>
+template <int CELL, int ACT, bool TR, bool LN = false, bool NOSAVE = false, bool SEG = false>
 __global__ __launch_bounds__(256, 1) void rec2_fwd_kernel(R2Args a) {
+    static_assert(!SEG || (!LN && !TR && CELL != PK_CELL_LSTM), "segments: liGRU / RNN without per-step LayerNorm");
     const int act = ACT >= 0 ? ACT : a.act;
     constexpr int G = pk_cell_gates(CELL), NS = pk_cell_saved(CELL);
     constexpr int LDA = pk_r2_lda_bf16(KPAD);
@@ -20,6 +21,7 @@
     const int tid = threadIdx.x, lane = tid & 63, wave = tid >> 6;
     const int c = blockIdx.x % a.C, p = blockIdx.x / a.C;
     const int H = a.H, Hp = a.Hp, B = a.B, T = a.T, GH = G * H;
+    const int t_begin = SEG ? a.t_begin : 0, t_end = SEG ? a.t_end : T;
     const int n_base = a.row0 + c * a.rpc;
     int nrows = a.R - n_base;
     nrows = nrows < a.rpc ? nrows : a.rpc;
@@ -89,6 +91,11 @@
         msk[r] = (a.mask != nullptr && ok) ? a.mask[(long)n * H + unit] : a.mask_scalar;
         hprev[r] = 0.f;
         cprev[r] = 0.f;
+        if (SEG && t_begin > 0 && ok) {
+            const int dir = n >= B ? 1 : 0, b = n - dir * B;
+            const int ts = dir ? (T - t_begin) : (t_begin - 1);
+            hprev[r] = a.Y[((long)ts * B + b) * a.YH + dir * H + unit];
+        }
     }
     const int vrow = lane >> 2, vu0 = ubase + (lane & 3) * 4;
     const int vn = n_base + (vrow < nrows ? vrow : 0);
@@ -146,10 +153,10 @@
             *reinterpret_cast<pk_f32x2*>(st_base + (long)tt * st_step) = st_val;
         }
     };
-#define PK_LP0(E) load_proj(0, E)
+#define PK_LP0(E) load_proj(t_begin, E)
     PK_EDGE_DISPATCH(PK_LP0);
     const u32x4 sentinel = u32x4{0xFFFFFFFFu, 0xFFFFFFFFu, 0xFFFFFFFFu, 0xFFFFFFFFu};
-    if (a.self_fill) {
+    if (a.self_fill && t_begin == 0) {
         for (int tt = 0; tt < PK_R2_FILL_AHEAD && tt < T; ++tt)
             pub_store<false>(rs, pbase + (pk_ok ? (unsigned)(pdir ? (T - 1 - tt) : tt) * TS : 0u), sentinel);
         asm volatile("s_waitcnt vmcnt(0)" ::: "memory");
@@ -161,7 +168,7 @@
     auto run = [&](auto FASTC, auto SEC) {
     const bool fast = decltype(FASTC)::value < 0 ? fast_rt : decltype(FASTC)::value != 0;
     constexpr int SE = decltype(SEC)::value;
-    for (int t = 0; t < T; ++t) {
+    for (int t = t_begin; t < t_end; ++t) {
         const int step_idx = t;
         PK_TRACE(0);
         f32x4 acc[G];
@@ -184,11 +191,11 @@
         if (t > 0) PK_BARRIER_LDS();
         else PK_LDS_ORDER();
         PK_TRACE(2);
-        if (t > 0) {
+        if (t > t_begin) {
 #define PK_FO(E) flush_outputs(t - 1, E)
             PK_EDGE_DISPATCH_S(PK_FO);
         }
-        if (t + 1 < T) {
+        if (t + 1 < t_end) {
 #define PK_LP1(E) load_proj(t + 1, E)
             PK_EDGE_DISPATCH_S(PK_LP1);
         }
@@ -303,7 +310,7 @@
     } else {
         PK_RUN_SPECIALISED(run, fast_rt);
     }
-#define PK_FOL(E) flush_outputs(T - 1, E)
+#define PK_FOL(E) flush_outputs(t_end - 1, E)
     PK_EDGE_DISPATCH(PK_FOL);
 }
 
@@ -804,6 +811,36 @@
     return pl.C * pl.Pn;
 }
 
+extern "C" int pk_proj_stream_plan(int T, int B, int bidir, int ncuts, const int* cuts, int* out_bands) {
+    if (T <= 0 || B <= 0 || ncuts <= 0 || ncuts > 16 || cuts == nullptr || out_bands == nullptr) return 0;
+    const long long TB = (long long)T * B;
+    if (TB < 8 * 256 || TB > 0x7FFFFFFFLL) return 0;
+    for (int k = 0; k < ncuts; ++k) {
+        if (cuts[k] <= (k ? cuts[k - 1] : 0) || cuts[k] >= T) return 0;
+        if (bidir && 2 * (long long)cuts[k] <= T) return 0;
+    }
+    long long lo = 0, hi = 0;
+    bool any = false;
+    for (int k = 0; k < ncuts; ++k) {
+        int* o = out_bands + 4 * k;
+        o[0] = o[1] = o[2] = o[3] = 0;
+        const long long c0 = bidir ? (long long)(T - cuts[k]) * B : 0, c1 = (long long)cuts[k] * B;
+        const long long a0 = (c0 + 255) / 256 * 256, a1 = c1 / 256 * 256;
+        if (a1 <= a0) continue;
+        if (!any) {
+            o[0] = (int)a0; o[1] = (int)(a1 - a0);
+            lo = a0; hi = a1; any = true;
+            continue;
+        }
+        if (a0 < lo) { o[0] = (int)a0; o[1] = (int)(lo - a0); lo = a0; }
+        if (a1 > hi) { o[2] = (int)hi; o[3] = (int)(a1 - hi); hi = a1; }
+    }
+    if (!any) return 0;
+    int* o = out_bands + 4 * ncuts;
+    o[0] = 0; o[1] = (int)lo; o[2] = (int)hi; o[3] = (int)(TB - hi);
+    return ncuts + 1;
+}
+
 extern "C" void pk_persist2_set_mode(int force_safe) { g2_force_safe = force_safe ? 1 : 0; }
 extern "C" void pk_persist2_set_poll_delay(int units) { g2_poll_delay = units; }
 extern "C" void pk_persist2_set_trace(void* dev_buf) { g2_trace = (unsigned long long*)dev_buf; }
@@ -830,6 +867,12 @@
     return act == PK_ACT_RELU ? rec2_bwd_kernel<CELL, PK_ACT_RELU, false>
          : act == PK_ACT_TANH ? rec2_bwd_kernel<CELL, PK_ACT_TANH, false> : rec2_bwd_kernel<CELL, -1, false>;
 }
+template <int CELL, bool NOSAVE>
+Rec2Kernel pick_fwd_seg(int act) {
+    return act == PK_ACT_RELU ? rec2_fwd_kernel<CELL, PK_ACT_RELU, false, false, NOSAVE, true>
+         : act == PK_ACT_TANH ? rec2_fwd_kernel<CELL, PK_ACT_TANH, false, false, NOSAVE, true>
+                              : rec2_fwd_kernel<CELL, -1, false, false, NOSAVE, true>;
+}
 inline bool traced(int cell, int act) { return g2_trace != nullptr && cell == PK_CELL_LIGRU && act == PK_ACT_RELU; }
 inline Rec2Kernel pick_fwd_ln(int cell) {
     return cell == PK_CELL_LIGRU ? rec2_fwd_kernel<PK_CELL_LIGRU, -1, false, true>
@@ -851,9 +894,17 @@
 static int rec_fwd_bf16_impl(void* stream, int cell, int act, int T, int B, int bidir, int H, const float* P,
                              const float* pscale, const float* pshift, const float* U, const float* mask,
                              float mask_scalar, float* Y, float* S, uint16_t* Yb, int64_t y_pitch, int prefilled,
-                             const PkLnHost* ln) {
-    int rc = pk_rec2_check("pk_rec_fwd_bf16", 1, cell, T, B, bidir, H);
+                             const PkLnHost* ln, bool seg = false, int t_begin = 0, int t_end = 0) {
+    int rc = pk_rec2_check(seg ? "pk_rec_fwd_bf16_seg" : "pk_rec_fwd_bf16", 1, cell, T, B, bidir, H);
     if (rc) return rc;
+    if (seg) {
+        PK_REQUIRE((cell == PK_CELL_LIGRU || cell == PK_CELL_RNN) && !pk_rec3_covers(cell, 0) && !traced(cell, act),
+                   "pk_rec_fwd_bf16_seg: cell %d is not covered (liGRU / RNN on the second-generation forward kernel)", cell);
+        PK_REQUIRE(ln == nullptr, "pk_rec_fwd_bf16_seg: per-step LayerNorm is not covered");
+        PK_REQUIRE(Y != nullptr, "pk_rec_fwd_bf16_seg: Y must not be null (a segment resumes from it)");
+        PK_REQUIRE(prefilled == 2 && pk_rec_self_fill(cell) == 1, "pk_rec_fwd_bf16_seg: prefilled must be 2 (self-filling exchange)");
+        PK_REQUIRE(0 <= t_begin && t_begin < t_end && t_end <= T, "pk_rec_fwd_bf16_seg: bad step window [%d, %d) of %d", t_begin, t_end, T);
+    }
     PK_REQUIRE(S != nullptr || (ln == nullptr && !traced(cell, act)), "pk_rec_fwd_bf16: S may be null only without per-step LayerNorm");
     PK_REQUIRE(Y != nullptr || S == nullptr, "pk_rec_fwd_bf16: Y may be null only together with S");
     hipStream_t st = pk_stream(stream);
@@ -870,6 +921,7 @@
     a.P = P; a.pscale = pscale; a.pshift = pshift; a.U = U; a.mask = mask; a.mask_scalar = mask_scalar;
     a.Y = Y; a.S = S; a.Yb = (unsigned short*)Yb; a.Xb = nullptr; a.Ypitch = (int)y_pitch;
     a.dY = nullptr; a.dP2 = nullptr; a.dGb = nullptr; a.Gpitch = 0;
+    a.t_begin = seg ? t_begin : 0; a.t_end = seg ? t_end : T;
     rc = pk_rec2_host_setup(a, false, cell);
     if (rc) return rc;
     const bool lstm8 = cell == PK_CELL_LSTM && pk_rec2l_enabled();
@@ -877,19 +929,22 @@
     if (prefilled != 1 && !a.self_fill) PK_CHECK_HIP(hipMemsetAsync(Yb, 0xFF, (size_t)T * B * y_pitch * 2, st));
     rc = pk_rec2_ln_setup(st, a, pl, ln, false);
     if (rc) return rc;
-    if (lstm8 && !ln) return pk_rec2l_launch(st, a, pl, act, false);
-    if (!ln && pk_rec3_covers(cell, 0)) return pk_rec3_launch(st, a, pl, cell, act, false, traced(cell, act));
+    if (lstm8 && !ln && !seg) return pk_rec2l_launch(st, a, pl, act, false);
+    if (!ln && !seg && pk_rec3_covers(cell, 0)) return pk_rec3_launch(st, a, pl, cell, act, false, traced(cell, act));
     const int G = pk_cell_gates(cell);
     const size_t lds = 2 * (size_t)RMAX * pk_r2_lda_bf16(KPAD) * 2 + 4 * ((size_t)(G + 1 + pk_cell_saved(cell) + (ln ? 1 : 0)) * 1024 + 512) + 16;
     const bool nosave = S == nullptr;
-    const Rec2Kernel k = ln ? pick_fwd_ln(cell)
+    const Rec2Kernel k = seg ? (cell == PK_CELL_LIGRU ? (nosave ? pick_fwd_seg<PK_CELL_LIGRU, true>(act) : pick_fwd_seg<PK_CELL_LIGRU, false>(act))
+                                                      : (nosave ? pick_fwd_seg<PK_CELL_RNN, true>(act) : pick_fwd_seg<PK_CELL_RNN, false>(act)))
+                       : ln ? pick_fwd_ln(cell)
                        : nosave ? (cell == PK_CELL_LIGRU ? pick_fwd_nosave<PK_CELL_LIGRU>(act) : cell == PK_CELL_RNN ? pick_fwd_nosave<PK_CELL_RNN>(act)
                                                                                                                       : pick_fwd_nosave<PK_CELL_LSTM>(act))
                                 : pick_fwd(cell, act);
     {
-        static size_t granted[3][8] = {{0}, {0}, {0}};
+        static size_t granted[3][14] = {{0}, {0}, {0}};
         const int slot = cell == PK_CELL_LIGRU ? 0 : cell == PK_CELL_RNN ? 1 : 2;
-        const int as = ln ? 4 : nosave ? 5 + act_slot(act) : traced(cell, act) ? 3 : act_slot(act);
+        const int as = seg ? 8 + (nosave ? 3 : 0) + act_slot(act)
+                     : ln ? 4 : nosave ? 5 + act_slot(act) : traced(cell, act) ? 3 : act_slot(act);
         if (granted[slot][as] < lds) {
             PK_CHECK_HIP(hipFuncSetAttribute((const void*)k, hipFuncAttributeMaxDynamicSharedMemorySize, (int)lds));
             granted[slot][as] = lds;
@@ -901,9 +956,9 @@
         rc = pk_rec2_reset_handshake(st, a);
         if (rc) return rc;
         dim3 grid(pl.C * pl.Pn), block(256);
-        rc = pk_rec2_check_residency((const void*)k, 256, lds, pl.C * pl.Pn, "pk_rec_fwd_bf16");
+        rc = pk_rec2_check_residency((const void*)k, 256, lds, pl.C * pl.Pn, seg ? "pk_rec_fwd_bf16_seg" : "pk_rec_fwd_bf16");
         if (rc) return rc;
-        const int help = ln ? 0 : pk_rec_helper_wanted(false, pl.launches, cell);
+        const int help = (ln || seg) ? 0 : pk_rec_helper_wanted(false, pl.launches, cell);
         if (help && (rc = pk_rec_helper_fork(st)) != 0) return rc;
         hipLaunchKernelGGL(k, grid, block, lds, st, a);
         PK_LAUNCH_CHECK();
@@ -916,6 +971,13 @@
                                float mask_scalar, float* Y, float* S, uint16_t* Yb, int64_t y_pitch, int prefilled) {
     return rec_fwd_bf16_impl(stream, cell, act, T, B, bidir, H, P, pscale, pshift, U, mask, mask_scalar, Y, S, Yb, y_pitch,
                              prefilled, nullptr);
+}
+extern "C" int pk_rec_fwd_bf16_seg(void* stream, int cell, int act, int T, int B, int bidir, int H, const float* P,
+                                   const float* pscale, const float* pshift, const float* U, const float* mask,
+                                   float mask_scalar, float* Y, float* S, uint16_t* Yb, int64_t y_pitch, int prefilled,
+                                   int t_begin, int t_end) {
+    return rec_fwd_bf16_impl(stream, cell, act, T, B, bidir, H, P, pscale, pshift, U, mask, mask_scalar, Y, S, Yb, y_pitch,
+                             prefilled, nullptr, true, t_begin, t_end);
 }
 extern "C" int pk_rec_fwd_bf16_ln(void* stream, int cell, int act, int T, int B, int bidir, int H, const float* P,
                                   const float* pscale, const float* pshift, const float* U, const float* mask,
diff --git a/pytorch-kaldi_amd/functional.py b/pytorch-kaldi_amd/functional.py
--- a/pytorch-kaldi_amd/functional.py
+++ b/pytorch-kaldi_amd/functional.py
@@ -384,18 +384,23 @@
     _lib.check(rc, "pk_gemm_bf16_stats")
     if rb.value == 0:
         return done(*bn_stats(C if ldc == N else C.as_strided((M, N), (ldc, 1))))
+    if gates is not None:
+        return _merge_finalize_gates(lib, stats, rb.value, N, gates)
     mean, var = torch.empty(N, device=C.device), torch.empty(N, device=C.device)
-    if gates is not None:
-        gamma, beta, eps, H, rms, rvs, nbs, momentum, count = gates
-        G = len(rms)
-        scale, shift = torch.empty_like(mean), torch.empty_like(mean)
-        arr = lambda ts: (ctypes.c_void_p * G)(*[t.data_ptr() for t in ts])
-        _lib.check(lib.pk_bn_stats_merge_finalize_gates(_stream(), _p(stats), rb.value, G, H, _p(mean), _p(var), _p(gamma),
-                                                        _p(beta), eps, _p(scale), _p(shift), arr(rms), arr(rvs), arr(nbs),
-                                                        momentum, float(count)), "pk_bn_stats_merge_finalize_gates")
-        return mean, var, scale, shift
     _lib.check(lib.pk_bn_stats_merge(_stream(), _p(stats), rb.value, N, _p(mean), _p(var)), "pk_bn_stats_merge")
     return mean, var
+
+
+def _merge_finalize_gates(lib, stats, row_blocks, N, gates):
+    gamma, beta, eps, H, rms, rvs, nbs, momentum, count = gates
+    G = len(rms)
+    mean, var = torch.empty(N, device=stats.device), torch.empty(N, device=stats.device)
+    scale, shift = torch.empty_like(mean), torch.empty_like(mean)
+    arr = lambda ts: (ctypes.c_void_p * G)(*[t.data_ptr() for t in ts])
+    _lib.check(lib.pk_bn_stats_merge_finalize_gates(_stream(), _p(stats), row_blocks, G, H, _p(mean), _p(var), _p(gamma),
+                                                    _p(beta), eps, _p(scale), _p(shift), arr(rms), arr(rvs), arr(nbs),
+                                                    momentum, float(count)), "pk_bn_stats_merge_finalize_gates")
+    return mean, var, scale, shift
 
 
 def _splitk_bf(out_tiles, K):
@@ -1678,6 +1683,83 @@
             torch.cuda.current_stream().wait_stream(_Prefill.stream)
 
 
+class _ProjStream:
+    FRACTIONS = (0.54, 0.66, 0.78, 0.89)
+    streamed = 0
+
+    @staticmethod
+    def cuts(T, bidir):
+        e = _lib.experiment("proj_stream_cuts")
+        if e:
+            try:
+                return [int(v) for v in e.split(":")]
+            except ValueError:
+                return []
+        if bidir:
+            return sorted(set(int(round(T * f)) for f in _ProjStream.FRACTIONS))
+        return sorted(set(T * k // 5 for k in range(1, 5)))
+
+    @staticmethod
+    def plan(lib, cell, T, B, bidir, N_next):
+        if (_lib.experiment("proj_stream", "1") == "0" or not settings.wgrad_side or not settings.self_fill
+                or _lib.experiment("gemm_stats", "1") == "0" or cell not in ("liGRU", "RNN")
+                or (_lib.experiment("rec_gen_fwd") or _lib.experiment("rec_gen") or "2")[:1] not in ("2",)
+                or lib.pk_rec_self_fill(CELL[cell]) != 1 or torch.cuda.is_current_stream_capturing()):
+            return None
+        if lib.pk_gemm_bf16_stats_fused(T * B, N_next) != 1:
+            return None
+        cuts = _ProjStream.cuts(T, bidir)
+        if not cuts or len(cuts) > 16:
+            return None
+        out = (ctypes.c_int * (4 * (len(cuts) + 1)))()
+        n = lib.pk_proj_stream_plan(T, B, int(bidir), len(cuts), (ctypes.c_int * len(cuts))(*cuts), out)
+        if n != len(cuts) + 1:
+            return None
+        bands = [[(out[4 * k + 2 * j], out[4 * k + 2 * j + 1]) for j in (0, 1) if out[4 * k + 2 * j + 1] > 0] for k in range(n)]
+        return cuts, bands
+
+    @staticmethod
+    def run(lib, plan, nxt, Yb, T, B, ndir, H, like, run_segment):
+        cuts, bands = plan
+        TB = T * B
+        Wn = nxt["Wcat"].contiguous()
+        N = Wn.shape[0]
+        Hp = _up(H, 8)
+        Wb = cvt_bf16(Wn, ndir, H, Hp)
+        K = ndir * Hp
+        assert Wb.shape[1] == Yb.shape[1]
+        P = _new(TB, N, like=like)
+        stats = torch.empty(int(lib.pk_gemm_bf16_stats_floats(TB, N)), device=Yb.device, dtype=torch.float32)
+
+        def band(k):
+            for row0, rows in bands[k]:
+                _lib.check(lib.pk_gemm_bf16_stats_rows(_stream(), row0, rows, TB, N, K, 1.0, _p(Yb), Yb.shape[1], 1, _p(Wb),
+                                                       Wb.shape[1], 1, _p(P), N, None, _p(stats)), "pk_gemm_bf16_stats_rows")
+
+        main = torch.cuda.current_stream()
+        if _Side.stream is None:
+            _Side.stream = _make_side_stream()
+        side = _Side.stream
+        bounds = [0] + list(cuts) + [T]
+        ev = None
+        for k in range(len(bounds) - 1):
+            run_segment(bounds[k], bounds[k + 1])
+            if ev is not None and bands[k - 1]:
+                side.wait_event(ev)
+                with torch.cuda.stream(side):
+                    band(k - 1)
+            if k < len(bounds) - 2:
+                ev = torch.cuda.Event()
+                ev.record(main)
+        for t in (Yb, Wb, P, stats):
+            t.record_stream(side)
+        main.wait_stream(side)
+        band(len(bounds) - 2)
+        mean, var, pscale, pshift = _merge_finalize_gates(lib, stats, (TB + 255) // 256, N, nxt["gates"])
+        nxt["out"].update(Wb=Wb, P=P, mean=mean, var=var, pscale=pscale, pshift=pshift)
+        _ProjStream.streamed += 1
+
+
 class RecLayerPerfFn(torch.autograd.Function):
 
     @staticmethod
@@ -1696,7 +1778,12 @@
         TB, GH = T * B, G * H
         Wcat = Wcat.contiguous()
         Ucat = Ucat.contiguous()
-        if xb_in is None:
+        nxt = cfg[17] if len(cfg) > 17 else None
+        pre = (cfg[18] or None) if len(cfg) > 18 else None
+        if pre is not None:
+            assert xb_in is not None and pre["P"].shape == (TB, GH)
+            xb, Wb, K = xb_in, pre["Wb"], xseg[0] * xseg[2]
+        elif xb_in is None:
             xseg = None
             xb, Wb, K = cvt_bf16(_rows2d(x)), cvt_bf16(Wcat), D
         else:
@@ -1715,11 +1802,13 @@
         fill = _Prefill()
         if not self_fill:
             fill.start(Yb, Xb, dGb)
-        P = _new(TB, GH, like=Wcat)
+        P = pre["P"] if pre is not None else _new(TB, GH, like=Wcat)
         mean = var = None
         bn_bufs = cfg[14] if len(cfg) > 14 else None
         pscale = pshift = None
-        if use_bn and training and bn_bufs is not None:
+        if pre is not None:
+            mean, var, pscale, pshift = pre["mean"], pre["var"], pre["pscale"], pre["pshift"]
+        elif use_bn and training and bn_bufs is not None:
             mean, var, pscale, pshift = gemm_bf16_bn_stats(TB, GH, K, xb, xb.shape[1], 1, Wb, Wb.shape[1], 1, P, GH, gates=(
                 gamma, beta, eps, H, bn_bufs[0], bn_bufs[1], bn_bufs[2], momentum, ndir * TB))
         elif use_bn and training:
@@ -1750,10 +1839,21 @@
                                        Yb.shape[1], 2 if self_fill else fill.done)
             _lib.check(rc, "pk_rec2p_fwd_bf16")
         else:
-            rc = lib.pk_rec_fwd_bf16(_stream(), CELL[cell], ACT[act], T, B, int(bidir), H, _p(P), _p(pscale), _p(pshift),
-                                     _p(Ucat), _p(mask), float(mask_scalar), _p(Yarg), _p(S), _p(Yb), Yb.shape[1],
-                                     2 if self_fill else fill.done)
-            _lib.check(rc, "pk_rec_fwd_bf16")
+            plan = None
+            if nxt is not None and Yarg is not None and self_fill:
+                plan = _ProjStream.plan(lib, cell, T, B, bidir, nxt["Wcat"].shape[0])
+            if plan is not None:
+                def run_segment(t0, t1):
+                    _lib.check(lib.pk_rec_fwd_bf16_seg(_stream(), CELL[cell], ACT[act], T, B, int(bidir), H, _p(P), _p(pscale),
+                                                       _p(pshift), _p(Ucat), _p(mask), float(mask_scalar), _p(Yarg), _p(S),
+                                                       _p(Yb), Yb.shape[1], 2, t0, t1), "pk_rec_fwd_bf16_seg")
+
+                _ProjStream.run(lib, plan, nxt, Yb, T, B, ndir, H, Wcat, run_segment)
+            else:
+                rc = lib.pk_rec_fwd_bf16(_stream(), CELL[cell], ACT[act], T, B, int(bidir), H, _p(P), _p(pscale), _p(pshift),
+                                         _p(Ucat), _p(mask), float(mask_scalar), _p(Yarg), _p(S), _p(Yb), Yb.shape[1],
+                                         2 if self_fill else fill.done)
+                _lib.check(rc, "pk_rec_fwd_bf16")
         if S is not None:
             _force_kinks(S, cell, T, B, ndir, H)
         ctx.self_fill = self_fill
diff --git a/pytorch-kaldi_amd/nn.py b/pytorch-kaldi_amd/nn.py
--- a/pytorch-kaldi_amd/nn.py
+++ b/pytorch-kaldi_amd/nn.py
@@ -426,6 +426,22 @@
             out.append(list(self.ln[i].parameters()))
         return out
 
+    def _projection_ahead(self, j):
+        H = self._lay[j]
+        if (self.KIND not in ("liGRU", "RNN") or not (self._use_bn[j] and self.training)
+                or not F_.perf_path_ok(self.KIND, H, bool(self._use_ln[j]), True, True)):
+            return None
+        wps = [getattr(self, w)[j].weight.detach() for (w, _, _) in self._gates]
+        bns = [getattr(self, b)[j] for (_, _, b) in self._gates]
+        gps, bps = [b.weight.detach() for b in bns], [b.bias.detach() for b in bns]
+        Wcat, gamma, beta = F_.adjacent_view(wps), F_.adjacent_view(gps), F_.adjacent_view(bps)
+        Wcat = Wcat if Wcat is not None else torch.cat(wps, 0)
+        gamma = gamma if gamma is not None else torch.cat(gps, 0)
+        beta = beta if beta is not None else torch.cat(bps, 0)
+        return {"Wcat": Wcat, "out": {},
+                "bn": (gamma, beta, 1e-5, H, [b.running_mean for b in bns], [b.running_var for b in bns],
+                       [b.num_batches_tracked for b in bns], 0.05)}
+
     def forward(self, x, drop_masks=None):
         if not x.is_cuda:
             raise PkError("pytorch-kaldi_amd.nn.%s runs on the GPU only: set use_cuda=True" % self.KIND)
@@ -441,6 +457,7 @@
             masks = [m.to(x.device).float().contiguous() if m is not None else None for m in masks]
         batch = x.shape[1]
         xb = xseg = None
+        ahead = None
         for i in range(self._n_lay):
             mask_i, scalar_i = (masks[i], scalars[i]) if masks is not None else self._drop_mask(i, batch, x.device)
             H = self._lay[i]
@@ -489,10 +506,16 @@
                 stats_in_kernel = use_bn and self.training
                 bn_bufs = ([b.running_mean for b in bns], [b.running_var for b in bns],
                            [b.num_batches_tracked for b in bns]) if stats_in_kernel else None
+                pre = ahead["out"] if (ahead is not None and xb is not None) else None
+                ahead = None
+                if keep_y and i + 1 < self._n_lay and F_._lib.experiment("proj_stream", "1") != "0":
+                    ahead = self._projection_ahead(i + 1)
+                    if ahead is not None:
+                        ahead["gates"] = ahead["bn"] + ((2 if self.bidir else 1) * x.shape[0] * x.shape[1],)
                 y, bmean, bvar, xb = F_.RecLayerPerfFn.apply(x, xb, Wcat.detach() if side_w else Wcat, bcat,
                                                            Ucat.detach() if side_u else Ucat, gamma, beta, rmean, rvar,
                                                            mask_i, cfg + (xseg, wps, ups, side_w, side_u, bn_bufs, affine,
-                                                                          keep_y), edge_t)
+                                                                          keep_y, ahead, pre), edge_t)
                 xseg = (2 if self.bidir else 1, H, (H + 7) // 8 * 8)
                 if stats_in_kernel:
                     x = y
@@ -518,7 +541,7 @@
                 lnb = self.ln[i].beta if self._use_ln[i] else None
                 y, bmean, bvar = F_.RecLayerFn.apply(x, Wcat, bcat, Ucat, gamma, beta, rmean, rvar, mask_i, lng, lnb,
                                                      cfg + (wps, ups, side_w, side_u))
-                xb = xseg = None
+                xb = xseg = ahead = None
             if use_bn and self.training:
                 n = x.shape[0] * x.shape[1] * (2 if self.bidir else 1)
                 with torch.no_grad():
```

Result: no change. 3.792 million (-0.3%).
